# mimbres/neural-audio-fp

Hardware: AMD Instinct MI355X
Metric: fingerprint generation throughput (1-s segments/s) (higher is better)
Workload: dtype f32

## Files before the change

### include/nafp.h

```cpp
#ifndef NAFP_H
#define NAFP_H

#include <stdint.h>

#ifdef __cplusplus
extern "C" {
#endif

#define NAFP_ABI_VERSION 1

enum {
    NAFP_OK = 0,
    NAFP_ERR_INVALID_ARG = 1,
    NAFP_ERR_UNSUPPORTED = 2,
    NAFP_ERR_HIP = 3,
    NAFP_ERR_WORKSPACE = 4,
    NAFP_ERR_NO_WEIGHTS = 5
};

typedef struct nafp_melspec nafp_melspec;
typedef struct nafp_encoder nafp_encoder;

int nafp_abi_version(void);
const char* nafp_status_string(int status);
// ... 165 lines not shown
    int64_t n_indexed;
    int64_t indexed_samples;
    int32_t rate, channels, bps, min_block, max_block, refusal;
    uint8_t md5[16];
} nafp_flac_info;

typedef struct nafp_flac_index_entry {
    int64_t offset;
    int64_t first_sample;
    int64_t n_bytes;
    int32_t block_size;
    int32_t reserved;
} nafp_flac_index_entry;

typedef struct nafp_flac_frame {
    int64_t raw_off;
    int64_t scratch_off;
    int32_t n_bytes;
    int32_t block_size;
    int32_t channels;
    int32_t bps;
    int32_t rate;
    int32_t reserved;
} nafp_flac_frame;

int nafp_flac_streaminfo_host(const void* bytes, int64_t n_bytes, nafp_flac_info* info);
int nafp_flac_index_host(const void* bytes, int64_t n_bytes, nafp_flac_info* info, nafp_flac_index_entry* frames_out, int64_t cap);
int nafp_flac_decode_host(const void* raw, int64_t raw_size, const nafp_flac_frame* frames_host, int64_t n_frames, void* scratch,
                          int64_t scratch_size, int32_t* status_out);
int nafp_flac_check_frames_host(const nafp_flac_frame* frames_host, int64_t n_frames, int64_t raw_size, int64_t scratch_size);
int nafp_flac_decode(const uint8_t* raw, int64_t raw_size, const nafp_flac_frame* frames_dev, int64_t n_frames, uint8_t* scratch,
                     int64_t scratch_size, int32_t* status_dev, void* stream);


int nafp_encoder_create(nafp_encoder** enc, int in_f, int in_t, int emb_sz);
int nafp_encoder_destroy(nafp_encoder* enc);

#define NAFP_NORM_LAYER2D 0
#define NAFP_NORM_LAYER1D 1
#define NAFP_NORM_BATCH 2
int nafp_encoder_create_ex(nafp_encoder** enc, int in_f, int in_t, int emb_sz, int norm);
int nafp_encoder_norm(const nafp_encoder* enc);
int nafp_encoder_n_trainable(const nafp_encoder* enc);

int nafp_encoder_n_tensors(const nafp_encoder* enc);
int64_t nafp_encoder_tensor_numel(const nafp_encoder* enc, int index);
int nafp_encoder_tensor_shape(const nafp_encoder* enc, int index, int64_t dims_out[4]);
int64_t nafp_encoder_flat_dim(const nafp_encoder* enc);

int nafp_encoder_set_weights(nafp_encoder* enc, const float* const* tensors_host_array,
                             void* stream);

int64_t nafp_encoder_workspace_bytes(const nafp_encoder* enc, int64_t n_seg);

int nafp_encoder_forward(nafp_encoder* enc, const float* feat, int64_t n_seg,
                         void* workspace, int64_t workspace_bytes,
                         float* out_flat, float* out_emb, int l2norm, void* stream);

int nafp_encoder_forward_raw(nafp_encoder* enc, const float* raw_feat, const float* group_stat, int group_size,
                             int segment_norm, int64_t n_seg, void* workspace, int64_t workspace_bytes,
                             float* out_flat, float* out_emb, int l2norm, void* stream);

int64_t nafp_encoder_conv0_numel(const nafp_encoder* enc);
int nafp_encoder_conv0(nafp_encoder* enc, const float* feat, const float* group_stat, int group_size, int segment_norm,
                       int64_t n_seg, float* z0_out, long long* stats_out, void* stream);

#define NAFP_ENCODER_PROFILE_KERNELS 17
int nafp_encoder_profile_enable(nafp_encoder* enc, int max_forwards);
int nafp_encoder_profile_count(const nafp_encoder* enc);
int nafp_encoder_profile_coarse(nafp_encoder* enc, int coarse);
int nafp_encoder_profile_read(nafp_encoder* enc, int slot, float* ms_out_host);
int nafp_conv_timeline(void* dev_buf, int64_t capacity_u64, int cin, int cout, int positions);
int nafp_conv_timeline_grid(int* out5_host);
#define NAFP_CONV_PLAN_FIELDS 30
#define NAFP_PLAN_PLAIN 1
#define NAFP_PLAN_DGRAD 2
#define NAFP_PLAN_V_OUT 4
#define NAFP_PLAN_TICKETS 8
#define NAFP_PLAN_SPLIT_WEIGHTS 16
#define NAFP_PLAN_FUSE0 32
#define NAFP_PLAN_SIZE_DGRAD 64
int nafp_conv_plan(int in_f, int in_t, int layer, int64_t n_seg, int64_t plan_b, int flags, int64_t slab_floats,
                   int64_t* record_host, char* kernel_name_host, int name_capacity);

int64_t nafp_encoder_train_workspace_bytes(const nafp_encoder* enc, int64_t n_seg);
int nafp_encoder_forward_train(nafp_encoder* enc, const float* feat, int64_t n_seg, void* workspace,
                               int64_t workspace_bytes, float* out_emb, int l2norm, void* stream);
int nafp_encoder_backward(nafp_encoder* enc, const float* feat, const float* d_emb, int64_t n_seg,
                          void* workspace, int64_t workspace_bytes, float* const* grads_host_array,
                          int l2norm, void* stream);

#define NAFP_GRAD_GROUPS 4
int nafp_encoder_grad_group_range(const nafp_encoder* enc, int group, int* first_tensor, int* last_tensor);
int nafp_encoder_grad_group_wait(nafp_encoder* enc, int group, void* stream);

#define NAFP_OPT_FUSE_CONV0 1
#define NAFP_OPT_FUSED_LN_BWD 2
#define NAFP_OPT_BWD_OVERLAP 4
#define NAFP_OPT_SMALLNET 5
#define NAFP_OPT_BF16X3 3
#define NAFP_OPT_NONMATRIX 8
#define NAFP_NONMATRIX_CONV0 1
#define NAFP_NONMATRIX_KEEP_OWN 2
#define NAFP_NONMATRIX_ALL 3
#define NAFP_NONMATRIX_DEFAULT NAFP_NONMATRIX_ALL
int nafp_encoder_set_option(nafp_encoder* enc, int option, int value);

int nafp_encoder_div_enc(nafp_encoder* enc, const float* flat, int64_t n_seg,
                         float* out_emb, int l2norm, void* stream);

int nafp_l2_normalize_rows(const float* x, int64_t n_rows, int dim, float* out, void* stream);

int nafp_pack_embedding_grads(const float* d_a_all, const float* d_b_all, const float* loss_sum, float loss_scale,
                              int64_t world, int64_t n_anchors, int dim, float* send, void* stream);


int64_t nafp_ntxent_workspace_bytes(int64_t n_local, int64_t n_global);

int nafp_ntxent_forward(const float* emb_org_local, const float* emb_rep_local,
                        const float* emb_org_all, const float* emb_rep_all,
                        int64_t n_local, int64_t n_global, int64_t rank_offset, int d,
                        float tau, float* loss_sum, float* sim_mtx,
                        float* d_org_all, float* d_rep_all,
                        void* workspace, int64_t workspace_bytes, void* stream);


typedef struct { int f0, f1, t0, t1; } nafp_rect;

int nafp_specaug_apply(float* feat, int64_t n_seg, int F, int T, const nafp_rect* rects_host,
                       int n_rects, const unsigned char* active, float fill_value, void* stream);

int nafp_specaug_apply_fill_dev(float* feat, int64_t n_seg, int F, int T, const nafp_rect* rects_host,
                                int n_rects, const unsigned char* active, const float* fill_value_dev,
                                void* stream);
int64_t nafp_specaug_mean_workspace_bytes(void);
int nafp_specaug_mean(const float* feat, int64_t n, float* mean_out, void* workspace, int64_t workspace_bytes,
                      void* stream);

int nafp_specaug_apply_ex(float* feat, int64_t n_seg, int F, int T, const int32_t* rects_dev, int n_rects, int64_t n_sets,
                          const unsigned char* active_dev, const float* filler, int64_t n_fill_seg,
                          const float* scale_offset_dev, void* stream);
int nafp_specaug_range(const float* feat, int64_t n, float* scale_offset_out, void* workspace, int64_t workspace_bytes,
                       void* stream);


typedef struct {
    float* param; const float* grad; float* m; float* v;
    int64_t numel; int64_t var_len;
} nafp_opt_tensor;

float nafp_cosine_decay_lr_host(float lr0, int64_t step, int64_t decay_steps, float alpha);
float nafp_cosine_decay_restarts_lr_host(float lr0, int64_t step, int64_t first_decay_steps, float t_mul,
                                         float m_mul, float alpha);

int nafp_adam_step(const nafp_opt_tensor* tensors_host, int n, float lr, float beta1, float beta2,
                   float eps, int64_t step, void* stream);

int64_t nafp_lamb_workspace_bytes(const nafp_opt_tensor* tensors_host, int n);
int nafp_lamb_step(const nafp_opt_tensor* tensors_host, int n, float lr, float beta1, float beta2,
                   float eps, float weight_decay, int64_t step, void* workspace,
                   int64_t workspace_bytes, void* stream);

int64_t nafp_triplet_workspace_bytes(int64_t n_anchor, int64_t n_pos);
int nafp_triplet_forward(const float* emb_anchor, const float* emb_pos, int64_t n_anchor, int64_t n_pos, int dim,
                         int mode, float margin, float* loss_out, float* pairwise_dist, float* d_anchor,
                         float* d_pos, void* workspace, int64_t workspace_bytes, void* stream);
// ... 156 lines not shown
```

### neural-audio-fp_amd/_lib.py

```python
import ctypes
import os

import torch

_HERE = os.path.dirname(os.path.abspath(__file__))
LIB_PATH = os.environ.get('NAFP_LIB') or os.path.join(_HERE, 'libnafp.so')

c_i64 = ctypes.c_int64
c_int = ctypes.c_int
c_float = ctypes.c_float
c_void_p = ctypes.c_void_p

PROTOTYPES = {
    'nafp_abi_version': (c_int, []),
    'nafp_status_string': (ctypes.c_char_p, [c_int]),
    'nafp_last_hip_error': (c_int, []),
    'nafp_crc32c_host': (ctypes.c_uint32, [c_void_p, c_i64, ctypes.c_uint32]),
    'nafp_mel_filterbank_host': (c_int, [c_int, c_int, c_int, c_float, c_float, c_void_p]),
    'nafp_melspec_create': (c_int, [ctypes.POINTER(c_void_p), c_int, c_int, c_int, c_int, c_int, c_float, c_float]),
    'nafp_melspec_create_ex': (c_int, [ctypes.POINTER(c_void_p), c_int, c_int, c_int, c_int, c_int, c_float, c_float, c_int]),
    'nafp_melspec_plan_host': (c_int, [c_int, c_int, c_int, c_int, c_int, c_float, c_float, c_int, c_void_p]),
    'nafp_melspec_kernel': (c_int, [c_void_p]),
    'nafp_melspec_destroy': (c_int, [c_void_p]),
    'nafp_melspec_n_frames': (c_int, [c_void_p]),
    'nafp_melspec_n_mels': (c_int, [c_void_p]),
    'nafp_melspec_forward_f32': (c_int, [c_void_p, c_void_p, c_i64, c_int, c_int, c_void_p, c_void_p, c_void_p]),
    'nafp_melspec_forward_i16': (c_int, [c_void_p, c_void_p, c_i64, c_int, c_int, c_void_p, c_void_p, c_void_p]),
    'nafp_melspec_finish': (c_int, [c_void_p, c_void_p, c_void_p, c_i64, c_int, c_int, c_void_p]),
    'nafp_melspec_forward_windows_i16': (c_int, [c_void_p, c_void_p, c_void_p, c_void_p, c_i64, c_int, c_int, c_void_p,
                                                 c_void_p, c_void_p]),
    'nafp_resample_geometry': (c_int, [c_int, c_int, ctypes.POINTER(c_int), ctypes.POINTER(c_int), ctypes.POINTER(c_int),
                                       ctypes.POINTER(c_int)]),
    'nafp_resample_table_host': (c_int, [c_int, c_int, c_void_p]),
    'nafp_resample_n_out': (c_i64, [c_i64, c_int, c_int]),
    'nafp_resample_input_range': (c_int, [c_i64, c_i64, c_i64, c_int, c_int, ctypes.POINTER(c_i64), ctypes.POINTER(c_i64)]),
    'nafp_resample_check_pieces_host': (c_int, [c_int, c_int, c_void_p, c_i64, c_i64, c_i64]),
    'nafp_resample_create': (c_int, [ctypes.POINTER(c_void_p), c_int, c_int]),
    'nafp_resample_destroy': (c_int, [c_void_p]),
    'nafp_resample_i16': (c_int, [c_void_p, c_void_p, c_i64, c_void_p, c_i64, c_void_p, c_i64, c_void_p]),
    'nafp_ingest_geometry': (c_int, [c_int, c_int, ctypes.POINTER(c_int), ctypes.POINTER(c_int), ctypes.POINTER(c_int),
                                     ctypes.POINTER(c_int)]),
    'nafp_ingest_table_host': (c_int, [c_int, c_int, c_void_p]),
    'nafp_ingest_n_out': (c_i64, [c_i64, c_int, c_int]),
    'nafp_ingest_input_range': (c_int, [c_i64, c_i64, c_i64, c_int, c_int, ctypes.POINTER(c_i64), ctypes.POINTER(c_i64)]),
    'nafp_ingest_decode_host': (c_int, [c_int, c_void_p, c_i64, c_void_p]),
    'nafp_ingest_check_pieces_host': (c_int, [c_int, c_int, c_void_p, c_i64, c_i64, c_i64]),
    'nafp_ingest_create': (c_int, [ctypes.POINTER(c_void_p), c_int, c_int]),
    'nafp_ingest_destroy': (c_int, [c_void_p]),
    'nafp_ingest_i16': (c_int, [c_void_p, c_void_p, c_i64, c_void_p, c_i64, c_void_p, c_i64, c_void_p]),
    'nafp_varispeed_geometry': (c_int, [ctypes.c_uint32, ctypes.POINTER(c_int), ctypes.POINTER(c_int)]),
    'nafp_varispeed_table_host': (c_int, [ctypes.c_uint32, c_void_p]),
    'nafp_varispeed_n_out': (c_i64, [c_i64, ctypes.c_uint32]),
    'nafp_varispeed_input_range': (c_int, [c_i64, c_i64, c_i64, ctypes.c_uint32, ctypes.POINTER(c_i64), ctypes.POINTER(c_i64)]),
    'nafp_varispeed_check_pieces_host': (c_int, [ctypes.c_uint32, c_void_p, c_i64, c_i64, c_i64]),
    'nafp_varispeed_create': (c_int, [ctypes.POINTER(c_void_p), ctypes.c_uint32]),
    'nafp_varispeed_destroy': (c_int, [c_void_p]),
    'nafp_varispeed_i16': (c_int, [c_void_p, c_void_p, c_i64, c_void_p, c_i64, c_void_p, c_i64, c_void_p]),
    'nafp_codec_samples_per_block': (c_int, [c_int, c_int, c_int]),
    'nafp_codec_blocks_per_group': (c_int, [c_int, c_int, c_int]),
    'nafp_codec_decode_host': (c_int, [c_int, c_int, c_int, c_void_p, c_i64, c_void_p]),
    'nafp_codec_check_pieces_host': (c_int, [c_void_p, c_i64, c_i64, c_i64]),
    'nafp_codec_decode_i16': (c_int, [c_void_p, c_i64, c_void_p, c_i64, c_void_p, c_i64, c_void_p]),
    'nafp_flac_streaminfo_host': (c_int, [c_void_p, c_i64, c_void_p]),
    'nafp_flac_index_host': (c_int, [c_void_p, c_i64, c_void_p, c_void_p, c_i64]),
    'nafp_flac_decode_host': (c_int, [c_void_p, c_i64, c_void_p, c_i64, c_void_p, c_i64, c_void_p]),
    'nafp_flac_check_frames_host': (c_int, [c_void_p, c_i64, c_i64, c_i64]),
    'nafp_flac_decode': (c_int, [c_void_p, c_i64, c_void_p, c_i64, c_void_p, c_i64, c_void_p, c_void_p]),
    'nafp_encoder_create': (c_int, [ctypes.POINTER(c_void_p), c_int, c_int, c_int]),
    'nafp_encoder_create_ex': (c_int, [ctypes.POINTER(c_void_p), c_int, c_int, c_int, c_int]),
    'nafp_encoder_norm': (c_int, [c_void_p]),
    'nafp_encoder_n_trainable': (c_int, [c_void_p]),
    'nafp_encoder_destroy': (c_int, [c_void_p]),
    'nafp_encoder_n_tensors': (c_int, [c_void_p]),
    'nafp_encoder_tensor_numel': (c_i64, [c_void_p, c_int]),
    'nafp_encoder_tensor_shape': (c_int, [c_void_p, c_int, ctypes.POINTER(c_i64)]),
    'nafp_encoder_flat_dim': (c_i64, [c_void_p]),
    'nafp_encoder_set_weights': (c_int, [c_void_p, ctypes.POINTER(c_void_p), c_void_p]),
    'nafp_encoder_workspace_bytes': (c_i64, [c_void_p, c_i64]),
    'nafp_encoder_forward': (c_int, [c_void_p, c_void_p, c_i64, c_void_p, c_i64, c_void_p, c_void_p, c_int, c_void_p]),
    'nafp_encoder_forward_raw': (c_int, [c_void_p, c_void_p, c_void_p, c_int, c_int, c_i64, c_void_p, c_i64, c_void_p, c_void_p,
                                         c_int, c_void_p]),
    'nafp_encoder_conv0_numel': (c_i64, [c_void_p]),
    'nafp_encoder_conv0': (c_int, [c_void_p, c_void_p, c_void_p, c_int, c_int, c_i64, c_void_p, c_void_p, c_void_p]),
    'nafp_encoder_profile_enable': (c_int, [c_void_p, c_int]),
    'nafp_encoder_profile_count': (c_int, [c_void_p]),
    'nafp_encoder_profile_coarse': (c_int, [c_void_p, c_int]),
    'nafp_encoder_profile_read': (c_int, [c_void_p, c_int, c_void_p]),
    'nafp_conv_timeline': (c_int, [c_void_p, c_i64, c_int, c_int, c_int]),
    'nafp_conv_timeline_grid': (c_int, [c_void_p]),
    'nafp_conv_plan': (c_int, [c_int, c_int, c_int, c_i64, c_i64, c_int, c_i64, c_void_p, c_void_p, c_int]),
    'nafp_encoder_set_option': (c_int, [c_void_p, c_int, c_int]),
    'nafp_encoder_train_workspace_bytes': (c_i64, [c_void_p, c_i64]),
    'nafp_encoder_forward_train': (c_int, [c_void_p, c_void_p, c_i64, c_void_p, c_i64, c_void_p, c_int, c_void_p]),
    'nafp_encoder_backward': (c_int, [c_void_p, c_void_p, c_void_p, c_i64, c_void_p, c_i64,
                                      ctypes.POINTER(c_void_p), c_int, c_void_p]),
    'nafp_encoder_grad_group_range': (c_int, [c_void_p, c_int, ctypes.POINTER(c_int), ctypes.POINTER(c_int)]),
    'nafp_encoder_grad_group_wait': (c_int, [c_void_p, c_int, c_void_p]),
    'nafp_encoder_div_enc': (c_int, [c_void_p, c_void_p, c_i64, c_void_p, c_int, c_void_p]),
    'nafp_ntxent_workspace_bytes': (c_i64, [c_i64, c_i64]),
    'nafp_ntxent_forward': (c_int, [c_void_p, c_void_p, c_void_p, c_void_p, c_i64, c_i64, c_i64, c_int,
                                    c_float, c_void_p, c_void_p, c_void_p, c_void_p, c_void_p, c_i64, c_void_p]),
    'nafp_specaug_apply': (c_int, [c_void_p, c_i64, c_int, c_int, c_void_p, c_int, c_void_p, c_float, c_void_p]),
    'nafp_specaug_apply_fill_dev': (c_int, [c_void_p, c_i64, c_int, c_int, c_void_p, c_int, c_void_p, c_void_p, c_void_p]),
    'nafp_specaug_mean_workspace_bytes': (c_i64, []),
    'nafp_specaug_mean': (c_int, [c_void_p, c_i64, c_void_p, c_void_p, c_i64, c_void_p]),
    'nafp_specaug_apply_ex': (c_int, [c_void_p, c_i64, c_int, c_int, c_void_p, c_int, c_i64, c_void_p, c_void_p, c_i64, c_void_p, c_void_p]),
    'nafp_specaug_range': (c_int, [c_void_p, c_i64, c_void_p, c_void_p, c_i64, c_void_p]),
    'nafp_l2_normalize_rows': (c_int, [c_void_p, c_i64, c_int, c_void_p, c_void_p]),
    'nafp_pack_embedding_grads': (c_int, [c_void_p, c_void_p, c_void_p, c_float, c_i64, c_i64, c_int, c_void_p, c_void_p]),
    'nafp_cosine_decay_lr_host': (c_float, [c_float, c_i64, c_i64, c_float]),
    'nafp_cosine_decay_restarts_lr_host': (c_float, [c_float, c_i64, c_i64, c_float, c_float, c_float]),
    'nafp_adam_step': (c_int, [c_void_p, c_int, c_float, c_float, c_float, c_float, c_i64, c_void_p]),
    'nafp_lamb_workspace_bytes': (c_i64, [c_void_p, c_int]),
    'nafp_triplet_workspace_bytes': (c_i64, [c_i64, c_i64]),
    'nafp_triplet_forward': (c_int, [c_void_p, c_void_p, c_i64, c_i64, c_int, c_int, c_float, c_void_p, c_void_p, c_void_p,
                                     c_void_p, c_void_p, c_i64, c_void_p]),
    'nafp_augment_rows': (c_int, [c_void_p, c_void_p, c_i64, c_int, c_void_p, c_void_p]),
    'nafp_search_index_aux_floats': (c_i64, [c_i64]),
    'nafp_search_index_prepare': (c_int, [c_void_p, c_i64, c_int, c_void_p, c_void_p]),
    'nafp_search_workspace_bytes': (c_i64, [c_i64, c_i64, c_int]),
    'nafp_search_topk_l2': (c_int, [c_void_p, c_i64, c_void_p, c_void_p, c_i64, c_int, c_int, c_void_p, c_void_p,
                                    c_void_p, c_i64, c_void_p]),
    'nafp_search_topk_l2_excl': (c_int, [c_void_p, c_i64, c_void_p, c_void_p, c_i64, c_int, c_int, c_void_p, c_void_p, c_void_p,
                                         c_void_p, c_i64, c_void_p]),
    'nafp_search_seq_scores': (c_int, [c_void_p, c_void_p, c_i64, c_int, c_void_p, c_void_p, c_i64, c_void_p, c_int,
                                       c_void_p, c_void_p]),
    'nafp_search_seq_match': (c_int, [c_void_p, c_i64, c_void_p, c_i64, c_int, c_void_p, c_int, c_void_p, c_void_p, c_i64, c_int,
                                      c_int, c_void_p, c_void_p, c_void_p, c_void_p]),
    'nafp_search_identify': (c_int, [c_void_p, c_i64, c_void_p, c_i64, c_int, c_void_p, c_int, c_void_p, c_void_p, c_i64, c_int,
                                     c_void_p, c_int, c_int, c_int, c_int, c_int, c_void_p, c_void_p, c_void_p, c_void_p, c_void_p,
                                     c_void_p, c_void_p]),
    'nafp_search_identify_check_tracks_host': (c_int, [c_void_p, c_int, c_i64]),
    'nafp_search_identify_tempo': (c_int, [c_void_p, c_i64, c_void_p, c_i64, c_int, c_void_p, c_int, c_void_p, c_void_p, c_i64, c_int,
                                           c_void_p, c_int, c_void_p, c_int, c_int, c_int, c_int, c_int, c_void_p, c_void_p, c_void_p,
                                           c_void_p, c_void_p, c_void_p, c_void_p, c_void_p]),
    'nafp_ivf_bucket_workspace_bytes': (c_i64, [c_i64, c_int, c_int]),
    'nafp_ivf_bucket': (c_int, [c_void_p, c_int, c_i64, c_int, c_int, c_void_p, c_void_p, c_void_p, c_i64, c_void_p]),
    'nafp_ivf_kmeans_update': (c_int, [c_void_p, c_i64, c_int, c_int, c_void_p, c_void_p, c_int, c_void_p, c_void_p, c_void_p]),
    'nafp_ivf_residuals': (c_int, [c_void_p, c_i64, c_int, c_void_p, c_void_p, c_void_p, c_void_p]),
    'nafp_ivf_pq_encode': (c_int, [c_void_p, c_i64, c_int, c_void_p, c_void_p, c_void_p, c_int, c_void_p, c_void_p]),
    'nafp_ivf_probe': (c_int, [c_void_p, c_i64, c_void_p, c_int, c_int, c_int, c_void_p, c_void_p]),
    'nafp_ivf_flat_rows_bound': (c_i64, [c_i64, c_int]),
    'nafp_ivf_flat_lists': (c_int, [c_void_p, c_i64, c_int, c_void_p, c_void_p, c_int, c_void_p, c_void_p, c_void_p, c_void_p,
                                    c_void_p]),
    'nafp_ivf_pq_lists': (c_int, [c_void_p, c_i64, c_int, c_void_p, c_void_p, c_void_p]),
    'nafp_ivf_search_workspace_bytes': (c_i64, [c_i64, c_int, c_int, c_int, c_int]),
    'nafp_ivf_flat_search': (c_int, [c_void_p, c_i64, c_void_p, c_int, c_int, c_int, c_void_p, c_void_p, c_void_p, c_void_p, c_int,
                                     c_void_p, c_void_p, c_void_p, c_i64, c_void_p]),
    'nafp_ivf_pq_search': (c_int, [c_void_p, c_i64, c_void_p, c_int, c_int, c_int, c_void_p, c_int, c_void_p, c_void_p, c_void_p,
                                   c_int, c_void_p, c_void_p, c_void_p, c_i64, c_void_p]),
    'nafp_ivf_pq_search_ex': (c_int, [c_void_p, c_i64, c_void_p, c_int, c_int, c_int, c_void_p, c_int, c_void_p, c_void_p, c_void_p,
                                      c_int, c_void_p, c_void_p, c_int, c_void_p, c_i64, c_void_p]),
    'nafp_ivf_pq_adc_tables': (c_int, [c_void_p, c_i64, c_void_p, c_void_p, c_i64, c_void_p, c_int, c_int, c_void_p, c_int, c_int,
                                       c_void_p, c_void_p]),
    'nafp_ivf_pq_residuals': (c_int, [c_void_p, c_i64, c_int, c_void_p, c_int, c_void_p, c_void_p, c_void_p]),
    'nafp_ivf_refine_encode': (c_int, [c_void_p, c_i64, c_int, c_void_p, c_int, c_int, c_int, c_void_p, c_void_p]),
    'nafp_ivf_pq_wide_workspace_bytes': (c_i64, [c_i64, c_int, c_int, c_int]),
    'nafp_ivf_pq_search_wide': (c_int, [c_void_p, c_i64, c_void_p, c_int, c_int, c_int, c_void_p, c_int, c_void_p, c_void_p, c_void_p,
                                        c_int, c_void_p, c_void_p, c_int, c_void_p, c_i64, c_void_p]),
    'nafp_ivf_pqr_rerank': (c_int, [c_void_p, c_i64, c_int, c_void_p, c_int, c_void_p, c_void_p, c_void_p, c_int, c_void_p, c_void_p,
                                    c_int, c_int, c_void_p, c_i64, c_int, c_void_p, c_void_p, c_void_p]),
    'nafp_ivf_pqr_search': (c_int, [c_void_p, c_i64, c_void_p, c_int, c_int, c_int, c_void_p, c_int, c_void_p, c_void_p, c_void_p,
                                    c_void_p, c_void_p, c_void_p, c_int, c_int, c_void_p, c_i64, c_int, c_int, c_void_p, c_void_p,
                                    c_void_p, c_void_p, c_int, c_void_p, c_i64, c_void_p]),
    'nafp_hnsw_default_max_expansions': (c_int, [c_int]),
    'nafp_hnsw_reverse_workspace_bytes': (c_i64, [c_i64, c_i64, c_int, c_int]),
    'nafp_hnsw_search_workspace_bytes': (c_i64, [c_i64, c_int, c_int]),
    'nafp_hnsw_search_layer': (c_int, [c_void_p, c_i64, c_int, c_void_p, c_void_p, c_i64, c_i64, c_int, c_int, c_void_p, c_i64, c_void_p,
                                       c_void_p, c_int, c_int, c_int, c_void_p, c_void_p, c_void_p]),
    'nafp_hnsw_select_forward': (c_int, [c_void_p, c_i64, c_int, c_i64, c_i64, c_void_p, c_int, c_int, c_void_p, c_void_p, c_int, c_void_p,
                                         c_void_p, c_i64, c_i64, c_void_p]),
    'nafp_hnsw_reverse_links': (c_int, [c_void_p, c_i64, c_int, c_i64, c_i64, c_void_p, c_int, c_int, c_void_p, c_void_p, c_i64, c_i64,
                                        c_void_p, c_i64, c_void_p]),
# ... 97 lines not shown
```

### neural-audio-fp_amd/build.py

```python
import hashlib
import os
import subprocess
import sys
from concurrent.futures import ThreadPoolExecutor

HERE = os.path.dirname(os.path.abspath(__file__))
CSRC = os.path.join(HERE, 'csrc')
OBJ = os.path.join(HERE, 'build')
LIB = os.path.join(HERE, 'libnafp.so')
STAMP = os.path.join(HERE, '.libnafp.stamp')
SOURCES = ['api.hip', 'melspec.hip', 'melspec_any.hip', 'conv.hip', 'conv_plan.hip', 'tail.hip', 'ntxent.hip', 'optim.hip', 'specaug.hip', 'backward.hip',
           'search.hip', 'augment.hip', 'triplet.hip', 'norm.hip', 'ivf.hip', 'hnsw.hip', 'resample.hip', 'ingest.hip', 'codec.hip', 'flac.hip', 'varispeed.hip']
HEADERS = ['nafp_common.h', 'melspec_plan.h', 'codec_decode.h', 'flac_decode.h', os.path.join('..', '..', 'include', 'nafp.h')]
NO_PACKED_F32 = ['-Xclang', '-target-feature', '-Xclang', '-packed-fp32-ops']
FLAGS = ['--offload-arch=gfx950', '-O3', '-std=c++17', '-fPIC', '-Wall', '-Wno-unused-result', '-fno-gpu-rdc'] + NO_PACKED_F32
RESOURCE_FLAG = '-Rpass-analysis=kernel-resource-usage'


def _sha(paths, extra=''):
    h = hashlib.sha256()
    for f in paths:
        with open(os.path.join(CSRC, f), 'rb') as fh:
            h.update(fh.read())
    h.update(extra.encode())
    return h.hexdigest()


def _digest():
    return _sha(SOURCES + HEADERS, ' '.join(FLAGS))


def build(force=False, verbose=True):
    want = _digest()
    if not force and os.path.exists(LIB) and os.path.exists(STAMP):
        with open(STAMP) as fh:
            if fh.read().strip() == want:
                return LIB
    hipcc = os.environ.get('HIPCC', '/opt/rocm/bin/hipcc')
    os.makedirs(OBJ, exist_ok=True)

    def compile_one(src):
        obj = os.path.join(OBJ, src[:-4] + '.o')
        tag = _sha([src] + HEADERS, ' '.join(FLAGS))
        tag_path = obj + '.sha'
        if not force and os.path.exists(obj) and os.path.exists(tag_path) and open(tag_path).read().strip() == tag:
            return obj
        cmd = [hipcc] + FLAGS + [RESOURCE_FLAG, '-c', os.path.join(CSRC, src), '-o', obj]
        if verbose:
            print('[nafp build]', ' '.join(cmd), flush=True)
        res = subprocess.run(cmd, check=False, stderr=subprocess.PIPE, text=True)
        remarks = [ln for ln in res.stderr.splitlines() if 'kernel-resource-usage' in ln]
        rest = [ln for ln in res.stderr.splitlines() if 'kernel-resource-usage' not in ln and "'-packed-fp32-ops' is not a recognized feature" not in ln]
        if rest:
            print('\n'.join(rest), file=sys.stderr, flush=True)
        if res.returncode != 0:
            raise subprocess.CalledProcessError(res.returncode, cmd)
        with open(obj[:-2] + '.resources.txt', 'w') as fh:
            fh.write('\n'.join(ln.split('remark: ', 1)[-1].replace(' [-Rpass-analysis=kernel-resource-usage]', '') for ln in remarks) + '\n')
        with open(tag_path, 'w') as fh:
            fh.write(tag)
        return obj

    with ThreadPoolExecutor(max_workers=min(len(SOURCES), os.cpu_count() or 1, 8)) as pool:
        objs = list(pool.map(compile_one, SOURCES))
    cmd = [hipcc, '--offload-arch=gfx950', '-shared', '-fPIC', '-fno-gpu-rdc'] + objs + ['-o', LIB]
    if verbose:
        print('[nafp build]', ' '.join(cmd), flush=True)
    subprocess.run(cmd, check=True)
    with open(STAMP, 'w') as fh:
        fh.write(want)
    return LIB


def device_disassembly(lib=None):
    import struct
    import tempfile
    lib = lib or LIB
    llvm = os.environ.get('LLVM_BIN', '/opt/rocm/lib/llvm/bin')
    out = []
    with tempfile.TemporaryDirectory() as tmp:
        fat = os.path.join(tmp, 'fat.bin')
        subprocess.run([os.path.join(llvm, 'llvm-objcopy'), '--dump-section', '.hip_fatbin=' + fat, lib, os.path.join(tmp, 'unused.so')], check=True)
        blob = open(fat, 'rb').read()
        magic = b'__CLANG_OFFLOAD_BUNDLE__'
        at, n_obj = blob.find(magic), 0
        while at >= 0:
            n_entries, = struct.unpack_from('<Q', blob, at + len(magic))
            pos = at + len(magic) + 8
            for _ in range(n_entries):
                off, size, tlen = struct.unpack_from('<QQQ', blob, pos)
                triple = blob[pos + 24: pos + 24 + tlen].decode()
                pos += 24 + tlen
                if 'gfx950' in triple and size:
                    co = os.path.join(tmp, f'co{n_obj}.o')
                    with open(co, 'wb') as fh:
                        fh.write(blob[at + off: at + off + size])
# ... 31 lines not shown
```

### neural-audio-fp_amd/csrc/api.hip

```cpp
#include "nafp_common.h"

#include <algorithm>
#include <cstdio>
#include <cstdlib>
#include <cstring>
#include <vector>

namespace nafp {

thread_local int g_last_hip_error = 0;

static const int kHiddenCh[8] = {128, 128, 256, 256, 512, 512, 1024, 1024};
static const int kStrideT[8] = {2, 2, 2, 2, 1, 2, 1, 2};

std::vector<ConvGeom> encoder_geometry(int in_f, int in_t) {
    std::vector<ConvGeom> g;
    int F = in_f, T = in_t, C = 1;
    for (int i = 0; i < 8; ++i) {
        SamePad pt = same_pad(T, 3, kStrideT[i]);
        g.push_back(ConvGeom{0, F, T, C, F, pt.n_out, kHiddenCh[i], kStrideT[i], pt.before});
        T = pt.n_out; C = kHiddenCh[i];
        SamePad pf = same_pad(F, 3, 2);
        g.push_back(ConvGeom{1, F, T, C, pf.n_out, T, kHiddenCh[i], 2, pf.before});
        F = pf.n_out;
    }
    return g;
}

struct CopyTable { const float* src[96]; float* dst[96]; int64_t n[96]; int nz[96]; int count; int* nonfinite; };
__device__ __forceinline__ float nz_scale(float g) { return fabsf(g) < 1e-30f ? copysignf(1e-30f, g) : g; }
__device__ __forceinline__ bool nonfinite4(float4 v) {
    return !(fabsf(v.x) <= 3.4028234664e38f) || !(fabsf(v.y) <= 3.4028234664e38f) || !(fabsf(v.z) <= 3.4028234664e38f) || !(fabsf(v.w) <= 3.4028234664e38f);
}
__global__ __launch_bounds__(256) void multi_copy_kernel(const CopyTable t) {
    const int e = blockIdx.y;
    const float* __restrict__ s = t.src[e]; float* __restrict__ d = t.dst[e];
    const int64_t n = t.n[e];
    const bool nz = t.nz[e] != 0;
    bool bad = false;
    if ((((uintptr_t)s | (uintptr_t)d) & 15) == 0) {
        for (int64_t i = blockIdx.x * 256ll + threadIdx.x; i < n / 4; i += (int64_t)gridDim.x * 256) {
            float4 v = ((const float4*)s)[i];
            bad = bad || nonfinite4(v);
            if (nz) { v.x = nz_scale(v.x); v.y = nz_scale(v.y); v.z = nz_scale(v.z); v.w = nz_scale(v.w); }
            ((float4*)d)[i] = v;
        }
        for (int64_t i = n / 4 * 4 + blockIdx.x * 256ll + threadIdx.x; i < n; i += (int64_t)gridDim.x * 256) {
            bad = bad || !(fabsf(s[i]) <= 3.4028234664e38f);
            d[i] = nz ? nz_scale(s[i]) : s[i];
        }
    } else {
        for (int64_t i = blockIdx.x * 256ll + threadIdx.x; i < n; i += (int64_t)gridDim.x * 256) {
            bad = bad || !(fabsf(s[i]) <= 3.4028234664e38f);
            d[i] = nz ? nz_scale(s[i]) : s[i];
        }
    }
    if (bad && t.nonfinite) atomicOr(t.nonfinite, 1);
}
#define NAFP_OPT_DEBUG_SIDE_DELAY 6
#define NAFP_OPT_DEBUG_SW_DELAY 7
__global__ void debug_delay_kernel(long long us) {
    const unsigned long long t0 = __builtin_amdgcn_s_memrealtime();
    while ((long long)(__builtin_amdgcn_s_memrealtime() - t0) < us * 100) __builtin_amdgcn_s_sleep(32);
}
struct BiasTable { float* hb[16]; const float* bias[16]; int64_t n[16]; int cout[16]; int count; };
__global__ __launch_bounds__(256) void add_bias_kernel(const BiasTable t) {
    const int e = blockIdx.y;
    float* __restrict__ h = t.hb[e]; const float* __restrict__ b = t.bias[e];
    const int64_t n = t.n[e]; const int C = t.cout[e];
    for (int64_t i = blockIdx.x * 256ll + threadIdx.x; i < n; i += (int64_t)gridDim.x * 256) h[i] += b[i % C];
}

}

using namespace nafp;

constexpr int NAFP_PROF_EV = 34;
struct nafp_encoder {
    int in_f, in_t, emb_sz;
    int norm = NAFP_NORM_LAYER2D;
    int n_trainable = 68;
    std::vector<float*> d_gc, d_bc, d_mm, d_mv;
    bool ln1d_images_set = false;
// ... 580 lines not shown
    t.w1p = e->d_w1p; t.b1p = e->d_b1p; t.w2p = e->d_w2p; t.b2 = e->d_b2;
    t.out_flat = out_flat; t.out_emb = out_emb;
    t.D = (int)e->flat_dim; t.Q = e->emb_sz; t.S = e->S; t.l2norm = l2norm; t.nonfinite_weights = e->d_wflag; t.launch_error = nullptr;
    if (ev && e->prof_coarse < 2) NAFP_HIP_CHECK(hipEventRecord(ev[32], st));
    rc = launch_tail(t, n_seg, st);
    if (rc != NAFP_OK) return rc;
    if (ev && e->prof_coarse < 2) NAFP_HIP_CHECK(hipEventRecord(ev[33], st));
    return NAFP_OK;
}

extern "C" int nafp_encoder_profile_enable(nafp_encoder* e, int max_forwards) {
    if (!e || max_forwards < 0 || max_forwards > 4096) return NAFP_ERR_INVALID_ARG;
    profile_free(e);
    for (int i = 0; i < max_forwards * NAFP_PROF_EV; ++i) {
        hipEvent_t ev;
        static const int ev_mode = []() { const char* v = getenv("NAFP_PROF_EVENT_FENCE"); return v ? atoi(v) : 0; }();
        hipError_t err = ev_mode == 1 ? hipEventCreate(&ev)
                         : hipEventCreateWithFlags(&ev, ev_mode == 2 ? hipEventReleaseToDevice : hipEventDisableSystemFence);
        if (err != hipSuccess) { g_last_hip_error = (int)err; profile_free(e); return NAFP_ERR_HIP; }
        e->prof_events.push_back(ev);
    }
    e->prof_max = max_forwards;
    return NAFP_OK;
}

extern "C" int nafp_encoder_profile_coarse(nafp_encoder* e, int coarse) {
    if (!e) return NAFP_ERR_INVALID_ARG;
    e->prof_coarse = coarse < 0 ? 0 : (coarse > 2 ? 2 : coarse);
    return NAFP_OK;
}

extern "C" int nafp_encoder_profile_count(const nafp_encoder* e) { return e ? e->prof_count : -1; }

extern "C" int nafp_encoder_profile_read(nafp_encoder* e, int slot, float* ms_out_host) {
    if (!e || !ms_out_host || slot < 0 || slot >= e->prof_count) return NAFP_ERR_INVALID_ARG;
    hipEvent_t* ev = e->prof_events.data() + (size_t)NAFP_PROF_EV * slot;
    NAFP_HIP_CHECK(hipEventSynchronize(e->prof_coarse == 2 ? ev[31] : ev[33]));
    for (int k = 0; k < 17; ++k) ms_out_host[k] = 0.f;
    if (e->prof_coarse == 2) {
        NAFP_HIP_CHECK(hipEventElapsedTime(ms_out_host + 1, ev[2], ev[31]));
        return NAFP_OK;
    }
    NAFP_HIP_CHECK(hipEventElapsedTime(ms_out_host + 0, ev[0], ev[1]));
    NAFP_HIP_CHECK(hipEventElapsedTime(ms_out_host + 16, ev[32], ev[33]));
    if (e->prof_coarse) {
        NAFP_HIP_CHECK(hipEventElapsedTime(ms_out_host + 1, ev[1], ev[32]));
        return NAFP_OK;
    }
    for (int j = 1; j < 16; ++j) NAFP_HIP_CHECK(hipEventElapsedTime(ms_out_host + j, ev[2 * j], ev[2 * j + 1]));
    return NAFP_OK;
}

extern "C" int nafp_conv_timeline(void* dev_buf, int64_t capacity_u64, int cin, int cout, int positions) {
    if (dev_buf && capacity_u64 <= 0) return NAFP_ERR_INVALID_ARG;
    return conv_timeline_set((unsigned long long*)dev_buf, capacity_u64, cin, cout, positions);
}
extern "C" int nafp_conv_timeline_grid(int* out5_host) {
    if (!out5_host) return NAFP_ERR_INVALID_ARG;
    return conv_timeline_grid(out5_host);
}

extern "C" int nafp_conv_plan(int in_f, int in_t, int layer, int64_t n_seg, int64_t plan_b, int flags, int64_t slab_floats,
                              int64_t* record_host, char* kernel_name_host, int name_capacity) {
    if (in_f <= 0 || in_t <= 0 || layer < 1 || layer > 15 || n_seg <= 0 || plan_b < 0 || slab_floats < 0 || !record_host) return NAFP_ERR_INVALID_ARG;
    const std::vector<ConvGeom> geom = encoder_geometry(in_f, in_t);
    ConvPlanIn in{};
    in.B = n_seg; in.plan_b = plan_b; in.slab_floats = slab_floats;
    in.plain = flags & NAFP_PLAN_PLAIN; in.dgrad = flags & NAFP_PLAN_DGRAD; in.v_out = flags & NAFP_PLAN_V_OUT; in.tickets = flags & NAFP_PLAN_TICKETS;
    in.split_weights = flags & NAFP_PLAN_SPLIT_WEIGHTS; in.bf16x3 = (flags >> 8) & 3;
    in.fuse0 = flags & NAFP_PLAN_FUSE0; in.f0_geom = in.fuse0 ? &geom[0] : nullptr;
    const ConvPlan pl = plan_conv_gemm(in, geom[layer], conv_knobs());
    for (int i = 0; i < NAFP_CONV_PLAN_FIELDS; ++i) record_host[i] = 0;
    record_host[29] = conv_gemm_slab_floats(n_seg, geom[layer], (flags & NAFP_PLAN_SIZE_DGRAD) != 0, plan_b);
    if (pl.rc != NAFP_OK) return pl.rc;
    const ConvKernelRow& row = conv_kernel_rows[pl.kernel];
    const int64_t rec[29] = {pl.kernel, pl.BM, pl.bn, row.ring, pl.lds_bytes, pl.grid.x, pl.grid.y, pl.grid.z, pl.PT, pl.ST, pl.n_sg, pl.n_pb, pl.k_steps,
                             pl.S, pl.finish, pl.finish_f4, pl.finish_grid, pl.mode, row.epi, row.arith, pl.perm_on, pl.perm_n0, pl.perm_c0,
                             pl.opt, pl.xcd_group, pl.xcd_full, pl.log2_ncol, pl.range_step, pl.abl};
    for (int i = 0; i < 29; ++i) record_host[i] = rec[i];
    if (kernel_name_host && name_capacity > 0) snprintf(kernel_name_host, (size_t)name_capacity, "%s", row.name);
    return NAFP_OK;
}

extern "C" int nafp_encoder_div_enc(nafp_encoder* e, const float* flat, int64_t n_seg,
                                    float* out_emb, int l2norm, void* stream) {
    if (!e || !flat || !out_emb || n_seg < 0) return NAFP_ERR_INVALID_ARG;
    if (!e->has_weights) return NAFP_ERR_NO_WEIGHTS;
    TailArgs t;
    t.x = flat; t.stats = nullptr; t.ident_stats = false; t.gamma = nullptr; t.beta = nullptr;
    t.w1p = e->d_w1p; t.b1p = e->d_b1p; t.w2p = e->d_w2p; t.b2 = e->d_b2;
    t.out_flat = nullptr; t.out_emb = out_emb;
    t.D = (int)e->flat_dim; t.Q = e->emb_sz; t.S = e->S; t.l2norm = l2norm; t.nonfinite_weights = e->d_wflag; t.launch_error = nullptr;
    { int wrc = wait_weights(e, (hipStream_t)stream); if (wrc != NAFP_OK) return wrc; }
    return launch_tail(t, n_seg, (hipStream_t)stream);
}


namespace {
struct TrainLayout {
    int64_t B;
    stat_t* stats; unsigned* tickets; float* mr; float* sc;
    char* zero_begin; int64_t zero_bytes;
    double* lnsum[16]; float* S1[16]; float* S2[16];
    float* z[16]; float* v[16];
    float* slab; int64_t slab_floats;
    float* slab2; int64_t slab2_floats; unsigned* tickets2;
    float* dA; float* dB; float* dy;
    float* dts[16];
    float* dgp; float* dbp;
    int64_t bytes;
};

TrainLayout train_layout(const nafp_encoder* e, int64_t B, void* ws) {
    TrainLayout L; L.B = B;
    char* p = (char*)(((uintptr_t)ws + 255) & ~(uintptr_t)255);
    char* p0 = p;
    auto take = [&](int64_t bytes) { char* r = p; p += (bytes + 255) / 256 * 256; return r; };
    L.stats = (stat_t*)take((int64_t)sizeof(stat_t) * 2 * 16 * B);
    L.tickets = (unsigned*)take(2 * NAFP_TICKET_SLOTS * (int64_t)sizeof(unsigned));
    L.tickets2 = L.tickets + NAFP_TICKET_SLOTS;
    L.mr = (float*)take((int64_t)sizeof(float) * 2 * 16 * B);
    L.sc = (float*)take((int64_t)sizeof(float) * 8 * B);
    L.zero_begin = p;
    for (int j = 0; j < 16; ++j) L.lnsum[j] = (double*)take((int64_t)sizeof(double) * 2 * B);
    for (int j = 0; j < 16; ++j) {
        const int64_t n = (int64_t)e->geom[j].Fout * e->geom[j].Tout * e->geom[j].Cout;
        L.S1[j] = (float*)take((int64_t)sizeof(float) * n);
        L.S2[j] = (float*)take((int64_t)sizeof(float) * n);
    }
    L.zero_bytes = p - L.zero_begin;
    int64_t max_n = 0;
    for (int j = 0; j < 16; ++j) {
        const int64_t n = (int64_t)e->geom[j].Fout * e->geom[j].Tout * e->geom[j].Cout;
        max_n = std::max(max_n, n);
        L.z[j] = (float*)take((int64_t)sizeof(float) * n * B);
        L.v[j] = ((j == 0 && e->norm != NAFP_NORM_LAYER1D) || !e->keep_t()) ? nullptr : (float*)take((int64_t)sizeof(float) * n * B);
    }
    L.slab_floats = 0;
    for (int j = 1; j < 16; ++j)
        L.slab_floats = std::max(L.slab_floats, std::max(conv_gemm_slab_floats(B, e->geom[j], true), wgrad_slab_floats(B, e->geom[j])));
    L.slab = (float*)take((int64_t)sizeof(float) * L.slab_floats);
    L.slab2_floats = 0;
    for (int j = 1; j < 16; ++j)
        if (e->geom[j].Fout * e->geom[j].Tout < 16) L.slab2_floats = std::max(L.slab2_floats, wgrad_slab_floats(B, e->geom[j]));
    L.slab2 = (float*)take((int64_t)sizeof(float) * L.slab2_floats);
    L.dA = (float*)take((int64_t)sizeof(float) * max_n * B);
    L.dB = (float*)take((int64_t)sizeof(float) * max_n * B);
    L.dy = (float*)take((int64_t)sizeof(float) * e->emb_sz * B);
    for (int j = 0; j < 16; ++j) {
        const int64_t n = (int64_t)e->geom[j].Fout * e->geom[j].Tout * e->geom[j].Cout;
        L.dts[j] = (j >= 1 && e->geom[j].Fout * e->geom[j].Tout < 16) ? (float*)take((int64_t)sizeof(float) * n * B) : nullptr;
    }
    L.dgp = nullptr; L.dbp = nullptr;
    if (e->norm != NAFP_NORM_LAYER2D) {
        L.dgp = (float*)take((int64_t)sizeof(float) * 2 * max_n);
        L.dbp = L.dgp + max_n;
    }
    L.bytes = (p - p0) + 256;
    return L;
}
}

extern "C" int64_t nafp_encoder_train_workspace_bytes(const nafp_encoder* e, int64_t n_seg) {
    if (!e || n_seg < 0) return -1;
    return train_layout(e, n_seg, nullptr).bytes;
}
// ... 252 lines not shown
```

### neural-audio-fp_amd/csrc/conv.hip

```cpp
#include "nafp_common.h"
#include <hip/hip_ext.h>

#include <cstdlib>

namespace nafp {

using f32x16 = __attribute__((ext_vector_type(16))) float;
using f32x2 = __attribute__((ext_vector_type(2))) float;
#ifndef NAFP_Z_AUX
#define NAFP_Z_AUX 0
#endif
#ifndef NAFP_T_AUX
#define NAFP_T_AUX 2
#endif
__device__ __forceinline__ int f2i(float x) { return __builtin_bit_cast(int, x); }

__device__ __forceinline__ f32x2 elu2(f32x2 t) {
    const f32x2 m = t * 1.44269504088896341f;
    f32x2 e;
    e.x = fminf(fmaxf(__builtin_amdgcn_exp2f(m.x), 0.f), 1.f);
    e.y = fminf(fmaxf(__builtin_amdgcn_exp2f(m.y), 0.f), 1.f);
    e = e - 1.0f;
    f32x2 r;
    r.x = fmaxf(t.x, e.x); r.y = fmaxf(t.y, e.y);
    return r;
}



template <bool STORE, int ROWS0>
__global__ __launch_bounds__(256) void conv0_kernel(
        const float* __restrict__ feat, const float* __restrict__ w3, const float* __restrict__ bias,
        const float* __restrict__ gamma, float* __restrict__ y, float* __restrict__ v_out,
        stat_t* __restrict__ stats, int F, int Tin, int Tout, int Cout, int stride, int pad,
        const float* __restrict__ gstat, int group_size, int segment_norm, int ident_stats) {
    constexpr int NP = 4;
    __shared__ float s_x[ROWS0 * 64 + 8];
    __shared__ double red[8];
    const int tid = threadIdx.x, lane = tid & 63, wave = tid >> 6;
    const int blocks_per_sample = (F + ROWS0 - 1) / ROWS0;
    const int64_t b = blockIdx.x / blocks_per_sample;
    const int f0 = (blockIdx.x % blocks_per_sample) * ROWS0;
    const int cgroups = Cout / 4;
    const int pos_per_iter = 256 / cgroups;
    const int cg = tid % cgroups, pslot = tid / cgroups;
    const int rows = min(ROWS0, F - f0);
    const int npos = rows * Tout;
    {
        float gmax = 0.f, nh = 0.f, nd = 1.f;
        if (gstat) {
            const int64_t g = group_size > 0 ? b / group_size : 0;
            gmax = gstat[2 * g];
            if (segment_norm) {
                const float mn = fmaxf(gstat[2 * g + 1] - gmax, -80.f);
                nh = mn / 2.f; nd = fabsf(nh + 1e-10f);
            }
        }
        const float* xin = feat + (b * F + f0) * (int64_t)Tin;
        for (int i = tid; i < rows * Tin; i += 256) {
            float v = xin[i];
            if (gstat) {
                v = max_keep_nan(v - gmax, -80.f);
                if (segment_norm) v = (v - nh) / nd;
            }
            s_x[(i / Tin) * 64 + (i % Tin)] = v;
        }
    }
    const float4 w0 = *(const float4*)(w3 + 0 * Cout + 4 * cg);
    const float4 w1 = *(const float4*)(w3 + 1 * Cout + 4 * cg);
    const float4 w2 = *(const float4*)(w3 + 2 * Cout + 4 * cg);
    const float4 bb = *(const float4*)(bias + 4 * cg);
    float* yout = STORE ? y + ((b * F + f0) * (int64_t)Tout) * Cout : nullptr;
    const float* gin = STORE ? gamma + ((int64_t)f0 * Tout) * Cout : nullptr;
    __syncthreads();
    float s = 0.f, q = 0.f;
    float4 g[NP], gn[NP];
#pragma unroll
    for (int i = 0; i < NP; ++i) {
        const int p = pslot + i * pos_per_iter;
        g[i] = make_float4(0.f, 0.f, 0.f, 0.f);
        if (STORE && p < npos) g[i] = *(const float4*)(gin + (int64_t)p * Cout + 4 * cg);
    }
    for (int p0 = pslot; p0 < npos; p0 += NP * pos_per_iter) {
// ... 223 lines not shown
        s += v; q = fmaf(v, v, q);
    }
    if (!live) { s = 0.f; q = 0.f; }
    const double ds = wave_sum((double)s), dq = wave_sum((double)q);
    if (lane == 0) { red[wave] = ds; red[4 + wave] = dq; }
    __syncthreads();
    if (tid == 0) {
        stat_add(stats + 2 * b, red[0] + red[1] + red[2] + red[3]);
        stat_add(stats + 2 * b + 1, red[4] + red[5] + red[6] + red[7]);
    }
}

int launch_conv0_stats(const float* feat, const float* w3, const float* bias, stat_t* stats, int64_t B,
                       const ConvGeom& g, hipStream_t st, const float* gstat, int group_size, int segment_norm) {
    if (g.Cin != 1 || g.axis != 0 || (g.Cout % 4) != 0 || 256 % (g.Cout / 4) != 0 || g.Tin > 64) return NAFP_ERR_UNSUPPORTED;
    static const bool old_form = []() { const char* e = getenv("NAFP_CONV0_STATS_OLD"); return e && e[0] == '1'; }();
    if (!old_form) {
        const int64_t bps = ((int64_t)g.Fin * g.Tout + 255) / 256;
        conv0_stats_kernel<<<dim3((unsigned)(B * bps)), 256, 0, st>>>(feat, w3, bias, stats, g.Fin, g.Tin, g.Tout, g.Cout, g.stride, g.pad,
                                                                      gstat, group_size, segment_norm);
        NAFP_LAUNCH_CHECK();
        return NAFP_OK;
    }
    constexpr int R = 32;
    const int64_t blocks = B * ((g.Fin + R - 1) / R);
    conv0_kernel<false, R><<<dim3((unsigned)blocks), 256, 0, st>>>(feat, w3, bias, nullptr, nullptr, nullptr, stats,
                                                                   g.Fin, g.Tin, g.Tout, g.Cout, g.stride, g.pad, gstat, group_size, segment_norm, 0);
    NAFP_LAUNCH_CHECK();
    return NAFP_OK;
}

constexpr int BN = 128;

#ifdef NAFP_ABLATION
#define NAFP_ABL(p_, bits_) ((p_).abl & (bits_))
#elif defined(NAFP_ABL_CONST)
#define NAFP_ABL(p_, bits_) ((NAFP_ABL_CONST) & (bits_))
#else
#define NAFP_ABL(p_, bits_) (0)
#endif

struct ConvKernelParams {
    const float* x;
    const float* wp;
    const float* wp_hm;
    const unsigned short* wp_l;
    const float* G;
    const float* Hb;
    const float* gamma_out;
    const float* bias;
    const stat_t* stats_in;
    stat_t* stats_out;
    float* y;
    float* v_out;
    int Fin, Tin, Cin, Tout, Cout;
    int axis, stride, pad;
    int B, P;
    int PT, ST, log2ST;
    int n_sg;
    int n_pb, log2_ncol;
    int xcd_group, xcd_full;
    int64_t sample_in;
    int tap_stride;
    double inv_n_in;
    int mode;
    int dgrad;
    int perm_on, perm_n0, perm_c0;
    unsigned wp_bytes;
    int n_split;
    int abl;
    unsigned* tickets;
    float* y_final;
    unsigned long long* tl;
    int opt;
    int keep_own;
    const float* f0_feat;
    const float* f0_w;
    const float* f0_bias;
    const float* f0_gamma;
    int f0_T, f0_stride, f0_pad;
    const float* f0_gstat;
    int f0_group, f0_segnorm;
    ScalarsJob sj;
};

typedef __attribute__((address_space(3))) void* lds_ptr_t;
typedef unsigned u32x4 __attribute__((ext_vector_type(4)));

__device__ __forceinline__ u32x4 make_rsrc(const void* base, unsigned bytes) {
    const unsigned long long a = (unsigned long long)base;
    u32x4 r;
    r.x = __builtin_amdgcn_readfirstlane((unsigned)a);
    r.y = __builtin_amdgcn_readfirstlane((unsigned)(a >> 32) & 0xffffu);
    r.z = __builtin_amdgcn_readfirstlane(bytes);
    r.w = 0x00020000u;
    return r;
}

__device__ __forceinline__ void lds_dma16(unsigned lds_addr, unsigned voff, u32x4 rsrc, unsigned soff) {
    unsigned keep;
    lds_addr = __builtin_amdgcn_readfirstlane(lds_addr);
    soff = __builtin_amdgcn_readfirstlane(soff);
    asm volatile("s_mov_b32 %0, m0\n\ts_mov_b32 m0, %1\n\ts_nop 4\n\t"
                 "buffer_load_dwordx4 %2, %3, %4 offen lds\n\ts_mov_b32 m0, %0"
                 : "=&s"(keep) : "s"(lds_addr), "v"(voff), "s"(rsrc), "s"(soff) : "memory");
}

struct RowGeom { int inner; unsigned mask; };
__device__ __forceinline__ RowGeom row_geom(const ConvKernelParams& p, int pos) {
    const int fo = pos / p.Tout, to = pos - fo * p.Tout;
    RowGeom g; g.mask = 0;
    if (!p.dgrad) {
        int pos0, lim;
        if (p.axis == 0) { pos0 = to * p.stride - p.pad; lim = p.Tin; g.inner = (fo * p.Tin + pos0) * p.Cin; }
        else             { pos0 = fo * p.stride - p.pad; lim = p.Fin; g.inner = (pos0 * p.Tin + to) * p.Cin; }
#pragma unroll
        for (int t = 0; t < 3; ++t)
            if (pos0 + t >= 0 && pos0 + t < lim) g.mask |= 1u << t;
    } else {
        const int u = (p.axis == 0 ? to : fo) + p.pad;
        const int n_out = p.axis == 0 ? p.Tin : p.Fin;
        const int S = p.axis == 0 ? p.Cin : p.Tin * p.Cin;
        const int A0 = p.axis == 0 ? (fo * p.Tin) * p.Cin : to * p.Cin;
        const int sh = p.stride == 2 ? 1 : 0;
        g.inner = A0 + ((u * S) >> sh);
#pragma unroll
        for (int k = 0; k < 3; ++k) {
            const int d = u - k;
            if (d >= 0 && (d & sh) == 0 && (d >> sh) < n_out) g.mask |= 1u << k;
        }
    }
    return g;
}

__device__ __forceinline__ int tile_pos(const ConvKernelParams& p, int idx) {
    if (!p.perm_on || idx >= p.P) return idx;
    if (p.perm_on == 2) {
        const int L = p.Tout, lines = p.P / L, n0 = L - 1;
        if (idx < lines * n0) { const int line = idx / n0; return line * L + (idx - line * n0); }
        return (idx - lines * n0) * L + n0;
    }
    const int n0 = p.perm_n0;
    if (p.axis == 0) {
        const int L = p.Tout, lines = p.P / L, n1 = L - n0;
        if (idx < lines * n0) { const int line = idx / n0; return line * L + 2 * (idx - line * n0) + p.perm_c0; }
        const int j = idx - lines * n0, line = j / n1;
        return line * L + 2 * (j - line * n1) + 1 - p.perm_c0;
    }
    if (idx < n0 * p.Tout) { const int e = idx / p.Tout; return (2 * e + p.perm_c0) * p.Tout + (idx - e * p.Tout); }
    const int j = idx - n0 * p.Tout, e = j / p.Tout;
    return (2 * e + 1 - p.perm_c0) * p.Tout + (j - e * p.Tout);
}

__device__ __forceinline__ float half_wave_sum_dpp(float x) {
    int v = __builtin_bit_cast(int, x);
#define NAFP_DPP_ADD(ctrl_, rmask_)                                                                       \
    v = __builtin_bit_cast(int, __builtin_bit_cast(float, v) +                                            \
                                    __builtin_bit_cast(float, __builtin_amdgcn_update_dpp(0, v, ctrl_, rmask_, 0xf, true)));
    NAFP_DPP_ADD(0x111, 0xf)
    NAFP_DPP_ADD(0x112, 0xf)
    NAFP_DPP_ADD(0x114, 0xf)
    NAFP_DPP_ADD(0x118, 0xf)
    NAFP_DPP_ADD(0x142, 0xa)
#undef NAFP_DPP_ADD
    return __builtin_bit_cast(float, v);
}

#ifndef NAFP_EXP_X6_NOSPLIT
#define NAFP_EXP_X6_NOSPLIT 0
#endif
#ifndef NAFP_EXP_SKIP_TAP2
#define NAFP_EXP_SKIP_TAP2 0
#endif
template <int BM, int BNT, int BK, int NSTAGE, bool FUSE0, int EPI, int PREC = 0>
__device__ __forceinline__ bool conv_gemm_body(const ConvKernelParams& p) {
    static_assert(!FUSE0 || (BK == 16 && BM == 128), "the in-kernel conv0 generator is written for BK = 16, BM = 128");
    static_assert(BM == 128 || BM == 256, "tile rows");
    static_assert(BNT == 128 || (BNT == 64 && BM == 128 && !FUSE0), "tile columns");
    constexpr int NIW = BNT / 64;
    constexpr int NT = 2 * BM;
    constexpr int NW = BM / 32;
    constexpr int CH = BK / 4;
    constexpr int RPI = 64 / CH;
    constexpr int NI = 32 / RPI;
    constexpr int BROWS = BNT / NW;
    constexpr int NIB = BROWS / RPI;
    static_assert(NIB >= 1, "B rows per wave");
    constexpr int TILE = (FUSE0 && PREC == 2) ? BM * 24 : BM * BK;
    constexpr int TILEB = BNT * BK;
    constexpr int LROWS = BNT / NW;
    constexpr int TILEL = PREC == 2 ? BNT * 8 : 0;
    constexpr int STAGE = TILE + TILEB + TILEL;
    constexpr int NDMA = NI + NIB + (PREC == 2 ? 1 : 0);
    extern __shared__ __attribute__((aligned(16))) float smem[];
    float* sRB = smem + NSTAGE * STAGE;
    float* sCB = sRB + BM;
    int* sPos = (int*)(sCB + BM);
    int* sInner = sPos + 32;
    unsigned* sMask = (unsigned*)(sPos + 64);
    float* sW0 = sCB + BM + 96;
    const int tid = threadIdx.x, lane = tid & 63;
    const int wave = __builtin_amdgcn_readfirstlane(tid >> 6);
    const int wm = wave >> 1, wn = wave & 1;
    int sg = blockIdx.x, pb = blockIdx.y, colz = blockIdx.z, zsp = 0;
    if (p.opt & 8) {
        const unsigned lin = blockIdx.x, G = (unsigned)p.xcd_group;
        unsigned v = lin;
        if (lin < (unsigned)p.xcd_full) {
            const unsigned xcd = lin & 7u, j = lin >> 3;
            const unsigned blk = j / G, i = j - blk * G;
            v = (blk * 8u + xcd) * G + i;
        }
        unsigned rt;
        if (p.opt & 16) {
            const unsigned n_rt = (unsigned)(p.n_sg * p.n_pb);
            unsigned t = v / n_rt; rt = v - t * n_rt;
            if (p.n_split > 1) { const unsigned c = t / (unsigned)p.n_split; zsp = (int)(t - c * (unsigned)p.n_split); t = c; }
            colz = (int)t;
        } else {
            colz = (int)(v & ((1u << p.log2_ncol) - 1u)); v >>= p.log2_ncol;
            if (p.n_split > 1) { const unsigned r = v / (unsigned)p.n_split; zsp = (int)(v - r * (unsigned)p.n_split); v = r; }
            rt = v;
        }
        pb = (int)(rt / (unsigned)p.n_sg); sg = (int)(rt - (unsigned)pb * (unsigned)p.n_sg);
    } else
    if (!(p.opt & 4)) { pb = blockIdx.x / p.n_sg; sg = blockIdx.x - pb * p.n_sg; colz = blockIdx.y; zsp = blockIdx.z; }
    if ((EPI == 3 || EPI == 5) && p.sj.sc) {
        const long long wg = blockIdx.x + (long long)gridDim.x * (blockIdx.y + (long long)gridDim.y * blockIdx.z);
        const long long n_wg = (long long)gridDim.x * gridDim.y * gridDim.z;
        for (long long b = wg * NT + tid; b < p.sj.B; b += n_wg * NT) {
            const float mean = p.sj.mr[2 * b], rstd = p.sj.mr[2 * b + 1];
            float* o = p.sj.sc + 8 * b;
            o[0] = mean; o[1] = rstd;
            o[2] = (float)(p.sj.lnsum[2 * b] * p.sj.inv_n); o[3] = (float)(p.sj.lnsum[2 * b + 1] * p.sj.inv_n);
            o[4] = 1.f / rstd;
            o[5] = p.sj.mr_prev ? p.sj.mr_prev[2 * b + 1] : 1.f;
            o[6] = p.sj.mr_prev ? -p.sj.mr_prev[2 * b] : 0.f;
            o[7] = 0.f;
        }
    }
    const int tile_n0 = colz * BNT;
    const int K = 3 * p.Cin;
#define NAFP_TL(k_)                                                                            \
    if (p.tl && lane == 0)                                                                                 \
        p.tl[(((size_t)blockIdx.x + (size_t)gridDim.x * (blockIdx.y + (size_t)gridDim.y * blockIdx.z)) * 8 + wave) * 8 + (k_)] = \
            __builtin_readcyclecounter();
    if (p.tl && lane == 0)
        p.tl[(((size_t)blockIdx.x + (size_t)gridDim.x * (blockIdx.y + (size_t)gridDim.y * blockIdx.z)) * 8 + wave) * 8] =
            (unsigned long long)__builtin_amdgcn_s_getreg(0xF804) |
            ((unsigned long long)__builtin_amdgcn_s_getreg(0xF814) << 32);
    NAFP_TL(1)
    if (p.opt & 1) __builtin_amdgcn_s_setprio(3);
    const int ST1 = p.ST - 1;
    const int b0 = sg * p.ST;
    const int nb = min(p.ST, p.B - b0);

    const bool stat_thread = tid >= 64 && tid < 64 + p.ST;
    double st_sum = 0.0, st_sq = 0.0;
    if (stat_thread && p.mode != 1 && b0 + tid - 64 < p.B) {
        st_sum = stat_get(p.stats_in + 2 * (int64_t)(b0 + tid - 64));
        st_sq = stat_get(p.stats_in + 2 * (int64_t)(b0 + tid - 64) + 1);
        if (st_sq != st_sq && p.stats_out) stat_poison(p.stats_out + 2 * (int64_t)(b0 + tid - 64));
    }
    if (tid < 32) {
        int pos = p.P, inner = 0; unsigned mask = 0;
        if (tid < p.PT) {
            pos = tile_pos(p, pb * p.PT + tid);
            if (pos < p.P) { const RowGeom rg = row_geom(p, pos); inner = rg.inner; mask = rg.mask; }
        }
        sPos[tid] = pos; sInner[tid] = inner; sMask[tid] = mask;
    }
    __syncthreads();

    constexpr unsigned OOB = 0x80000000u;
    unsigned voffA[NI];
    unsigned vmaskA[NI];
    unsigned voffB[NIB];
#pragma unroll
    for (int q = 0; q < NIB; ++q) {
        const int lr = wave * BROWS + q * RPI + lane / CH;
        const int pc = lane % CH;
        const int swz = BK == 32 ? ((lr >> 1) & 7) : ((lr >> 2) & 3);
        voffB[q] = (unsigned)((tile_n0 + lr) * K + (pc ^ swz) * 4) * 4u;
    }
#pragma unroll
    for (int q = 0; q < NI; ++q) {
        const int lr = wave * 32 + q * RPI + lane / CH;
        const int pc = lane % CH;
        const int swz = BK == 32 ? ((lr >> 1) & 7) : ((lr >> 2) & 3);
        const int lc = pc ^ swz;
        const int slot_q = lr >> p.log2ST;
        const int sl = lr & ST1;
        voffA[q] = 0; vmaskA[q] = 0;
        if (sPos[slot_q] < p.P && sl < nb) {
            voffA[q] = (unsigned)(sl * (int)p.sample_in + sInner[slot_q] + lc * 4) * 4u;
            vmaskA[q] = sMask[slot_q];
        }
    }
    float x0[3][3];
    unsigned g_valid = 0;
    int g_off = 0;
    const int g_row = tid >> 1, g_ch = (tid & 1) * 8;
    const int g_swz = (g_row >> 2) & 3;
    if (FUSE0) {
        for (int i = tid; i < 4 * p.Cin; i += NT) sW0[i] = i < 3 * p.Cin ? p.f0_w[i] : p.f0_bias[i - 3 * p.Cin];
#pragma unroll
        for (int t = 0; t < 3; ++t) { x0[t][0] = 0.f; x0[t][1] = 0.f; x0[t][2] = 0.f; }
        const int pos = pb * p.PT + (g_row >> p.log2ST);
        const int sl = g_row & ST1;
        if (pos < p.P && sl < nb) {
            float f0_gmax = 0.f, f0_nh = 0.f, f0_nd = 1.f;
            if (p.f0_gstat) {
                const int64_t gi = p.f0_group > 0 ? (int64_t)(b0 + sl) / p.f0_group : 0;
                f0_gmax = p.f0_gstat[2 * gi];
                if (p.f0_segnorm) { const float mn = fmaxf(p.f0_gstat[2 * gi + 1] - f0_gmax, -80.f); f0_nh = mn / 2.f; f0_nd = fabsf(f0_nh + 1e-10f); }
            }
            const int fo = pos / p.Tout, to = pos - fo * p.Tout;
            const int f00 = fo * p.stride - p.pad;
            g_off = (f00 * p.Tin + to) * p.Cin;
            const int t00 = to * p.f0_stride - p.f0_pad;
            const float* fb = p.f0_feat + ((int64_t)(b0 + sl) * p.Fin) * p.f0_T;
#pragma unroll
            for (int t = 0; t < 3; ++t) {
                const int f = f00 + t;
                if (f >= 0 && f < p.Fin) {
                    g_valid |= 1u << t;
#pragma unroll
                    for (int k = 0; k < 3; ++k) {
                        const int tt = t00 + k;
                        float xv = 0.f;
                        if (tt >= 0 && tt < p.f0_T) {
                            xv = fb[(int64_t)f * p.f0_T + tt];
                            if (p.f0_gstat) {
                                xv = max_keep_nan(xv - f0_gmax, -80.f);
                                if (p.f0_segnorm) xv = (xv - f0_nh) / f0_nd;
                            }
                        }
                        x0[t][k] = xv;
                    }
                }
            }
        }
        __syncthreads();
    }
    unsigned live = 0;
    {
        const unsigned m = sMask[lane & 31];
#pragma unroll
        for (int t = 0; t < 3; ++t)
            if (__ballot((m >> t) & 1u) != 0ull) live |= 1u << t;
    }
    unsigned tap_pack = 0; int n_live = 0;
#pragma unroll
    for (int t = 0; t < 3; ++t)
        if (live & (1u << t)) { tap_pack |= (unsigned)t << (2 * n_live); ++n_live; }
    const int cpt = p.Cin / BK;
    const int n_steps_all = n_live * cpt;
    int s_begin = 0, n_steps = n_steps_all;
    if (p.n_split > 1) {
        s_begin = (int)((unsigned)(n_steps_all * zsp) / (unsigned)p.n_split);
        n_steps = (int)((unsigned)(n_steps_all * (zsp + 1)) / (unsigned)p.n_split);
    }
#define NAFP_STEP_AT(step_, tsel_, c0_)                                                        \
    const int tsel_ = s_begin == 0 ? ((step_) >= cpt ? 1 : 0) : (step_) / cpt;                 \
    const int c0_ = ((step_) - tsel_ * cpt) * BK;

    const u32x4 rsA = make_rsrc(p.x + (int64_t)b0 * p.sample_in,
                                NAFP_ABL(p, 512) ? 0u : (unsigned)nb * (unsigned)p.sample_in * 4u);
    const u32x4 rsB = make_rsrc(PREC == 2 ? p.wp_hm : p.wp, NAFP_ABL(p, 4096) ? 0u : p.wp_bytes);
    const unsigned lds0 = (unsigned)(unsigned long long)(lds_ptr_t)smem + (unsigned)(wave * 32 * BK * 4);
    const unsigned ldsB0 = (unsigned)(unsigned long long)(lds_ptr_t)smem + (unsigned)((TILE + wave * BROWS * BK) * 4);
    const u32x4 rsL = make_rsrc((const float*)p.wp_l, NAFP_ABL(p, 4096) ? 0u : p.wp_bytes / 2);
    const unsigned ldsL0 = (unsigned)(unsigned long long)(lds_ptr_t)smem + (unsigned)((TILE + TILEB) * 4 + wave * LROWS * 32);
    const unsigned voffL = (unsigned)((tile_n0 + wave * LROWS + (lane >> 1)) * K) * 2u + (unsigned)(lane & 1) * 16u;
#define NAFP_DMA_L(slot_, k0_)                                                                 \
    if (PREC == 2 && lane < 2 * LROWS) lds_dma16(ldsL0 + (unsigned)((slot_) * STAGE * 4), voffL, rsL, (unsigned)((k0_) * 2));

#define NAFP_DMA_STEP(s_, slot_)                                                              \
    {                                                                                          \
        NAFP_STEP_AT(s_, tsel_l, c0_l)                                                         \
        const int tap_l = (int)((tap_pack >> (2 * tsel_l)) & 3u);                              \
        const unsigned la_l = lds0 + (unsigned)((slot_) * STAGE * 4);                          \
        const unsigned lb_l = ldsB0 + (unsigned)((slot_) * STAGE * 4);                         \
        const unsigned tapb_l = (unsigned)(tap_l * p.tap_stride) * 4u;                         \
        _Pragma("unroll") for (int q = 0; q < NI; ++q) {                                       \
            const unsigned va = ((vmaskA[q] >> tap_l) & 1u) ? voffA[q] + tapb_l : OOB;         \
            if (!FUSE0) lds_dma16(la_l + q * RPI * BK * 4, va, rsA, (unsigned)(c0_l * 4));     \
            if (q < NIB) lds_dma16(lb_l + q * RPI * BK * 4, voffB[q], rsB,                      \
                                   (unsigned)((tap_l * p.Cin + c0_l) * 4));                    \
        }                                                                                      \
        NAFP_DMA_L(slot_, tap_l * p.Cin + c0_l)                                                \
    }
    float4 gg0 = make_float4(0.f, 0.f, 0.f, 0.f), gg1 = gg0;
#define NAFP_GEN_LOAD(s_)                                                                     \
    {                                                                                          \
        const int tsel_l = (s_) / cpt;                                                         \
        const int tap_l = (int)((tap_pack >> (2 * tsel_l)) & 3u);                              \
        const int c0_l = ((s_) - tsel_l * cpt) * BK;                                           \
        const int go_l = ((g_valid >> tap_l) & 1u) ? g_off + tap_l * p.tap_stride + c0_l + g_ch : 0; \
        gg0 = *(const float4*)(p.f0_gamma + go_l);                                             \
        gg1 = *(const float4*)(p.f0_gamma + go_l + 4);                                         \
    }
#define NAFP_GEN_ONE(j_, G_) \
    __fmul_rn((ok_l ? elu1(fmaf(xc_l, wt_l[2 * p.Cin + (j_)], fmaf(xb_l, wt_l[p.Cin + (j_)], fmaf(xa_l, wt_l[(j_)], wt_l[3 * p.Cin + (j_)])))) : 0.f), (G_))
#define NAFP_GEN_STORE(s_, slot_)                                                             \
    {                                                                                          \
        const int tsel_l = (s_) / cpt;                                                         \
        const int tap_l = (int)((tap_pack >> (2 * tsel_l)) & 3u);                              \
        const int c0_l = ((s_) - tsel_l * cpt) * BK;                                           \
        const bool ok_l = (g_valid >> tap_l) & 1u;                                             \
        const float xa_l = tap_l == 0 ? x0[0][0] : (tap_l == 1 ? x0[1][0] : x0[2][0]);         \
        const float xb_l = tap_l == 0 ? x0[0][1] : (tap_l == 1 ? x0[1][1] : x0[2][1]);         \
        const float xc_l = tap_l == 0 ? x0[0][2] : (tap_l == 1 ? x0[1][2] : x0[2][2]);         \
        const float* wt_l = sW0 + c0_l + g_ch;                                                 \
        float* dst_l = smem + (slot_) * STAGE + g_row * BK;                                    \
        *(float4*)(dst_l + (((2 * (tid & 1)) ^ g_swz) * 4)) = make_float4(                      \
            NAFP_GEN_ONE(0, gg0.x), NAFP_GEN_ONE(1, gg0.y), NAFP_GEN_ONE(2, gg0.z), NAFP_GEN_ONE(3, gg0.w)); \
        *(float4*)(dst_l + (((2 * (tid & 1) + 1) ^ g_swz) * 4)) = make_float4(                  \
            NAFP_GEN_ONE(4, gg1.x), NAFP_GEN_ONE(5, gg1.y), NAFP_GEN_ONE(6, gg1.z), NAFP_GEN_ONE(7, gg1.w)); \
    }

    f32x16 acc[2][NIW];
#pragma unroll
    for (int mi = 0; mi < 2; ++mi)
#pragma unroll
        for (int ni = 0; ni < NIW; ++ni)
#pragma unroll
            for (int r = 0; r < 16; ++r) acc[mi][ni][r] = 0.f;

    NAFP_TL(2)
    if (p.opt & 1) __builtin_amdgcn_s_setprio(0);
#pragma unroll
    for (int s = 0; s < NSTAGE - 1; ++s)
        if (s_begin + s < n_steps) {
            NAFP_DMA_STEP(s_begin + s, s)
            if (FUSE0 && PREC != 2) {
                NAFP_GEN_LOAD(s_begin + s)
                NAFP_GEN_STORE(s_begin + s, s)
            }
        }

    if (stat_thread) {
        float r = 0.f, c = 0.f;
        if (p.mode != 1 && b0 + tid - 64 < p.B) {
            if (p.inv_n_in < 0.0) {
                const double z = st_sq * 0.0;
                r = (float)(1.0 + z); c = (float)z;
            } else {
                const double mean = st_sum * p.inv_n_in;
                double var = st_sq * p.inv_n_in - mean * mean;
                var = var < 0.0 ? 0.0 : var;
                const double rstd = 1.0 / sqrt(var + (double)LN_EPS);
                r = (float)rstd; c = (float)(-mean * rstd);
            }
        }
        sRB[tid - 64] = r; sCB[tid - 64] = c;
    }

    const int rl = lane & 31, hh = lane >> 5;
    const int rswz = BK == 32 ? ((rl >> 1) & 7) : ((rl >> 2) & 3);
    const int aoff = (wm * 64 + rl) * BK, boff = TILE + (wn * (BNT / 2) + rl) * BK;
    const int ncol = lane & 31;
    const int n_base = tile_n0 + wn * (BNT / 2) + ncol;
    const int g4 = p.ST >> 2;
    constexpr int MIL = 1;
    float Gv[MIL][4][NIW], Hv[MIL][4][NIW], gv[MIL][4][NIW];
    const int pc_bytes = p.P * p.Cout * 4;
    const __amdgpu_buffer_rsrc_t rsG = __builtin_amdgcn_make_buffer_rsrc(const_cast<float*>(p.G), 0, pc_bytes, 0x00020000);
    const __amdgpu_buffer_rsrc_t rsH = __builtin_amdgcn_make_buffer_rsrc(const_cast<float*>(p.Hb), 0, pc_bytes, 0x00020000);
    const __amdgpu_buffer_rsrc_t rsg = __builtin_amdgcn_make_buffer_rsrc(const_cast<float*>(p.gamma_out), 0, pc_bytes, 0x00020000);
#define NAFP_EPI_LOAD(mi_, slot_)                                                              \
    _Pragma("unroll") for (int rg = 0; rg < 4; ++rg) {                                         \
        const int grp_l = wm * 16 + (mi_) * 8 + 2 * rg + (lane >> 5);                          \
        const int pos_l = sPos[grp_l >> (p.log2ST - 2)];                \
        const int pofs_l = pos_l < p.P ? (pos_l * p.Cout + n_base) * 4 : (int)0x80000000;      \
        _Pragma("unroll") for (int ni = 0; ni < NIW; ++ni) {                                   \
            if NAFP_ABL(p, 32) { Gv[slot_][rg][ni] = 0.5f; Hv[slot_][rg][ni] = 0.25f; gv[slot_][rg][ni] = 1.5f; continue; } \
            Gv[slot_][rg][ni] = __builtin_bit_cast(float, __builtin_amdgcn_raw_buffer_load_b32(rsG, pofs_l, ni * 128, 0)); \
            Hv[slot_][rg][ni] = __builtin_bit_cast(float, __builtin_amdgcn_raw_buffer_load_b32(rsH, pofs_l, ni * 128, 0)); \
            gv[slot_][rg][ni] = __builtin_bit_cast(float, __builtin_amdgcn_raw_buffer_load_b32(rsg, pofs_l, ni * 128, 0)); \
        }                                                                                      \
    }
    int slot = 0;
    if NAFP_ABL(p, 8) {
        asm volatile("s_waitcnt vmcnt(0)" ::: "memory");
        if (acc[0][0][0] == 12345.678f) p.y[tid] = smem[tid];
        return false;
    }
#define NAFP_LD_FRAG(St_, kk_, a_, b_)                                                         \
    {                                                                                          \
        const int pc4_l = ((2 * (kk_) + hh) ^ rswz) * 4;                                       \
        _Pragma("unroll") for (int mi = 0; mi < 2; ++mi) a_[mi] = *(const float4*)((St_) + aoff + mi * 32 * BK + pc4_l);   \
        _Pragma("unroll") for (int ni = 0; ni < NIW; ++ni) b_[ni] = *(const float4*)((St_) + boff + ni * 32 * BK + pc4_l); \
    }
#define NAFP_MM_FRAG(a_, b_)                                                                   \
    _Pragma("unroll") for (int mi = 0; mi < 2; ++mi)                                           \
        _Pragma("unroll") for (int ni = 0; ni < NIW; ++ni) {                                   \
            acc[mi][ni] = __builtin_amdgcn_mfma_f32_32x32x2f32(a_[mi].x, b_[ni].x, acc[mi][ni], 0, 0, 0); \
            acc[mi][ni] = __builtin_amdgcn_mfma_f32_32x32x2f32(a_[mi].y, b_[ni].y, acc[mi][ni], 0, 0, 0); \
            acc[mi][ni] = __builtin_amdgcn_mfma_f32_32x32x2f32(a_[mi].z, b_[ni].z, acc[mi][ni], 0, 0, 0); \
            acc[mi][ni] = __builtin_amdgcn_mfma_f32_32x32x2f32(a_[mi].w, b_[ni].w, acc[mi][ni], 0, 0, 0); \
        }
#define NAFP_WAIT_STEP(s_)                                                                     \
    if (NSTAGE == 2 || (s_) + NSTAGE - 2 >= n_steps) asm volatile("s_waitcnt vmcnt(0)" ::: "memory"); \
    else asm volatile("s_waitcnt vmcnt(%0)" :: "i"((NSTAGE - 2) * NDMA) : "memory");
    if (!FUSE0 && BK == 16 && !NAFP_ABL(p, 4 | 2048) && s_begin < n_steps) {
        float4 a0[2], b0[NIW], a1[2], b1[NIW];
        NAFP_STEP_AT(s_begin + NSTAGE - 1, d_tsel0, d_c00)
        int d_tsel = d_tsel0, d_c0 = d_c00;
        int d_tap = 0; unsigned d_tapb = 0;
        unsigned cur_va[NI];
#define NAFP_DMA_TAP()                                                                         \
        {                                                                                      \
            d_tap = (int)((tap_pack >> (2 * d_tsel)) & 3u); d_tapb = (unsigned)(d_tap * p.tap_stride) * 4u; \
            _Pragma("unroll") for (int q = 0; q < NI; ++q) cur_va[q] = (((vmaskA[q] >> d_tap) & 1u) && !(NAFP_EXP_SKIP_TAP2 && d_tap == 2)) ? voffA[q] + d_tapb : OOB; \
        }
        NAFP_DMA_TAP()
#define NAFP_DMA_PIECE(q_, slot_)                                                              \
        {                                                                                      \
            lds_dma16(lds0 + (unsigned)((slot_) * STAGE * 4) + (q_) * RPI * BK * 4, cur_va[q_], rsA, (unsigned)(d_c0 * 4)); \
            if ((q_) < NIB) lds_dma16(ldsB0 + (unsigned)((slot_) * STAGE * 4) + (q_) * RPI * BK * 4, voffB[(q_) < NIB ? (q_) : 0], rsB, \
                                      (unsigned)((d_tap * p.Cin + d_c0) * 4));                 \
            if ((q_) == NI - 1) { d_c0 += BK; if (d_c0 == p.Cin) { d_c0 = 0; ++d_tsel; NAFP_DMA_TAP() } } \
        }
#define NAFP_MM_HALF(a_, b_, mi_)                                                              \
        _Pragma("unroll") for (int ni = 0; ni < NIW; ++ni) {                                   \
            acc[mi_][ni] = __builtin_amdgcn_mfma_f32_32x32x2f32(a_[mi_].x, b_[ni].x, acc[mi_][ni], 0, 0, 0); \
            acc[mi_][ni] = __builtin_amdgcn_mfma_f32_32x32x2f32(a_[mi_].y, b_[ni].y, acc[mi_][ni], 0, 0, 0); \
            acc[mi_][ni] = __builtin_amdgcn_mfma_f32_32x32x2f32(a_[mi_].z, b_[ni].z, acc[mi_][ni], 0, 0, 0); \
            acc[mi_][ni] = __builtin_amdgcn_mfma_f32_32x32x2f32(a_[mi_].w, b_[ni].w, acc[mi_][ni], 0, 0, 0); \
        }
        static_assert(NI == 2, "the DMA of a step is issued as two pieces");
        if (PREC >= 1) {
            typedef __bf16 bf16x8 __attribute__((ext_vector_type(8)));
            for (int s = s_begin; s < n_steps; ++s) {
                NAFP_WAIT_STEP(s)
                __builtin_amdgcn_s_barrier();
                if (s == s_begin) { NAFP_TL(3) }
                const bool has_next = s + NSTAGE - 1 < n_steps && !NAFP_ABL(p, 1);
                int nslot = slot + NSTAGE - 1; if (nslot >= NSTAGE) nslot -= NSTAGE;
                const float* St = smem + slot * STAGE;
                float4 af[2][2], bf[PREC == 2 ? 1 : NIW][2];
                bf16x8 ah[2], al[2], bh[NIW], bl[NIW];
                bf16x8 am[PREC == 2 ? 2 : 1], bm[PREC == 2 ? NIW : 1];
#pragma unroll
                for (int c = 0; c < 2; ++c) {
                    const int pc4 = ((2 * hh + c) ^ rswz) * 4;
#pragma unroll
                    for (int mi = 0; mi < 2; ++mi) af[mi][c] = *(const float4*)(St + aoff + mi * 32 * BK + pc4);
                    if (PREC != 2) {
#pragma unroll
                        for (int ni = 0; ni < NIW; ++ni) bf[ni][c] = *(const float4*)(St + boff + ni * 32 * BK + pc4);
                    }
                }
                if (PREC == 2) {
#pragma unroll
                    for (int ni = 0; ni < NIW; ++ni) {
                        bh[ni] = *(const bf16x8*)(St + boff + ni * 32 * BK + ((hh ^ rswz) * 4));
                        bm[ni] = *(const bf16x8*)(St + boff + ni * 32 * BK + (((2 + hh) ^ rswz) * 4));
                        bl[ni] = *(const bf16x8*)(St + TILE + TILEB + (wn * (BNT / 2) + ni * 32 + rl) * 8 + hh * 4);
                    }
                }
                if (has_next) { NAFP_DMA_PIECE(0, nslot) NAFP_DMA_L(nslot, d_tap * p.Cin + d_c0) NAFP_DMA_PIECE(1, nslot) }
#define NAFP_SPLIT8(f_, hi_, mid_, lo_)                                                        \
                {                                                                                  \
                    const float x_l[8] = {f_[0].x, f_[0].y, f_[0].z, f_[0].w, f_[1].x, f_[1].y, f_[1].z, f_[1].w}; \
                    _Pragma("unroll") for (int e = 0; e < 8; ++e) {                                \
                        const __bf16 h_l = (__bf16)x_l[e];                                         \
                        const float r1_l = x_l[e] - (float)h_l;                                    \
                        hi_[e] = h_l;                                                              \
                        if (PREC == 2 && NAFP_EXP_X6_NOSPLIT) {                                    \
                            mid_[e] = h_l; lo_[e] = h_l;       \
                        } else if (PREC == 2) {                                                    \
                            const __bf16 m_l = (__bf16)r1_l;                                       \
                            mid_[e] = m_l; lo_[e] = (__bf16)(r1_l - (float)m_l);                   \
                        } else {                                                                   \
                            lo_[e] = (__bf16)r1_l;                                                 \
                        }                                                                          \
                    }                                                                              \
                }
#define NAFP_SPLIT8_PAIRS(f_, hi_, mid_, lo_)                                                  \
                {                                                                                  \
                    typedef __bf16 bf16x2_l __attribute__((ext_vector_type(2)));                   \
                    typedef float f32x2_l __attribute__((ext_vector_type(2)));                     \
                    typedef unsigned u32x4_l __attribute__((ext_vector_type(4)));                  \
                    const float x_l[8] = {f_[0].x, f_[0].y, f_[0].z, f_[0].w, f_[1].x, f_[1].y, f_[1].z, f_[1].w}; \
                    u32x4_l uh_l, um_l, ul_l;                                                      \
                    _Pragma("unroll") for (int e = 0; e < 4; ++e) {                                \
                        f32x2_l x2; x2.x = x_l[2 * e]; x2.y = x_l[2 * e + 1];                      \
                        const unsigned h2 = __builtin_bit_cast(unsigned, __builtin_convertvector(x2, bf16x2_l)); \
                        f32x2_l r2; r2.x = x2.x - __uint_as_float(h2 << 16); r2.y = x2.y - __uint_as_float(h2 & 0xffff0000u); \
                        const unsigned m2 = __builtin_bit_cast(unsigned, __builtin_convertvector(r2, bf16x2_l)); \
                        f32x2_l t2; t2.x = r2.x - __uint_as_float(m2 << 16); t2.y = r2.y - __uint_as_float(m2 & 0xffff0000u); \
                        uh_l[e] = h2; um_l[e] = m2; ul_l[e] = __builtin_bit_cast(unsigned, __builtin_convertvector(t2, bf16x2_l)); \
                    }                                                                              \
                    hi_ = __builtin_bit_cast(bf16x8, uh_l); mid_ = __builtin_bit_cast(bf16x8, um_l); lo_ = __builtin_bit_cast(bf16x8, ul_l); \
                }
                if (PREC == 2 && !NAFP_EXP_X6_NOSPLIT) {
#pragma unroll
                    for (int mi = 0; mi < 2; ++mi) NAFP_SPLIT8_PAIRS(af[mi], ah[mi], am[PREC == 2 ? mi : 0], al[mi])
                } else {
#pragma unroll
                for (int mi = 0; mi < 2; ++mi) NAFP_SPLIT8(af[mi], ah[mi], am[PREC == 2 ? mi : 0], al[mi])
                }
#undef NAFP_SPLIT8_PAIRS
                if (PREC != 2) {
#pragma unroll
                    for (int ni = 0; ni < NIW; ++ni) NAFP_SPLIT8(bf[PREC == 2 ? 0 : ni], bh[ni], bm[0], bl[ni])
                }
#undef NAFP_SPLIT8
#pragma unroll
                for (int mi = 0; mi < 2; ++mi)
#pragma unroll
                    for (int ni = 0; ni < NIW; ++ni) {
                        if (PREC == 2) {
                            acc[mi][ni] = __builtin_amdgcn_mfma_f32_32x32x16_bf16(al[mi], bh[ni], acc[mi][ni], 0, 0, 0);
                            acc[mi][ni] = __builtin_amdgcn_mfma_f32_32x32x16_bf16(am[PREC == 2 ? mi : 0], bm[PREC == 2 ? ni : 0], acc[mi][ni], 0, 0, 0);
                            acc[mi][ni] = __builtin_amdgcn_mfma_f32_32x32x16_bf16(ah[mi], bl[ni], acc[mi][ni], 0, 0, 0);
                            acc[mi][ni] = __builtin_amdgcn_mfma_f32_32x32x16_bf16(am[PREC == 2 ? mi : 0], bh[ni], acc[mi][ni], 0, 0, 0);
                            acc[mi][ni] = __builtin_amdgcn_mfma_f32_32x32x16_bf16(ah[mi], bm[PREC == 2 ? ni : 0], acc[mi][ni], 0, 0, 0);
                            acc[mi][ni] = __builtin_amdgcn_mfma_f32_32x32x16_bf16(ah[mi], bh[ni], acc[mi][ni], 0, 0, 0);
                        } else {
                            acc[mi][ni] = __builtin_amdgcn_mfma_f32_32x32x16_bf16(al[mi], bh[ni], acc[mi][ni], 0, 0, 0);
                            acc[mi][ni] = __builtin_amdgcn_mfma_f32_32x32x16_bf16(ah[mi], bl[ni], acc[mi][ni], 0, 0, 0);
                            acc[mi][ni] = __builtin_amdgcn_mfma_f32_32x32x16_bf16(ah[mi], bh[ni], acc[mi][ni], 0, 0, 0);
                        }
                    }
                if (++slot == NSTAGE) slot = 0;
            }
        } else {
        {
            NAFP_WAIT_STEP(s_begin)
            __builtin_amdgcn_s_barrier();
            NAFP_TL(3)
            const float* St = smem + slot * STAGE;
            NAFP_LD_FRAG(St, 0, a0, b0)
            NAFP_LD_FRAG(St, 1, a1, b1)
            __builtin_amdgcn_sched_barrier(0);
            if (s_begin + NSTAGE - 1 < n_steps && !NAFP_ABL(p, 1)) { NAFP_DMA_PIECE(0, NSTAGE - 1) NAFP_DMA_PIECE(1, NSTAGE - 1) }
            __builtin_amdgcn_sched_barrier(0);
            NAFP_MM_FRAG(a0, b0)
            __builtin_amdgcn_sched_barrier(0);
            slot = 1;
        }
#define NAFP_K_STEP(SLOT_, NSLOT_)                                                             \
        {                                                                                      \
             \
            asm volatile("s_waitcnt lgkmcnt(0)" ::: "memory");                                 \
            NAFP_WAIT_STEP(s)                                                                  \
            __builtin_amdgcn_s_barrier();                                                      \
            const bool has_next = s + NSTAGE - 1 < n_steps && !NAFP_ABL(p, 1);                 \
            const int nslot = (NSLOT_);                                                        \
            const float* St = smem + (SLOT_) * STAGE;                                          \
            NAFP_LD_FRAG(St, 0, a0, b0)                                                        \
            __builtin_amdgcn_sched_barrier(0);                                                 \
            NAFP_MM_HALF(a1, b1, 0)                                                            \
            __builtin_amdgcn_sched_barrier(0);                                                 \
            if (has_next) { NAFP_DMA_PIECE(0, nslot) }                                         \
            __builtin_amdgcn_sched_barrier(0);                                                 \
            NAFP_MM_HALF(a1, b1, 1)                                                            \
            __builtin_amdgcn_sched_barrier(0);                                                 \
            if (has_next) { NAFP_DMA_PIECE(1, nslot) }                                         \
            NAFP_LD_FRAG(St, 1, a1, b1)                                                        \
            __builtin_amdgcn_sched_barrier(0);                                                 \
            if (s == n_steps - 1) break;           \
            NAFP_MM_FRAG(a0, b0)                                                               \
            __builtin_amdgcn_sched_barrier(0);                                                 \
            ++s;                                                                               \
        }
        static_assert(PREC != 0 || NSTAGE == 3 || BNT == 64, "the K-loop body is written out once per ring slot (128-column tiles)");
        if (s_begin + 1 < n_steps) {
            if (BNT == 128) {
                for (int s = s_begin + 1;;) {
                    NAFP_K_STEP(1, 0)
                    NAFP_K_STEP(2, 1)
                    NAFP_K_STEP(0, 2)
                }
            } else {
                int rs = 1;
                int s = s_begin + 1;
                for (; s < n_steps - 1;) {
                    NAFP_K_STEP(rs, (rs == 0 ? NSTAGE - 1 : rs - 1))
                    if (++rs == NSTAGE) rs = 0;
                }
                do { NAFP_K_STEP(rs, (rs == 0 ? NSTAGE - 1 : rs - 1)) } while (false);
            }
        }
#undef NAFP_K_STEP
        if ((EPI == 0 || EPI == 1) && BM == 128) { NAFP_EPI_LOAD(0, 0) }
        __builtin_amdgcn_sched_barrier(0);
        if (s_begin + 1 < n_steps) { NAFP_MM_FRAG(a0, b0) }
        NAFP_MM_FRAG(a1, b1)
        }
#undef NAFP_DMA_PIECE
#undef NAFP_DMA_TAP
#undef NAFP_MM_HALF
    } else if (FUSE0 && PREC == 2) {
        typedef __bf16 bf16x8 __attribute__((ext_vector_type(8)));
        static_assert(!(FUSE0 && PREC == 2) || NSTAGE == 2, "two ring slots");
        constexpr int C0 = 128;
        const int a_rd = (wm * 64 + rl) * 8 + ((hh ^ ((rl >> 3) & 1)) * 4);
        const int a_wr = g_row * 8 + (((tid & 1) ^ ((g_row >> 3) & 1)) * 4);
        const __amdgpu_buffer_rsrc_t rsG0 = __builtin_amdgcn_make_buffer_rsrc(const_cast<float*>(p.f0_gamma), 0, (int)((unsigned)p.sample_in * 4u), 0x00020000);
        int gvoff0, gvoff1, gvoff2;
        gvoff0 = (g_valid & 1u) ? (g_off + g_ch) * 4 : (int)0x80000000;
        gvoff1 = (g_valid & 2u) ? (g_off + p.tap_stride + g_ch) * 4 : (int)0x80000000;
        gvoff2 = (g_valid & 4u) ? (g_off + 2 * p.tap_stride + g_ch) * 4 : (int)0x80000000;
        const float* wrow = sW0 + g_ch;
        int g_tsel = 0, g_c0 = 0;
        float4 wq[8], gq[2];
        float gxa = 0.f, gxb = 0.f, gxc = 0.f;
#define NAFP_X6_GEN_REQ()                                                                      \
        {                                                                                      \
            const int tap_l = (int)((tap_pack >> (2 * g_tsel)) & 3u);                          \
            gxa = tap_l == 0 ? x0[0][0] : (tap_l == 1 ? x0[1][0] : x0[2][0]);                  \
            gxb = tap_l == 0 ? x0[0][1] : (tap_l == 1 ? x0[1][1] : x0[2][1]);                  \
            gxc = tap_l == 0 ? x0[0][2] : (tap_l == 1 ? x0[1][2] : x0[2][2]);                  \
            const int gv_l = tap_l == 0 ? gvoff0 : (tap_l == 1 ? gvoff1 : gvoff2);             \
            gq[0] = __builtin_bit_cast(float4, __builtin_amdgcn_raw_buffer_load_b128(rsG0, gv_l, g_c0 * 4, 0));      \
            gq[1] = __builtin_bit_cast(float4, __builtin_amdgcn_raw_buffer_load_b128(rsG0, gv_l + 16, g_c0 * 4, 0)); \
            const float* w_l = wrow + g_c0;                                                    \
            _Pragma("unroll") for (int r_ = 0; r_ < 4; ++r_) {                                 \
                wq[2 * r_] = *(const float4*)(w_l + r_ * C0); wq[2 * r_ + 1] = *(const float4*)(w_l + r_ * C0 + 4); \
            }                                                                                  \
            g_c0 += BK; if (g_c0 == C0) { g_c0 = 0; ++g_tsel; }                                \
        }
#define NAFP_X6_GEN_ONE(e_) \
        __fmul_rn(elu1(fmaf(gxc, ((const float*)&wq[4])[e_], fmaf(gxb, ((const float*)&wq[2])[e_], fmaf(gxa, ((const float*)&wq[0])[e_], ((const float*)&wq[6])[e_])))), ((const float*)&gq[0])[e_])
#define NAFP_X6_GEN(slot_)                                                                     \
        {                                                                                      \
            bf16x8 h_l, m_l, l_l;                                                              \
            _Pragma("unroll") for (int e = 0; e < 8; ++e) {                                    \
                const float v_l = NAFP_X6_GEN_ONE(e);                                          \
                const __bf16 hh_l = (__bf16)v_l;                                               \
                const float r1_l = v_l - (float)hh_l;                                          \
                const __bf16 mm_l = (__bf16)r1_l;                                              \
                h_l[e] = hh_l; m_l[e] = mm_l; l_l[e] = (__bf16)(r1_l - (float)mm_l);           \
            }                                                                                  \
            float* dst_l = smem + (slot_) * STAGE + a_wr;                                      \
            *(bf16x8*)dst_l = h_l; *(bf16x8*)(dst_l + BM * 8) = m_l; *(bf16x8*)(dst_l + 2 * BM * 8) = l_l; \
        }
        NAFP_X6_GEN_REQ()
        NAFP_X6_GEN(0)
#define NAFP_X6_MFMAS()                                                                        \
        _Pragma("unroll") for (int mi = 0; mi < 2; ++mi)                                       \
            _Pragma("unroll") for (int ni = 0; ni < NIW; ++ni) {                               \
                acc[mi][ni] = __builtin_amdgcn_mfma_f32_32x32x16_bf16(al[mi], bh[ni], acc[mi][ni], 0, 0, 0); \
                acc[mi][ni] = __builtin_amdgcn_mfma_f32_32x32x16_bf16(am[mi], bm[ni], acc[mi][ni], 0, 0, 0); \
                acc[mi][ni] = __builtin_amdgcn_mfma_f32_32x32x16_bf16(ah[mi], bl[ni], acc[mi][ni], 0, 0, 0); \
                acc[mi][ni] = __builtin_amdgcn_mfma_f32_32x32x16_bf16(am[mi], bh[ni], acc[mi][ni], 0, 0, 0); \
                acc[mi][ni] = __builtin_amdgcn_mfma_f32_32x32x16_bf16(ah[mi], bm[ni], acc[mi][ni], 0, 0, 0); \
                acc[mi][ni] = __builtin_amdgcn_mfma_f32_32x32x16_bf16(ah[mi], bh[ni], acc[mi][ni], 0, 0, 0); \
            }
#define NAFP_X6_READ_FRAGS(St_)                                                                \
        _Pragma("unroll") for (int mi = 0; mi < 2; ++mi) {                                     \
            ah[mi] = *(const bf16x8*)((St_) + a_rd + mi * 32 * 8);                             \
            am[mi] = *(const bf16x8*)((St_) + BM * 8 + a_rd + mi * 32 * 8);                    \
            al[mi] = *(const bf16x8*)((St_) + 2 * BM * 8 + a_rd + mi * 32 * 8);                \
        }                                                                                      \
        _Pragma("unroll") for (int ni = 0; ni < NIW; ++ni) {                                   \
            bh[ni] = *(const bf16x8*)((St_) + boff + ni * 32 * BK + ((hh ^ rswz) * 4));        \
            bm[ni] = *(const bf16x8*)((St_) + boff + ni * 32 * BK + (((2 + hh) ^ rswz) * 4));  \
            bl[ni] = *(const bf16x8*)((St_) + TILE + TILEB + (wn * (BNT / 2) + ni * 32 + rl) * 8 + hh * 4); \
        }
        int s = 0;
        for (; s + 1 < n_steps; ++s) {
            asm volatile("s_waitcnt vmcnt(0) lgkmcnt(0)" ::: "memory");
            __builtin_amdgcn_s_barrier();
            if (s == 0) { NAFP_TL(3) }
            const int nslot = slot ^ 1;
            const float* St = smem + slot * STAGE;
            bf16x8 ah[2], am[2], al[2], bh[NIW], bm[NIW], bl[NIW];
            NAFP_X6_READ_FRAGS(St)
            NAFP_DMA_STEP(s + 1, nslot)
            NAFP_X6_GEN_REQ()
            NAFP_X6_MFMAS()
            NAFP_X6_GEN(nslot)
            slot = nslot;
        }
        {
            asm volatile("s_waitcnt vmcnt(0) lgkmcnt(0)" ::: "memory");
            __builtin_amdgcn_s_barrier();
            const float* St = smem + slot * STAGE;
            bf16x8 ah[2], am[2], al[2], bh[NIW], bm[NIW], bl[NIW];
            NAFP_X6_READ_FRAGS(St)
            NAFP_X6_MFMAS()
        }
#undef NAFP_X6_GEN_REQ
#undef NAFP_X6_GEN_ONE
#undef NAFP_X6_GEN
#undef NAFP_X6_MFMAS
#undef NAFP_X6_READ_FRAGS
    } else
    for (int s = s_begin; s < n_steps; ++s) {
        if (FUSE0) asm volatile("s_waitcnt vmcnt(0) lgkmcnt(0)" ::: "memory");
        else if (NSTAGE == 2 || s + NSTAGE - 2 >= n_steps) asm volatile("s_waitcnt vmcnt(0)" ::: "memory");
        else asm volatile("s_waitcnt vmcnt(%0)" :: "i"((NSTAGE - 2) * (NI + NIB)) : "memory");
        __builtin_amdgcn_s_barrier();
        const bool has_next = s + NSTAGE - 1 < n_steps && !NAFP_ABL(p, 1);
        int nslot = slot + NSTAGE - 1; if (nslot >= NSTAGE) nslot -= NSTAGE;
        const float* St = smem + slot * STAGE;
        if NAFP_ABL(p, 4) {
            if (has_next) { NAFP_DMA_STEP(s + NSTAGE - 1, nslot) }
            if (++slot == NSTAGE) slot = 0;
            continue;
        }
        float4 a0[2], b0[NIW];
        {
            const int pc4 = ((0 + hh) ^ rswz) * 4;
#pragma unroll
            for (int mi = 0; mi < 2; ++mi) a0[mi] = *(const float4*)(St + aoff + mi * 32 * BK + pc4);
#pragma unroll
            for (int ni = 0; ni < NIW; ++ni) b0[ni] = *(const float4*)(St + boff + ni * 32 * BK + pc4);
        }
        if (has_next) {
            NAFP_DMA_STEP(s + NSTAGE - 1, nslot)
            if (FUSE0) NAFP_GEN_LOAD(s + NSTAGE - 1)
        }
#pragma unroll
        for (int kk = 0; kk < BK / 8; ++kk) {
            const int pc4 = ((2 * kk + hh) ^ rswz) * 4;
            float4 a[2], b[NIW];
#pragma unroll
            for (int mi = 0; mi < 2; ++mi) a[mi] = kk == 0 ? a0[mi] : *(const float4*)(St + aoff + mi * 32 * BK + pc4);
#pragma unroll
            for (int ni = 0; ni < NIW; ++ni) b[ni] = kk == 0 ? b0[ni] : *(const float4*)(St + boff + ni * 32 * BK + pc4);
#pragma unroll
            for (int mi = 0; mi < 2; ++mi)
#pragma unroll
                for (int ni = 0; ni < NIW; ++ni) {
                    acc[mi][ni] = __builtin_amdgcn_mfma_f32_32x32x2f32(a[mi].x, b[ni].x, acc[mi][ni], 0, 0, 0);
                    acc[mi][ni] = __builtin_amdgcn_mfma_f32_32x32x2f32(a[mi].y, b[ni].y, acc[mi][ni], 0, 0, 0);
                    acc[mi][ni] = __builtin_amdgcn_mfma_f32_32x32x2f32(a[mi].z, b[ni].z, acc[mi][ni], 0, 0, 0);
                    acc[mi][ni] = __builtin_amdgcn_mfma_f32_32x32x2f32(a[mi].w, b[ni].w, acc[mi][ni], 0, 0, 0);
                }
        }
        if (FUSE0 && has_next) NAFP_GEN_STORE(s + NSTAGE - 1, nslot)
        if (++slot == NSTAGE) slot = 0;
    }
    NAFP_TL(4)
    if (p.opt & 2) __builtin_amdgcn_s_setprio(3);
    asm volatile("s_waitcnt lgkmcnt(0)" ::: "memory");
    __builtin_amdgcn_s_barrier();
    NAFP_TL(5)

    if NAFP_ABL(p, 2) {
        float t = 0.f;
#pragma unroll
        for (int mi = 0; mi < 2; ++mi)
#pragma unroll
            for (int ni = 0; ni < NIW; ++ni)
#pragma unroll
                for (int r = 0; r < 16; ++r) t += acc[mi][ni][r];
        if (t == 12345.678f) p.y[tid] = t;
        return false;
    }
    const int ystep_b = p.P * p.Cout * 4;
    if (EPI == 3) {
        float bv[NIW];
#pragma unroll
        for (int ni = 0; ni < NIW; ++ni) bv[ni] = p.bias ? p.bias[n_base + ni * 32] : 0.f;
#pragma unroll
        for (int ni = 0; ni < NIW; ++ni) asm volatile("" : "+v"(bv[ni]));
        const __amdgpu_buffer_rsrc_t rsP = __builtin_amdgcn_make_buffer_rsrc(
            p.y + ((int64_t)zsp * p.B + b0) * p.P * p.Cout, 0, (int)((unsigned)nb * (unsigned)ystep_b), 0x00020000);
#pragma unroll
        for (int mi = 0; mi < 2; ++mi)
#pragma unroll
            for (int rg = 0; rg < 4; ++rg) {
                const int grp = wm * 16 + mi * 8 + 2 * rg + (lane >> 5);
                const int pos = sPos[grp >> (p.log2ST - 2)];
                const int sl0 = (grp & (g4 - 1)) << 2;
                const int voff = pos < p.P ? ((sl0 * p.P + pos) * p.Cout + n_base) * 4 : (int)0x80000000;
#pragma unroll
                for (int q = 0; q < 4; ++q)
#pragma unroll
                    for (int ni = 0; ni < NIW; ++ni)
                        __builtin_amdgcn_raw_buffer_store_b32(f2i(acc[mi][ni][rg * 4 + q] + bv[ni]), rsP, voff, q * ystep_b + ni * 128, 0);
            }
        NAFP_TL(6)
        NAFP_TL(7)
        return false;
    }

    if (EPI == 4 || EPI == 5) {
        const __amdgpu_buffer_rsrc_t rsP = __builtin_amdgcn_make_buffer_rsrc(
            p.y + ((int64_t)zsp * p.B + b0) * p.P * p.Cout, 0, (int)((unsigned)nb * (unsigned)ystep_b), 0x00020000);
        auto form_voff = [&](int mi, int rg) {
            const int grp = wm * 16 + mi * 8 + 2 * rg + (lane >> 5);
            const int pos = sPos[grp >> (p.log2ST - 2)];
            const int sl0 = (grp & (g4 - 1)) << 2;
            return pos < p.P ? ((sl0 * p.P + pos) * p.Cout + n_base) * 4 : (int)0x80000000;
        };
        int voffs[2][4];
        if (EPI == 5) {
#pragma unroll
            for (int mi = 0; mi < 2; ++mi)
#pragma unroll
                for (int rg = 0; rg < 4; ++rg) voffs[mi][rg] = form_voff(mi, rg);
        }
        auto voff_of = [&](int mi, int rg) { return EPI == 5 ? voffs[mi][rg] : form_voff(mi, rg); };
        auto store_part = [&]() {
#pragma unroll
            for (int mi = 0; mi < 2; ++mi)
#pragma unroll
                for (int rg = 0; rg < 4; ++rg) {
                    const int voff = voff_of(mi, rg);
#pragma unroll
                    for (int q = 0; q < 4; ++q)
#pragma unroll
                        for (int ni = 0; ni < NIW; ++ni)
                            __builtin_amdgcn_raw_buffer_store_b32(f2i(acc[mi][ni][rg * 4 + q]), rsP, voff, q * ystep_b + ni * 128, 17);
                }
            asm volatile("s_waitcnt vmcnt(0)" ::: "memory");
            __builtin_amdgcn_s_barrier();
        };
        unsigned* sTicket = (unsigned*)smem;
        const unsigned tile_id = (unsigned)((pb * p.n_sg + sg) * (p.Cout / BNT) + colz);
        const bool keep_own = EPI == 4 && p.keep_own;
        if (keep_own) {
            __syncthreads();
            if (tid == 0) sTicket[0] = __hip_atomic_fetch_add(p.tickets + tile_id, 1u, __ATOMIC_RELAXED, __HIP_MEMORY_SCOPE_AGENT);
// ... 59 lines not shown
        }
    }

    f32x2 s2[2] = {{0.f, 0.f}, {0.f, 0.f}}, q2[2] = {{0.f, 0.f}, {0.f, 0.f}};
    float* rowS = smem;
    float* rowQ = smem + BM;
    const bool fast_stats = (EPI != 2 && EPI != 4) || p.ST == 4 || p.ST == 8;
    if (!fast_stats) {
        if (tid < BM) { rowS[tid] = 0.f; rowQ[tid] = 0.f; }
        __syncthreads();
    }
    constexpr bool PREF = (EPI == 0 || EPI == 1) && !FUSE0 && BK == 16 && BM == 128 && PREC == 0;
    if (MIL == 2) { if (!PREF) { NAFP_EPI_LOAD(0, 0) } NAFP_EPI_LOAD(1, MIL - 1) }
    const __amdgpu_buffer_rsrc_t rsY = __builtin_amdgcn_make_buffer_rsrc(
        (EPI == 4 ? p.y_final : p.y) + (int64_t)b0 * p.P * p.Cout, 0, (int)((unsigned)nb * (unsigned)ystep_b), 0x00020000);
    const __amdgpu_buffer_rsrc_t rsV = __builtin_amdgcn_make_buffer_rsrc(
        (p.v_out ? p.v_out : (EPI == 4 ? p.y_final : p.y)) + (int64_t)b0 * p.P * p.Cout, 0, (int)((unsigned)nb * (unsigned)ystep_b), 0x00020000);
#define NAFP_EPI_MAIN(KEEP_, FAST_)                                                            \
    _Pragma("unroll") for (int mi = 0; mi < 2; ++mi) {                                         \
        const int ms = MIL == 2 ? mi : 0;                                                      \
        if (MIL == 1 && !(PREF && mi == 0)) { NAFP_EPI_LOAD(mi, 0) }                           \
        _Pragma("unroll") for (int rg = 0; rg < 4; ++rg) {                                     \
            const int grp = wm * 16 + mi * 8 + 2 * rg + (lane >> 5);       \
            const int pos = sPos[grp >> (p.log2ST - 2)];                                       \
            const int sl0 = (grp & (g4 - 1)) << 2;                          \
            const int voff = pos < p.P ? ((sl0 * p.P + pos) * p.Cout + n_base) * 4 : (int)0x80000000; \
            _Pragma("unroll") for (int qp = 0; qp < 2; ++qp) {              \
                const int r0 = rg * 4 + 2 * qp;                                                \
                const f32x2 rb2 = *(const f32x2*)(sRB + sl0 + 2 * qp), cb2 = *(const f32x2*)(sCB + sl0 + 2 * qp); \
                f32x2 rs2 = {0.f, 0.f}, rq2 = {0.f, 0.f};                                      \
                _Pragma("unroll") for (int ni = 0; ni < NIW; ++ni) {                           \
                    const f32x2 a2 = {acc[mi][ni][r0], acc[mi][ni][r0 + 1]};                   \
                    const f32x2 t2 = __builtin_elementwise_fma(rb2, a2, __builtin_elementwise_fma(cb2, (f32x2)(Gv[ms][rg][ni]), (f32x2)(Hv[ms][rg][ni]))); \
                    const f32x2 v2 = NAFP_ABL(p, 128) ? t2 : elu2(t2);     \
                    const f32x2 z2 = v2 * gv[ms][rg][ni];                                      \
                    if (!NAFP_ABL(p, 64)) {                                 \
                        __builtin_amdgcn_raw_buffer_store_b32(f2i(z2.x), rsY, voff, (2 * qp) * ystep_b + ni * 128, NAFP_Z_AUX); \
                        __builtin_amdgcn_raw_buffer_store_b32(f2i(z2.y), rsY, voff, (2 * qp + 1) * ystep_b + ni * 128, NAFP_Z_AUX); \
                    }                                                                          \
                    if (KEEP_) {                                            \
                        __builtin_amdgcn_raw_buffer_store_b32(f2i(t2.x), rsV, voff, (2 * qp) * ystep_b + ni * 128, NAFP_T_AUX); \
                        __builtin_amdgcn_raw_buffer_store_b32(f2i(t2.y), rsV, voff, (2 * qp + 1) * ystep_b + ni * 128, NAFP_T_AUX); \
                    }                                                                          \
                    rs2 += v2; rq2 = __builtin_elementwise_fma(v2, v2, rq2);                   \
                }                                                                              \
                if (FAST_) { s2[qp] += rs2; q2[qp] += rq2; }                                   \
                else {                                                                         \
                    _Pragma("unroll") for (int h2 = 0; h2 < 2; ++h2) {                         \
                        float rs = rs2[h2], rq = rq2[h2];                                      \
                        _Pragma("unroll") for (int o = 16; o > 0; o >>= 1) { rs += __shfl_xor(rs, o, 64); rq += __shfl_xor(rq, o, 64); } \
                        if (ncol == 0) { atomicAdd(rowS + (grp << 2) + 2 * qp + h2, rs); atomicAdd(rowQ + (grp << 2) + 2 * qp + h2, rq); } \
                    }                                                                          \
                }                                                                              \
            }                                                                                  \
        }                                                                                      \
    }
    if (EPI == 0) { NAFP_EPI_MAIN(false, true) }
    else if (EPI == 1) { NAFP_EPI_MAIN(true, true) }
    else if (fast_stats) {
        if (p.v_out) { NAFP_EPI_MAIN(true, true) } else { NAFP_EPI_MAIN(false, true) }
    } else {
        if (p.v_out) { NAFP_EPI_MAIN(true, false) } else { NAFP_EPI_MAIN(false, false) }
    }
#undef NAFP_EPI_MAIN
    NAFP_TL(6)
    if NAFP_ABL(p, 16) {
        if (s2[0].x + s2[0].y + s2[1].x + s2[1].y + q2[0].x + q2[0].y + q2[1].x + q2[1].y == 12345.678f) p.y[tid] = 1.f;
        return false;
    }
    if (fast_stats) {
        double* red = (double*)smem;
        float hs[4], hq[4];
#pragma unroll
        for (int q = 0; q < 4; ++q) { hs[q] = half_wave_sum_dpp(s2[q >> 1][q & 1]); hq[q] = half_wave_sum_dpp(q2[q >> 1][q & 1]); }
        if ((lane & 31) == 31) {
#pragma unroll
            for (int q = 0; q < 4; ++q) {
                red[wave * 16 + (lane >> 5) * 8 + q] = (double)hs[q];
                red[wave * 16 + (lane >> 5) * 8 + 4 + q] = (double)hq[q];
            }
        }
        __syncthreads();
        if (tid < 2 * p.ST) {
            const int which = tid / p.ST, sl = tid - which * p.ST;
            const int b = sg * p.ST + sl;
            if (b < p.B) {
                double t = 0.0;
                if (p.ST == 8) {
#pragma unroll
                    for (int w = 0; w < NW; ++w) t += red[w * 16 + (sl >> 2) * 8 + which * 4 + (sl & 3)];
                } else {
#pragma unroll
                    for (int w = 0; w < NW; ++w) t += red[w * 16 + which * 4 + sl] + red[w * 16 + 8 + which * 4 + sl];
                }
                stat_add(p.stats_out + 2 * (int64_t)b + which, t, p.inv_n_in < 0.0);
            }
        }
    } else {
        __syncthreads();
        if (tid < p.ST) {
            const int b = sg * p.ST + tid;
            if (b < p.B) {
                double ds = 0.0, dq = 0.0;
                for (int pl = 0; pl < p.PT; ++pl) { ds += (double)rowS[pl * p.ST + tid]; dq += (double)rowQ[pl * p.ST + tid]; }
                stat_add(p.stats_out + 2 * (int64_t)b, ds, p.inv_n_in < 0.0);
                stat_add(p.stats_out + 2 * (int64_t)b + 1, dq, p.inv_n_in < 0.0);
            }
        }
    }
    NAFP_TL(7)
#undef NAFP_TL
    return true;
}

#define NAFP_GEMM_KERNEL(name_, BM_, BN_, BK_, NSTAGE_, MINW_, FUSE0_, EPI_)                 \
    __global__ __launch_bounds__(2 * BM_, MINW_) void name_(const ConvKernelParams p) {       \
        conv_gemm_body<BM_, BN_, BK_, NSTAGE_, FUSE0_, EPI_>(p);                              \
    }
#define NAFP_GEMM_KERNEL_BF16X3(name_, BM_, BN_, NSTAGE_, MINW_)                                \
    __global__ __launch_bounds__(2 * BM_, MINW_) void name_(const ConvKernelParams p) {       \
        conv_gemm_body<BM_, BN_, 16, NSTAGE_, false, 0, 1>(p);                                \
    }
#define NAFP_GEMM_KERNEL_BF16X6(name_, BM_, BN_, NSTAGE_, MINW_, EPI_)                          \
    __global__ __launch_bounds__(2 * BM_, MINW_) void name_(const ConvKernelParams p) {       \
        conv_gemm_body<BM_, BN_, 16, NSTAGE_, false, EPI_, 2>(p);                             \
    }
#define NAFP_GEMM_KERNELS(name_, BM_, BN_, MINW_)                                             \
    NAFP_GEMM_KERNEL(name_##_infer, BM_, BN_, 16, 3, MINW_, false, 0)                         \
    NAFP_GEMM_KERNEL(name_##_train, BM_, BN_, 16, 3, MINW_, false, 1)                         \
    NAFP_GEMM_KERNEL(name_##_any, BM_, BN_, 16, 3, MINW_, false, 2)                           \
    NAFP_GEMM_KERNEL(name_##_plain, BM_, BN_, 16, 3, MINW_, false, 3)
NAFP_GEMM_KERNELS(conv_gemm_k16s3, 128, 128, 3)
NAFP_GEMM_KERNEL(conv_gemm_k16s3_fuse0, 128, 128, 16, 3, 3, true, 0)
NAFP_GEMM_KERNEL(conv_gemm_n64k16s3_infer, 128, 64, 16, 3, 4, false, 0)
NAFP_GEMM_KERNEL(conv_gemm_n64k16s3_train, 128, 64, 16, 3, 4, false, 1)
NAFP_GEMM_KERNEL(conv_gemm_n64k16s3_any, 128, 64, 16, 3, 4, false, 2)
NAFP_GEMM_KERNEL(conv_gemm_n64k16s3_plain, 128, 64, 16, 3, 4, false, 3)
NAFP_GEMM_KERNEL(conv_gemm_n64k16s3_splitfin, 128, 64, 16, 3, 4, false, 4)
NAFP_GEMM_KERNEL(conv_gemm_n64k16s3_plainfin, 128, 64, 16, 3, 4, false, 5)
NAFP_GEMM_KERNEL(conv_gemm_k16s3_plainfin, 128, 128, 16, 3, 3, false, 5)
NAFP_GEMM_KERNEL(conv_gemm_n64k16s2_infer, 128, 64, 16, 2, 5, false, 0)
NAFP_GEMM_KERNEL(conv_gemm_n64k16s2_train, 128, 64, 16, 2, 5, false, 1)
NAFP_GEMM_KERNEL(conv_gemm_n64k16s2_splitfin, 128, 64, 16, 2, 5, false, 4)
NAFP_GEMM_KERNEL(conv_gemm_m256k16s3_infer, 256, 128, 16, 3, 4, false, 0)
NAFP_GEMM_KERNEL(conv_gemm_m256k16s3_train, 256, 128, 16, 3, 4, false, 1)
NAFP_GEMM_KERNEL(conv_gemm_m256k16s3_plain, 256, 128, 16, 3, 4, false, 3)

NAFP_GEMM_KERNEL_BF16X3(conv_gemm_k16s3_infer_bf16x3, 128, 128, 3, 3)
NAFP_GEMM_KERNEL_BF16X3(conv_gemm_m256k16s3_infer_bf16x3, 256, 128, 3, 4)
NAFP_GEMM_KERNEL_BF16X3(conv_gemm_n64k16s2_infer_bf16x3, 128, 64, 2, 5)
#ifndef NAFP_X6_K16_NSTAGE
#define NAFP_X6_K16_NSTAGE 2
#endif
#ifndef NAFP_X6_K16_MINW
#define NAFP_X6_K16_MINW 3
#endif
NAFP_GEMM_KERNEL_BF16X6(conv_gemm_k16s3_infer_bf16x6, 128, 128, NAFP_X6_K16_NSTAGE, NAFP_X6_K16_MINW, 0)
NAFP_GEMM_KERNEL_BF16X6(conv_gemm_n64k16s2_infer_bf16x6, 128, 64, 2, 4, 0)
NAFP_GEMM_KERNEL_BF16X6(conv_gemm_k16s3_plain_bf16x6, 128, 128, NAFP_X6_K16_NSTAGE, NAFP_X6_K16_MINW, 3)
NAFP_GEMM_KERNEL_BF16X6(conv_gemm_k16s3_train_bf16x6, 128, 128, NAFP_X6_K16_NSTAGE, NAFP_X6_K16_MINW, 1)
NAFP_GEMM_KERNEL_BF16X6(conv_gemm_n64k16s2_train_bf16x6, 128, 64, 2, 4, 1)
NAFP_GEMM_KERNEL_BF16X6(conv_gemm_k16s3_any_bf16x6, 128, 128, NAFP_X6_K16_NSTAGE, NAFP_X6_K16_MINW, 2)
NAFP_GEMM_KERNEL_BF16X6(conv_gemm_n64k16s2_any_bf16x6, 128, 64, 2, 4, 2)
NAFP_GEMM_KERNEL_BF16X6(conv_gemm_n64k16s2_plain_bf16x6, 128, 64, 2, 4, 3)
__global__ __launch_bounds__(256, 3) void conv_gemm_k16s2_fuse0_bf16x6(const ConvKernelParams p) {
    conv_gemm_body<128, 128, 16, 2, true, 0, 2>(p);
}

#define NAFP_ROW(k_, BM_, bn_, ring_, extra_, epi_, arith_, fuse0_) {k_, #k_, BM_, bn_, ring_, extra_, epi_, arith_, fuse0_},
const ConvKernelRow conv_kernel_rows[] = {
    NAFP_ROW(conv_gemm_k16s3_infer, 128, 128, 3, 0, 0, 0, false)
    NAFP_ROW(conv_gemm_k16s3_train, 128, 128, 3, 0, 1, 0, false)
    NAFP_ROW(conv_gemm_k16s3_any, 128, 128, 3, 0, 2, 0, false)
    NAFP_ROW(conv_gemm_k16s3_plain, 128, 128, 3, 0, 3, 0, false)
    NAFP_ROW(conv_gemm_k16s3_plainfin, 128, 128, 3, 0, 5, 0, false)
    NAFP_ROW(conv_gemm_k16s3_fuse0, 128, 128, 3, 0, 0, 0, true)
    NAFP_ROW(conv_gemm_n64k16s3_infer, 128, 64, 3, 0, 0, 0, false)
    NAFP_ROW(conv_gemm_n64k16s3_train, 128, 64, 3, 0, 1, 0, false)
    NAFP_ROW(conv_gemm_n64k16s3_any, 128, 64, 3, 0, 2, 0, false)
    NAFP_ROW(conv_gemm_n64k16s3_plain, 128, 64, 3, 0, 3, 0, false)
    NAFP_ROW(conv_gemm_n64k16s3_splitfin, 128, 64, 3, 0, 4, 0, false)
    NAFP_ROW(conv_gemm_n64k16s3_plainfin, 128, 64, 3, 0, 5, 0, false)
    NAFP_ROW(conv_gemm_n64k16s2_infer, 128, 64, 2, 0, 0, 0, false)
    NAFP_ROW(conv_gemm_n64k16s2_train, 128, 64, 2, 0, 1, 0, false)
    NAFP_ROW(conv_gemm_n64k16s2_splitfin, 128, 64, 2, 0, 4, 0, false)
    NAFP_ROW(conv_gemm_m256k16s3_infer, 256, 128, 3, 0, 0, 0, false)
    NAFP_ROW(conv_gemm_m256k16s3_train, 256, 128, 3, 0, 1, 0, false)
    NAFP_ROW(conv_gemm_m256k16s3_plain, 256, 128, 3, 0, 3, 0, false)
    NAFP_ROW(conv_gemm_k16s3_infer_bf16x3, 128, 128, 3, 0, 0, 1, false)
    NAFP_ROW(conv_gemm_m256k16s3_infer_bf16x3, 256, 128, 3, 0, 0, 1, false)
    NAFP_ROW(conv_gemm_n64k16s2_infer_bf16x3, 128, 64, 2, 0, 0, 1, false)
    NAFP_ROW(conv_gemm_k16s3_infer_bf16x6, 128, 128, NAFP_X6_K16_NSTAGE, 128 * 8, 0, 2, false)
    NAFP_ROW(conv_gemm_k16s3_train_bf16x6, 128, 128, NAFP_X6_K16_NSTAGE, 128 * 8, 1, 2, false)
    NAFP_ROW(conv_gemm_k16s3_any_bf16x6, 128, 128, NAFP_X6_K16_NSTAGE, 128 * 8, 2, 2, false)
    NAFP_ROW(conv_gemm_k16s3_plain_bf16x6, 128, 128, NAFP_X6_K16_NSTAGE, 128 * 8, 3, 2, false)
    NAFP_ROW(conv_gemm_n64k16s2_infer_bf16x6, 128, 64, 2, 64 * 8, 0, 2, false)
    NAFP_ROW(conv_gemm_n64k16s2_train_bf16x6, 128, 64, 2, 64 * 8, 1, 2, false)
    NAFP_ROW(conv_gemm_n64k16s2_any_bf16x6, 128, 64, 2, 64 * 8, 2, 2, false)
    NAFP_ROW(conv_gemm_n64k16s2_plain_bf16x6, 128, 64, 2, 64 * 8, 3, 2, false)
    NAFP_ROW(conv_gemm_k16s2_fuse0_bf16x6, 128, 128, 2, 128 * 8 + 128 * 8, 0, 2, true)
};
#undef NAFP_ROW
const int conv_kernel_row_count = (int)(sizeof(conv_kernel_rows) / sizeof(conv_kernel_rows[0]));

__global__ __launch_bounds__(256) void split_weights_multi_kernel(const SplitTable t) {
    const float* __restrict__ wp = t.wp[blockIdx.y];
    unsigned short* __restrict__ hm = (unsigned short*)t.hm[blockIdx.y];
    unsigned short* __restrict__ wl = (unsigned short*)t.wl[blockIdx.y];
    const int64_t n8 = t.n8[blockIdx.y];
    const int K = t.K[blockIdx.y];
    typedef unsigned short u16x8 __attribute__((ext_vector_type(8)));
    for (int64_t i8 = blockIdx.x * 256ll + threadIdx.x; i8 < n8; i8 += (int64_t)gridDim.x * 256) {
        const int64_t i = i8 * 8;
        const float4 a = *(const float4*)(wp + i), b = *(const float4*)(wp + i + 4);
        const float x[8] = {a.x, a.y, a.z, a.w, b.x, b.y, b.z, b.w};
        u16x8 vh, vm, vl;
#pragma unroll
        for (int e = 0; e < 8; ++e) {
            const __bf16 h = (__bf16)x[e];
            const float r1 = x[e] - (float)h;
            const __bf16 m = (__bf16)r1;
            vh[e] = __builtin_bit_cast(unsigned short, h);
            vm[e] = __builtin_bit_cast(unsigned short, m);
            vl[e] = __builtin_bit_cast(unsigned short, (__bf16)(r1 - (float)m));
        }
        const int64_t row = i / K;
        const int k = (int)(i - row * K);
        const int64_t base = row * 2 * K + (int64_t)(k >> 4) * 32 + (k & 8);
        *(u16x8*)(hm + base) = vh;
        *(u16x8*)(hm + base + 16) = vm;
        *(u16x8*)(wl + i) = vl;
    }
}

int launch_split_weights_multi(const SplitTable& t, hipStream_t st) {
    if (t.count <= 0) return NAFP_OK;
    int64_t n8_max = 0;
    for (int j = 0; j < t.count; ++j) {
        if (t.K[j] % 16 != 0) return NAFP_ERR_UNSUPPORTED;
        n8_max = std::max(n8_max, t.n8[j]);
    }
    split_weights_multi_kernel<<<dim3((unsigned)std::min<int64_t>((n8_max + 255) / 256, 1024), (unsigned)t.count), 256, 0, st>>>(t);
    NAFP_LAUNCH_CHECK();
    return NAFP_OK;
}

static int launch_variant(const ConvKernelRow& row, int lds, ConvKernelParams p, dim3 grid, hipStream_t st, hipEvent_t ev_start, hipEvent_t ev_stop) {
    NAFP_HIP_CHECK(hipFuncSetAttribute((const void*)row.fn, hipFuncAttributeMaxDynamicSharedMemorySize, lds));
    if (ev_start || ev_stop) {
        void* args[] = {(void*)&p};
        NAFP_HIP_CHECK(hipExtLaunchKernel((const void*)row.fn, grid, dim3(2 * row.BM), args, (size_t)lds, st, ev_start, ev_stop, 0));
    } else {
        row.fn<<<grid, 2 * row.BM, lds, st>>>(p);
    }
    NAFP_LAUNCH_CHECK();
    return NAFP_OK;
}

constexpr int FIN_MAXS = 64;
template <int FIN_F4>
__global__ __launch_bounds__(256) void splitk_finish_kernel(
        const float* __restrict__ slab, int S, const float* __restrict__ G, const float* __restrict__ Hb,
        const float* __restrict__ gamma_out, const stat_t* __restrict__ stats_in,
        stat_t* __restrict__ stats_out, float* __restrict__ y, float* __restrict__ v_out, int B, int P, int Cout,
        double inv_n_in) {
    __shared__ float sR[FIN_MAXS], sC[FIN_MAXS];
    __shared__ float sPart[4][FIN_F4 / 256][2][2];
    __shared__ int sPartB[4][FIN_F4 / 256][2];
    const int tid = threadIdx.x, lane = tid & 63;
    const int c4 = Cout / 4;
    const int64_t total = (int64_t)B * P * c4;
    const int64_t i0 = (int64_t)blockIdx.x * FIN_F4;
    const int64_t i_last = std::min<int64_t>(total, i0 + FIN_F4) - 1;
    const int b_first = (int)((i0 / c4) / P), b_last = (int)((i_last / c4) / P);
    if (tid <= b_last - b_first) {
        const int b = b_first + tid;
        stat_ln_scalars(stats_in + 2 * (int64_t)b, inv_n_in, &sR[tid], &sC[tid]);
        stat_forward_poison(stats_in + 2 * (int64_t)b, stats_out + 2 * (int64_t)b);
    }
    __syncthreads();
    const int64_t slab_stride4 = total;
#pragma unroll 1
    for (int e = 0; e < FIN_F4 / 256; ++e) {
        const int64_t idx = i0 + e * 256 + tid;
        const bool live = idx < total;
        const int64_t ii = live ? idx : i0;
        const int64_t row = ii / c4;
        const int n = (int)(ii - row * c4) * 4;
        const int b = (int)(row / P), pos = (int)(row - (int64_t)b * P);
        const float4* src = (const float4*)slab + ii;
        float4 acc = src[0];
        for (int sp = 1; sp < S; ++sp) {
            const float4 t = src[sp * slab_stride4];
            acc.x += t.x; acc.y += t.y; acc.z += t.z; acc.w += t.w;
        }
        const float4 g4 = *(const float4*)(G + (int64_t)pos * Cout + n);
        const float4 h4 = *(const float4*)(Hb + (int64_t)pos * Cout + n);
        const float4 go = *(const float4*)(gamma_out + (int64_t)pos * Cout + n);
        const float rb = sR[b - b_first], cb = sC[b - b_first];
        float4 tq, v;
        tq.x = fmaf(rb, acc.x, fmaf(cb, g4.x, h4.x));
        tq.y = fmaf(rb, acc.y, fmaf(cb, g4.y, h4.y));
        tq.z = fmaf(rb, acc.z, fmaf(cb, g4.z, h4.z));
        tq.w = fmaf(rb, acc.w, fmaf(cb, g4.w, h4.w));
        v.x = elu1(tq.x); v.y = elu1(tq.y); v.z = elu1(tq.z); v.w = elu1(tq.w);
        float s = live ? (v.x + v.y) + (v.z + v.w) : 0.f;
        float q = live ? (v.x * v.x + v.y * v.y) + (v.z * v.z + v.w * v.w) : 0.f;
        if (live) {
            ((float4*)y)[idx] = make_float4(v.x * go.x, v.y * go.y, v.z * go.z, v.w * go.w);
            if (v_out) ((float4*)v_out)[idx] = tq;
        }
        const int b_lo = __shfl(b, 0, 64), b_hi = __shfl(b, 63, 64);
        const float s_lo = wave_sum(b == b_lo ? s : 0.f), q_lo = wave_sum(b == b_lo ? q : 0.f);
        const float s_hi = wave_sum(b != b_lo ? s : 0.f), q_hi = wave_sum(b != b_lo ? q : 0.f);
        if (lane == 0) {
            const int w = tid >> 6;
            sPart[w][e][0][0] = s_lo; sPart[w][e][0][1] = q_lo; sPartB[w][e][0] = b_lo;
            sPart[w][e][1][0] = s_hi; sPart[w][e][1][1] = q_hi; sPartB[w][e][1] = b_hi != b_lo ? b_hi : -1;
        }
    }
    __syncthreads();
    if (tid <= b_last - b_first) {
        const int b = b_first + tid;
        double ds = 0.0, dq = 0.0;
        for (int w = 0; w < 4; ++w)
            for (int e = 0; e < FIN_F4 / 256; ++e)
                for (int h = 0; h < 2; ++h)
                    if (sPartB[w][e][h] == b) { ds += (double)sPart[w][e][h][0]; dq += (double)sPart[w][e][h][1]; }
        stat_add(stats_out + 2 * (int64_t)b, ds, inv_n_in < 0.0);
        stat_add(stats_out + 2 * (int64_t)b + 1, dq, inv_n_in < 0.0);
    }
}

__global__ __launch_bounds__(256) void plain_finish_kernel(const float* __restrict__ slab, int S, const float* __restrict__ bias,
                                                          float* __restrict__ y, int64_t n4, int Cout) {
    for (int64_t i = blockIdx.x * 256ll + threadIdx.x; i < n4; i += (int64_t)gridDim.x * 256) {
        float4 acc = ((const float4*)slab)[i];
        for (int sp = 1; sp < S; ++sp) {
            const float4 t = ((const float4*)slab)[i + sp * n4];
            acc.x += t.x; acc.y += t.y; acc.z += t.z; acc.w += t.w;
        }
        if (bias) {
            const float4 bv = *(const float4*)(bias + (4 * i) % Cout);
            acc.x += bv.x; acc.y += bv.y; acc.z += bv.z; acc.w += bv.w;
        }
        ((float4*)y)[i] = acc;
    }
}

static struct { unsigned long long* buf; int64_t capacity; int cin, cout, positions; int last_grid[5]; } g_timeline = {};
int conv_timeline_set(unsigned long long* buf, int64_t capacity_u64, int cin, int cout, int positions) {
    g_timeline.buf = buf; g_timeline.capacity = capacity_u64; g_timeline.cin = cin; g_timeline.cout = cout; g_timeline.positions = positions;
    return NAFP_OK;
}
int conv_timeline_grid(int* out5) { for (int i = 0; i < 5; ++i) out5[i] = g_timeline.last_grid[i]; return NAFP_OK; }

template <int FIN_F4>
static void launch_splitk_finish(const ConvGemmArgs& a, const ConvPlan& pl, const ConvKernelParams& p, hipStream_t st) {
    if (a.ev_stop) hipExtLaunchKernelGGL(splitk_finish_kernel<FIN_F4>, dim3(pl.finish_grid), dim3(256), 0, st, nullptr, a.ev_stop, 0, (const float*)a.slab,
                                         pl.S, a.G, a.Hb, a.gamma_out, a.stats_in, a.stats_out, a.y, a.v_out, p.B, p.P, p.Cout, p.inv_n_in);
    else splitk_finish_kernel<FIN_F4><<<pl.finish_grid, 256, 0, st>>>(a.slab, pl.S, a.G, a.Hb, a.gamma_out, a.stats_in, a.stats_out, a.y, a.v_out,
                                                                     p.B, p.P, p.Cout, p.inv_n_in);
}

int launch_conv_gemm(const ConvGemmArgs& a, int64_t B, const ConvGeom& g, hipStream_t st) {
    ConvPlanIn in{};
    in.B = B; in.plan_b = a.plan_b; in.plain = a.plain; in.dgrad = a.dgrad; in.v_out = a.v_out != nullptr; in.tickets = a.tickets != nullptr;
    in.split_weights = a.wp_hm && a.wp_l; in.bf16x3 = a.bf16x3; in.slab_floats = a.slab ? a.slab_floats : 0;
    in.fuse0 = a.f0_feat != nullptr; in.f0_geom = a.f0_geom;
    const ConvPlan pl = plan_conv_gemm(in, g, conv_knobs());
    if (pl.rc != NAFP_OK) return pl.rc;
    const ConvKernelRow& row = conv_kernel_rows[pl.kernel];
    const bool d = a.dgrad, in_kernel = pl.finish == CONV_FINISH_IN_KERNEL_FULL || pl.finish == CONV_FINISH_IN_KERNEL_PLAIN;

    ConvKernelParams p;
    p.x = a.x; p.wp = a.wp; p.G = a.G; p.Hb = a.Hb; p.gamma_out = a.gamma_out; p.bias = a.bias;
    p.wp_hm = row.arith == 2 ? a.wp_hm : nullptr; p.wp_l = row.arith == 2 ? (const unsigned short*)a.wp_l : nullptr;
    p.stats_in = a.stats_in; p.stats_out = a.stats_out; p.y = a.y; p.v_out = a.v_out;
    p.Fin = d ? g.Fout : g.Fin; p.Tin = d ? g.Tout : g.Tin; p.Cin = d ? g.Cout : g.Cin; p.Tout = d ? g.Tin : g.Tout; p.Cout = d ? g.Cin : g.Cout;
    p.axis = g.axis; p.stride = g.stride; p.pad = g.pad;
    p.B = (int)B; p.P = pl.P;
    p.PT = pl.PT; p.ST = pl.ST;
    p.log2ST = 0;
    while ((1 << p.log2ST) < p.ST) ++p.log2ST;
    p.n_sg = pl.n_sg; p.n_pb = pl.n_pb; p.log2_ncol = pl.log2_ncol; p.xcd_group = pl.xcd_group; p.xcd_full = pl.xcd_full;
    p.sample_in = (int64_t)p.Fin * p.Tin * p.Cin;
    p.tap_stride = d ? -((g.axis == 0 ? g.Cout : g.Tout * g.Cout) / g.stride) : (g.axis == 0 ? g.Cin : g.Tin * g.Cin);
    p.inv_n_in = d ? 1.0 : a.ident_stats ? -1.0 : 1.0 / (double)p.sample_in;
    p.mode = pl.mode; p.dgrad = d;
    p.perm_on = pl.perm_on; p.perm_n0 = pl.perm_n0; p.perm_c0 = pl.perm_c0;
    p.wp_bytes = pl.wp_bytes; p.n_split = pl.S; p.abl = pl.abl; p.opt = pl.opt;
    if (pl.S > 1) { p.y = a.slab; p.bias = pl.finish == CONV_FINISH_IN_KERNEL_PLAIN ? a.bias : nullptr; }
    p.tickets = in_kernel ? a.tickets : nullptr; p.y_final = a.y;
    p.keep_own = (a.nonmatrix & NAFP_NONMATRIX_KEEP_OWN) && pl.finish == CONV_FINISH_IN_KERNEL_FULL && pl.S == 2;
    p.f0_feat = nullptr; p.f0_w = nullptr; p.f0_bias = nullptr; p.f0_gamma = nullptr;
    p.f0_T = 0; p.f0_stride = 1; p.f0_pad = 0; p.f0_gstat = nullptr; p.f0_group = 0; p.f0_segnorm = 0;
    if (a.f0_feat) {
        p.f0_feat = a.f0_feat; p.f0_w = a.f0_w; p.f0_bias = a.f0_bias; p.f0_gamma = a.f0_gamma;
        p.f0_T = a.f0_geom->Tin; p.f0_stride = a.f0_geom->stride; p.f0_pad = a.f0_geom->pad;
        p.f0_gstat = a.f0_gstat; p.f0_group = a.f0_group; p.f0_segnorm = a.f0_segnorm;
    }
    p.sj = (a.sj && a.plain) ? *a.sj : ScalarsJob{nullptr, nullptr, nullptr, nullptr, 0, 0.0};
    p.tl = nullptr;
    if (g_timeline.buf && ((!a.plain && !a.dgrad && g.Cin == g_timeline.cin) || (a.dgrad && g.Cin == -g_timeline.cin)) &&
        g.Cout == g_timeline.cout && g.Fout * g.Tout == g_timeline.positions &&
        (int64_t)pl.grid.x * pl.grid.y * pl.grid.z * 64 <= g_timeline.capacity) {
        p.tl = g_timeline.buf;
        g_timeline.last_grid[0] = (int)pl.grid.x; g_timeline.last_grid[1] = (int)pl.grid.y; g_timeline.last_grid[2] = (int)pl.grid.z;
        g_timeline.last_grid[3] = pl.BM; g_timeline.last_grid[4] = pl.bn;
    }

    const bool finish_follows = pl.finish == CONV_FINISH_KERNEL;
    hipEvent_t ev_stop = finish_follows ? nullptr : a.ev_stop;
    if (pl.range_step > 0) {
        const int64_t out_per_sample = (int64_t)p.P * p.Cout;
        int rc = NAFP_OK;
        for (int64_t b0 = 0; b0 < B && rc == NAFP_OK; b0 += pl.range_step) {
            ConvKernelParams q = p;
            const int64_t bc = std::min<int64_t>(pl.range_step, B - b0);
            q.B = (int)bc; q.n_sg = (int)((bc + p.ST - 1) / p.ST);
            q.x = p.x + b0 * p.sample_in; q.y_final = p.y_final + b0 * out_per_sample;
            if (p.v_out) q.v_out = p.v_out + b0 * out_per_sample;
            q.stats_in = p.stats_in + 2 * b0; q.stats_out = p.stats_out + 2 * b0;
            rc = launch_variant(row, pl.lds_bytes, q, dim3((unsigned)((int64_t)q.n_sg * pl.n_pb), pl.grid.y, pl.grid.z), st,
                                b0 == 0 ? a.ev_start : nullptr, b0 + pl.range_step >= B ? ev_stop : nullptr);
        }
        return rc;
    }
    const int rc = launch_variant(row, pl.lds_bytes, p, pl.grid, st, a.ev_start, ev_stop);
    if (rc != NAFP_OK || !finish_follows) return rc;
    if (a.plain) {
        const int64_t n4 = B * p.P * p.Cout / 4;
        if (a.ev_stop) hipExtLaunchKernelGGL(plain_finish_kernel, dim3(pl.finish_grid), dim3(256), 0, st, nullptr, a.ev_stop, 0, (const float*)a.slab, pl.S, a.bias, a.y, n4, p.Cout);
        else plain_finish_kernel<<<pl.finish_grid, 256, 0, st>>>(a.slab, pl.S, a.bias, a.y, n4, p.Cout);
    } else if (pl.finish_f4 == 1024) launch_splitk_finish<1024>(a, pl, p, st);
    else if (pl.finish_f4 == 512) launch_splitk_finish<512>(a, pl, p, st);
    else launch_splitk_finish<256>(a, pl, p, st);
    NAFP_LAUNCH_CHECK();
    return NAFP_OK;
}

struct DgradLnParams {
    ConvKernelParams c;
    const float* t;
    const float* gamma;
    const float* G; const float* Hb;
    const float* sc;
    float* dts;
    float* dgamma; float* dbeta; float* dbias;
    float* S1; float* S2;
    double* lnsum_below;
    int n_groups, groups_per_wg, n_chunks;
};

__global__ __launch_bounds__(256, 3) void dgrad_ln_kernel(const DgradLnParams q) {
    constexpr int BM = 128, BK = 16, NSTAGE = 3, CH = 4, RPI = 16, NI = 2;
    constexpr int TILE = BM * BK, STAGE = 2 * TILE;
    constexpr unsigned OOB = 0x80000000u;
    const ConvKernelParams& p = q.c;
    extern __shared__ __attribute__((aligned(16))) float smem[];
    float* sSc = smem + NSTAGE * STAGE;
    float* sRow = sSc + BM * 8;
    float* sCol = sRow + BM * 2;
    float* sDummy = sCol + 5 * BN;
    const int tid = threadIdx.x, lane = tid & 63;
    const int wave = __builtin_amdgcn_readfirstlane(tid >> 6);
    const int wm = wave >> 1, wn = wave & 1;
    const int chunk = blockIdx.x % q.n_chunks;
    const int pos = tile_pos(p, blockIdx.x / q.n_chunks);
    const int tile_n0 = blockIdx.y * BN;
    const int K = 3 * p.Cin;
    const int C = p.Cout;
    const RowGeom rg = row_geom(p, pos);
    unsigned tap_pack = 0; int n_live = 0;
#pragma unroll
    for (int t = 0; t < 3; ++t)
        if (rg.mask & (1u << t)) { tap_pack |= (unsigned)t << (2 * n_live); ++n_live; }
    const int cpt = p.Cin / BK, n_steps = n_live * cpt;

    unsigned voffA[NI], voffB[NI];
#pragma unroll
    for (int i = 0; i < NI; ++i) {
        const int lr = wave * 32 + i * RPI + lane / CH;
        const int lc = (lane % CH) ^ ((lr >> 2) & 3);
        voffA[i] = (unsigned)(lr * (int)p.sample_in + rg.inner + lc * 4) * 4u;
        voffB[i] = (unsigned)((tile_n0 + lr) * K + lc * 4) * 4u;
    }
    const u32x4 rsB = make_rsrc(p.wp, p.wp_bytes);
    const unsigned lds0 = (unsigned)(unsigned long long)(lds_ptr_t)smem + (unsigned)(wave * 32 * BK * 4);
    const int rl = lane & 31, hh = lane >> 5;
    const int rswz = (rl >> 2) & 3;
    const int aoff = (wm * 64 + rl) * BK, boff = TILE + (wn * 64 + rl) * BK;
    const int ncol = lane & 31;
    const int n_base = tile_n0 + wn * 64 + ncol;
    float gam[2], Gq[2], Hq[2];
#pragma unroll
    for (int ni = 0; ni < 2; ++ni) {
        const int o = pos * C + n_base + ni * 32;
        gam[ni] = q.gamma[o];
        Gq[ni] = q.lnsum_below ? q.G[o] : 0.f;
        Hq[ni] = q.lnsum_below ? q.Hb[o] : 0.f;
    }
    float ag[2] = {0.f, 0.f}, ab[2] = {0.f, 0.f}, a1[2] = {0.f, 0.f}, a2[2] = {0.f, 0.f};

    const int g_begin = chunk * q.groups_per_wg, g_end = min(q.n_groups, g_begin + q.groups_per_wg);
    for (int grp = g_begin; grp < g_end; ++grp) {
        const int b0 = grp * BM;
        const int nb = min(BM, p.B - b0);
        {
            const int r = tid >> 1, h = tid & 1;
            float4 v = make_float4(0.f, 0.f, 0.f, 0.f);
            if (r < nb) v = *(const float4*)(q.sc + 8 * (int64_t)(b0 + r) + 4 * h);
            *(float4*)(sSc + 8 * r + 4 * h) = v;
            sRow[tid] = 0.f;
            asm volatile("s_waitcnt lgkmcnt(0)" ::: "memory");
        }
        const u32x4 rsA = make_rsrc(p.x + (int64_t)b0 * p.sample_in, (unsigned)nb * (unsigned)p.sample_in * 4u);
        f32x16 acc[2][2];
#pragma unroll
        for (int mi = 0; mi < 2; ++mi)
#pragma unroll
            for (int ni = 0; ni < 2; ++ni)
#pragma unroll
                for (int r = 0; r < 16; ++r) acc[mi][ni][r] = 0.f;
#define NAFP_DL_DMA(s_, slot_)                                                                 \
        {                                                                                      \
            const int tsel_l = (s_) / cpt;                                                     \
            const int tap_l = (int)((tap_pack >> (2 * tsel_l)) & 3u);                          \
            const int c0_l = ((s_) - tsel_l * cpt) * BK;                                       \
            const unsigned la_l = lds0 + (unsigned)((slot_) * STAGE * 4);                      \
            const unsigned tapb_l = (unsigned)(tap_l * p.tap_stride) * 4u;                     \
            _Pragma("unroll") for (int i = 0; i < NI; ++i) {                                   \
                const int lr_l = wave * 32 + i * RPI + lane / CH;                              \
                lds_dma16(la_l + i * RPI * BK * 4, lr_l < nb ? voffA[i] + tapb_l : OOB, rsA, (unsigned)(c0_l * 4)); \
                lds_dma16(la_l + (TILE + i * RPI * BK) * 4, voffB[i], rsB, (unsigned)((tap_l * p.Cin + c0_l) * 4)); \
            }                                                                                  \
        }
#pragma unroll
        for (int s = 0; s < NSTAGE - 1; ++s)
            if (s < n_steps) NAFP_DL_DMA(s, s)
        int slot = 0;
        for (int s = 0; s < n_steps; ++s) {
            if (s + NSTAGE - 2 >= n_steps) asm volatile("s_waitcnt vmcnt(0)" ::: "memory");
            else asm volatile("s_waitcnt vmcnt(%0)" :: "i"((NSTAGE - 2) * 2 * NI) : "memory");
            __builtin_amdgcn_s_barrier();
            int nslot = slot + NSTAGE - 1; if (nslot >= NSTAGE) nslot -= NSTAGE;
            const float* St = smem + slot * STAGE;
            float4 a0[2], b0v[2];
            {
                const int pc4 = ((0 + hh) ^ rswz) * 4;
#pragma unroll
                for (int mi = 0; mi < 2; ++mi) a0[mi] = *(const float4*)(St + aoff + mi * 32 * BK + pc4);
#pragma unroll
                for (int ni = 0; ni < 2; ++ni) b0v[ni] = *(const float4*)(St + boff + ni * 32 * BK + pc4);
            }
            if (s + NSTAGE - 1 < n_steps) NAFP_DL_DMA(s + NSTAGE - 1, nslot)
#pragma unroll
            for (int kk = 0; kk < BK / 8; ++kk) {
                const int pc4 = ((2 * kk + hh) ^ rswz) * 4;
                float4 a[2], b[2];
#pragma unroll
                for (int mi = 0; mi < 2; ++mi) a[mi] = kk == 0 ? a0[mi] : *(const float4*)(St + aoff + mi * 32 * BK + pc4);
#pragma unroll
                for (int ni = 0; ni < 2; ++ni) b[ni] = kk == 0 ? b0v[ni] : *(const float4*)(St + boff + ni * 32 * BK + pc4);
#pragma unroll
                for (int mi = 0; mi < 2; ++mi)
#pragma unroll
                    for (int ni = 0; ni < 2; ++ni) {
                        acc[mi][ni] = __builtin_amdgcn_mfma_f32_32x32x2f32(a[mi].x, b[ni].x, acc[mi][ni], 0, 0, 0);
                        acc[mi][ni] = __builtin_amdgcn_mfma_f32_32x32x2f32(a[mi].y, b[ni].y, acc[mi][ni], 0, 0, 0);
                        acc[mi][ni] = __builtin_amdgcn_mfma_f32_32x32x2f32(a[mi].z, b[ni].z, acc[mi][ni], 0, 0, 0);
                        acc[mi][ni] = __builtin_amdgcn_mfma_f32_32x32x2f32(a[mi].w, b[ni].w, acc[mi][ni], 0, 0, 0);
                    }
            }
            if (++slot == NSTAGE) slot = 0;
        }
#undef NAFP_DL_DMA
        if (n_steps == 0) __syncthreads();
        {
            int PC = p.P * C;
            asm volatile("" : "+s"(PC));
            const __amdgpu_buffer_rsrc_t rsT = __builtin_amdgcn_make_buffer_rsrc(
                const_cast<float*>(q.t) + (int64_t)b0 * PC, 0, (int)((unsigned)nb * (unsigned)PC * 4u), 0x00020000);
            const __amdgpu_buffer_rsrc_t rsO = __builtin_amdgcn_make_buffer_rsrc(
                q.dts + (int64_t)b0 * PC, 0, (int)((unsigned)nb * (unsigned)PC * 4u), 0x00020000);
            const int voff = ((wm * 64 + 4 * hh) * PC + pos * C + n_base) * 4;
            const int row_bytes = PC * 4;
            const float* sScL = sSc + 8 * (wm * 64 + 4 * hh);
            float* sRowL = sRow + 2 * (wm * 64 + 4 * hh);
            const int nbl = nb - (wm * 64 + 4 * hh);
#pragma unroll
            for (int mi = 0; mi < 2; ++mi) {
#pragma unroll
                for (int rq = 0; rq < 4; ++rq) {
                    const int soff0 = (mi * 32 + 8 * rq) * row_bytes;
                    float tv[4][2];
#pragma unroll
                    for (int k = 0; k < 4; ++k) {
                        tv[k][0] = __builtin_bit_cast(float, __builtin_amdgcn_raw_buffer_load_b32(rsT, voff, soff0 + k * row_bytes, 0));
                        tv[k][1] = __builtin_bit_cast(float, __builtin_amdgcn_raw_buffer_load_b32(rsT, voff + 128, soff0 + k * row_bytes, 0));
                    }
#pragma unroll
                    for (int k = 0; k < 4; ++k) {
                        const int r = 4 * rq + k;
                        const int rl_ = mi * 32 + 8 * rq + k;
                        const bool valid = rl_ < nbl;
                        const float4 s0 = *(const float4*)(sScL + 8 * rl_), s1 = *(const float4*)(sScL + 8 * rl_ + 4);
                        const float mean = s0.x, rstd = s0.y, m1 = s0.z, m2 = s0.w, inv_r = s1.x, rprev = s1.y, cprev = s1.z;
                        float q1 = 0.f, q2 = 0.f;
#pragma unroll
                        for (int ni = 0; ni < 2; ++ni) {
                            const float tt = tv[k][ni], dd = acc[mi][ni][r];
                            const float vv = elu1(tt);
                            const float xt = (vv - mean) * rstd;
                            float dt = (dd * gam[ni] - m1 - xt * m2) * (vv > 0.f ? 1.f : vv + 1.f);
                            float du = dd * inv_r;
                            if (!valid) { dt = 0.f; du = 0.f; }
                            const float o = dt * rprev;
                            ag[ni] = fmaf(du, xt, ag[ni]); ab[ni] += du;
                            a1[ni] = fmaf(cprev, o, a1[ni]); a2[ni] += dt;
                            asm volatile("" : "+v"(ag[ni]), "+v"(ab[ni]), "+v"(a1[ni]), "+v"(a2[ni]));
                            q1 = fmaf(o, Gq[ni], q1); q2 = fmaf(o, tt - Hq[ni], q2);
                            __builtin_amdgcn_raw_buffer_store_b32(__builtin_bit_cast(int, o), rsO, voff + 128 * ni, soff0 + k * row_bytes, 0);
                        }
                        q1 = half_wave_sum_dpp(q1); q2 = half_wave_sum_dpp(q2);
                        float* dstq = ncol == 31 ? sRowL + 2 * rl_ : sDummy + lane;
                        atomicAdd(dstq, q1);
                        atomicAdd(ncol == 31 ? dstq + 1 : dstq, q2);
                    }
                    __builtin_amdgcn_sched_barrier(0);
                }
            }
        }
        __syncthreads();
        if (q.lnsum_below && tid < 2 * nb) atomicAdd(q.lnsum_below + 2 * (int64_t)b0 + tid, (double)sRow[tid]);
        __syncthreads();
    }
    for (int i = tid; i < 5 * BN; i += 256) sCol[i] = 0.f;
    __syncthreads();
#pragma unroll
    for (int ni = 0; ni < 2; ++ni) {
        float v0 = ag[ni] + __shfl_xor(ag[ni], 32, 64), v1 = ab[ni] + __shfl_xor(ab[ni], 32, 64);
        float v2 = a1[ni] + __shfl_xor(a1[ni], 32, 64), v3 = a2[ni] + __shfl_xor(a2[ni], 32, 64);
        if (hh == 0) {
            const int cidx = wn * 64 + ni * 32 + ncol;
            atomicAdd(sCol + 0 * BN + cidx, v0); atomicAdd(sCol + 1 * BN + cidx, v1);
            atomicAdd(sCol + 2 * BN + cidx, v2); atomicAdd(sCol + 3 * BN + cidx, v3);
        }
    }
    __syncthreads();
    if (tid < BN) {
        const int o = pos * C + tile_n0 + tid;
        atomicAdd(q.dgamma + o, sCol[0 * BN + tid]);
        atomicAdd(q.dbeta + o, sCol[1 * BN + tid]);
        if (q.S1) { atomicAdd(q.S1 + o, sCol[2 * BN + tid]); atomicAdd(q.S2 + o, sCol[3 * BN + tid]); }
        atomicAdd(q.dbias + tile_n0 + tid, sCol[3 * BN + tid]);
    }
}

bool dgrad_ln_eligible(int64_t B, const ConvGeom& g, int mode) {
    if (mode == 0 || g.Cin % BN != 0 || g.Cout % 16 != 0) return false;
    if ((int64_t)BN * g.Fout * g.Tout * g.Cout * 4 >= ((int64_t)1 << 31)) return false;
    if (mode == 2) return true;
    return B >= 64 && (int64_t)g.Fin * g.Tin * g.Cin >= 32768;
}

int launch_dgrad_ln(const DgradLnArgs& a, int64_t B, const ConvGeom& g, hipStream_t st) {
    if (!dgrad_ln_eligible(B, g, 2)) return NAFP_ERR_UNSUPPORTED;
    DgradLnParams q;
    ConvKernelParams& p = q.c;
    p.x = a.dts_in; p.wp = a.wd; p.G = nullptr; p.Hb = nullptr; p.gamma_out = nullptr; p.bias = nullptr;
    p.stats_in = nullptr; p.stats_out = nullptr; p.y = nullptr; p.v_out = nullptr;
    p.axis = g.axis; p.stride = g.stride; p.pad = g.pad;
    p.dgrad = 1;
    p.Fin = g.Fout; p.Tin = g.Tout; p.Cin = g.Cout; p.Cout = g.Cin; p.Tout = g.Tin;
    p.B = (int)B; p.P = g.Fin * g.Tin;
    p.PT = 1; p.ST = BN; p.log2ST = 7;
    p.n_sg = (int)((B + 127) / 128);
    p.sample_in = (int64_t)g.Fout * g.Tout * g.Cout;
    const int S = g.axis == 0 ? g.Cout : g.Tout * g.Cout;
    p.tap_stride = -(S / g.stride);
    p.inv_n_in = 1.0; p.mode = 1; p.n_split = 1; p.abl = 0; p.tl = nullptr; p.opt = 0; p.tickets = nullptr; p.y_final = nullptr; p.keep_own = 0;
    p.sj = ScalarsJob{nullptr, nullptr, nullptr, nullptr, 0, 0.0};
    p.perm_on = 0; p.perm_n0 = 0; p.perm_c0 = 0;
    p.wp_bytes = (unsigned)((int64_t)g.Cout * 3 * g.Cin * 4);
    p.f0_feat = nullptr; p.f0_w = nullptr; p.f0_bias = nullptr; p.f0_gamma = nullptr; p.f0_T = 0; p.f0_stride = 1; p.f0_pad = 0;
    q.t = a.t; q.gamma = a.gamma; q.G = a.G; q.Hb = a.Hb; q.sc = a.sc; q.dts = a.dts_out;
    q.dgamma = a.dgamma; q.dbeta = a.dbeta; q.dbias = a.dbias; q.S1 = a.S1; q.S2 = a.S2; q.lnsum_below = a.lnsum_below;
    q.n_groups = p.n_sg;
    const int64_t base = (int64_t)p.P * (g.Cin / BN);
    int chunks = (int)std::min<int64_t>(q.n_groups, std::max<int64_t>(1, (1536 + base - 1) / base));
    q.groups_per_wg = (q.n_groups + chunks - 1) / chunks;
    q.n_chunks = (q.n_groups + q.groups_per_wg - 1) / q.groups_per_wg;
    const int lds = (3 * 2 * 128 * 16 + 128 * 8 + 128 * 2 + 5 * BN + 64) * (int)sizeof(float);
    static bool attr = false;
    if (!attr) {
        NAFP_HIP_CHECK(hipFuncSetAttribute((const void*)dgrad_ln_kernel, hipFuncAttributeMaxDynamicSharedMemorySize, lds));
        attr = true;
    }
    dgrad_ln_kernel<<<dim3((unsigned)((int64_t)p.P * q.n_chunks), (unsigned)(g.Cin / BN)), 256, lds, st>>>(q);
    NAFP_LAUNCH_CHECK();
    return NAFP_OK;
}

__global__ void pack_conv_weight_kernel(const float* __restrict__ k3, float* __restrict__ wp, int K, int Cout) {
    __shared__ float t[32][33];
    const int k0 = blockIdx.x * 32, n0 = blockIdx.y * 32;
    const int tx = threadIdx.x & 31, ty = threadIdx.x >> 5;
    for (int r = ty; r < 32; r += 8)
        if (k0 + r < K && n0 + tx < Cout) t[r][tx] = k3[(int64_t)(k0 + r) * Cout + n0 + tx];
    __syncthreads();
    for (int r = ty; r < 32; r += 8)
        if (n0 + r < Cout && k0 + tx < K) wp[(int64_t)(n0 + r) * K + k0 + tx] = t[tx][r];
}

__global__ __launch_bounds__(256) void multi_pack_kernel(const PackTable t) {
    __shared__ float tile[32][33];
    int e = 0;
    while (e + 1 < t.count && t.unit0[e + 1] <= (int)blockIdx.x) ++e;
    const int u = (int)blockIdx.x - t.unit0[e];
    const float* __restrict__ k3 = t.k3[e];
    float* __restrict__ wp = t.wp[e]; float* __restrict__ wd = t.wd[e];
    const int Cin = t.cin[e], Cout = t.cout[e], K = 3 * Cin;
    const int tx = threadIdx.x & 31, ty = threadIdx.x >> 5;
    const int tiles_k = (K + 31) / 32, tiles_n = (Cout + 31) / 32;
    for (int tl = 8 * u; tl < 8 * u + 8 && tl < tiles_k * tiles_n; ++tl) {
        const int k0 = (tl % tiles_k) * 32, n0 = (tl / tiles_k) * 32;
        __syncthreads();
        for (int r = ty; r < 32; r += 8)
            if (k0 + r < K && n0 + tx < Cout) {
                const float w = k3[(int64_t)(k0 + r) * Cout + n0 + tx];
                tile[r][tx] = w;
                if (!(fabsf(w) <= 3.4028234664e38f) && t.nonfinite) atomicOr(t.nonfinite, 1);
            }
        __syncthreads();
        for (int r = ty; r < 32; r += 8)
            if (n0 + r < Cout && k0 + tx < K) wp[(int64_t)(n0 + r) * K + k0 + tx] = tile[tx][r];
    }
    if (wd) {
        const int64_t total = (int64_t)3 * Cin * Cout;
        for (int64_t i = (int64_t)u * 8192 + threadIdx.x; i < (int64_t)(u + 1) * 8192 && i < total; i += 256) {
            const int n = (int)(i % Cout);
            const int64_t r = i / Cout;
            const int c = (int)(r % Cin), k = (int)(r / Cin);
            wd[((int64_t)c * 3 + k) * Cout + n] = k3[i];
        }
    }
}

int launch_multi_pack(const PackTable& t0, hipStream_t st) {
    if (t0.count <= 0) return NAFP_OK;
    PackTable t = t0;
    t.unit0[0] = 0;
    for (int e = 0; e < t.count; ++e) {
        const int64_t tiles = (int64_t)((3 * t.cin[e] + 31) / 32) * ((t.cout[e] + 31) / 32);
        t.unit0[e + 1] = t.unit0[e] + (int)((std::max<int64_t>(tiles * 1024, (int64_t)3 * t.cin[e] * t.cout[e]) + 8191) / 8192);
    }
    multi_pack_kernel<<<dim3((unsigned)t.unit0[t.count]), 256, 0, st>>>(t);
    NAFP_LAUNCH_CHECK();
    return NAFP_OK;
}

__global__ __launch_bounds__(256) void gh_gemv_kernel(const GhTable t) {
    int e = 0;
    while (e + 1 < t.count && t.wg0[e + 1] <= (int)blockIdx.x) ++e;
    const int lane = threadIdx.x & 63, wave = threadIdx.x >> 6;
    const int Cin = t.cin[e], Cout = t.cout[e], P = t.P[e], K3 = 3 * Cin;
    const int n0 = ((int)blockIdx.x - t.wg0[e]) * 16 + wave * 4;
    const float* __restrict__ wp = t.wp[e];
    const float* __restrict__ x = t.x[e];
    float acc[4][16];
// ... 79 lines not shown
```

Measured before the change: 193,600.

## Replace runtime integer divisions with magic-number multiplies and seed accumulators from first MFMA

Result: no change. 192,000 (median of 2 runs) (-0.8%).

```diff
diff --git a/include/nafp.h b/include/nafp.h
--- a/include/nafp.h
+++ b/include/nafp.h
@@ -271,6 +271,8 @@
 #define NAFP_PLAN_SIZE_DGRAD 64
 int nafp_conv_plan(int in_f, int in_t, int layer, int64_t n_seg, int64_t plan_b, int flags, int64_t slab_floats,
                    int64_t* record_host, char* kernel_name_host, int name_capacity);
+
+int nafp_conv_divmagic(const uint32_t* d_host, const uint32_t* n_host, int64_t count, uint32_t* pair_host, uint32_t* q_host);
 
 int64_t nafp_encoder_train_workspace_bytes(const nafp_encoder* enc, int64_t n_seg);
 int nafp_encoder_forward_train(nafp_encoder* enc, const float* feat, int64_t n_seg, void* workspace,
diff --git a/neural-audio-fp_amd/_lib.py b/neural-audio-fp_amd/_lib.py
--- a/neural-audio-fp_amd/_lib.py
+++ b/neural-audio-fp_amd/_lib.py
@@ -89,6 +89,7 @@
     'nafp_conv_timeline': (c_int, [c_void_p, c_i64, c_int, c_int, c_int]),
     'nafp_conv_timeline_grid': (c_int, [c_void_p]),
     'nafp_conv_plan': (c_int, [c_int, c_int, c_int, c_i64, c_i64, c_int, c_i64, c_void_p, c_void_p, c_int]),
+    'nafp_conv_divmagic': (c_int, [c_void_p, c_void_p, c_i64, c_void_p, c_void_p]),
     'nafp_encoder_set_option': (c_int, [c_void_p, c_int, c_int]),
     'nafp_encoder_train_workspace_bytes': (c_i64, [c_void_p, c_i64]),
     'nafp_encoder_forward_train': (c_int, [c_void_p, c_void_p, c_i64, c_void_p, c_i64, c_void_p, c_int, c_void_p]),
diff --git a/neural-audio-fp_amd/build.py b/neural-audio-fp_amd/build.py
--- a/neural-audio-fp_amd/build.py
+++ b/neural-audio-fp_amd/build.py
@@ -11,7 +11,7 @@
 STAMP = os.path.join(HERE, '.libnafp.stamp')
 SOURCES = ['api.hip', 'melspec.hip', 'melspec_any.hip', 'conv.hip', 'conv_plan.hip', 'tail.hip', 'ntxent.hip', 'optim.hip', 'specaug.hip', 'backward.hip',
            'search.hip', 'augment.hip', 'triplet.hip', 'norm.hip', 'ivf.hip', 'hnsw.hip', 'resample.hip', 'ingest.hip', 'codec.hip', 'flac.hip', 'varispeed.hip']
-HEADERS = ['nafp_common.h', 'melspec_plan.h', 'codec_decode.h', 'flac_decode.h', os.path.join('..', '..', 'include', 'nafp.h')]
+HEADERS = ['nafp_common.h', 'conv_geom.h', 'melspec_plan.h', 'codec_decode.h', 'flac_decode.h', os.path.join('..', '..', 'include', 'nafp.h')]
 NO_PACKED_F32 = ['-Xclang', '-target-feature', '-Xclang', '-packed-fp32-ops']
 FLAGS = ['--offload-arch=gfx950', '-O3', '-std=c++17', '-fPIC', '-Wall', '-Wno-unused-result', '-fno-gpu-rdc'] + NO_PACKED_F32
 RESOURCE_FLAG = '-Rpass-analysis=kernel-resource-usage'
diff --git a/neural-audio-fp_amd/csrc/api.hip b/neural-audio-fp_amd/csrc/api.hip
--- a/neural-audio-fp_amd/csrc/api.hip
+++ b/neural-audio-fp_amd/csrc/api.hip
@@ -1,4 +1,5 @@
 #include "nafp_common.h"
+#include "conv_geom.h"
 
 #include <algorithm>
 #include <cstdio>
@@ -745,6 +746,17 @@
     return NAFP_OK;
 }
 
+extern "C" int nafp_conv_divmagic(const uint32_t* d_host, const uint32_t* n_host, int64_t count, uint32_t* pair_host, uint32_t* q_host) {
+    if (!d_host || !n_host || !pair_host || !q_host || count < 0) return NAFP_ERR_INVALID_ARG;
+    for (int64_t i = 0; i < count; ++i) {
+        if (d_host[i] == 0 || d_host[i] >= 0x80000000u || n_host[i] >= 0x80000000u) return NAFP_ERR_INVALID_ARG;
+        const DivMagic k = div_magic((int64_t)d_host[i]);
+        pair_host[2 * i] = k.m; pair_host[2 * i + 1] = k.sh;
+        q_host[i] = div_by(n_host[i], k);
+    }
+    return NAFP_OK;
+}
+
 extern "C" int nafp_encoder_div_enc(nafp_encoder* e, const float* flat, int64_t n_seg,
                                     float* out_emb, int l2norm, void* stream) {
     if (!e || !flat || !out_emb || n_seg < 0) return NAFP_ERR_INVALID_ARG;
diff --git a/neural-audio-fp_amd/csrc/conv.hip b/neural-audio-fp_amd/csrc/conv.hip
--- a/neural-audio-fp_amd/csrc/conv.hip
+++ b/neural-audio-fp_amd/csrc/conv.hip
@@ -1,4 +1,5 @@
 #include "nafp_common.h"
+#include "conv_geom.h"
 #include <hip/hip_ext.h>
 
 #include <cstdlib>
@@ -388,7 +389,19 @@
     const float* f0_gstat;
     int f0_group, f0_segnorm;
     ScalarsJob sj;
+    DivMagic dv_xcd_group, dv_n_rt, dv_n_sg, dv_n_split, dv_cpt, dv_Tout, dv_pn0, dv_pn1, dv_f0_group;
 };
+
+#ifndef NAFP_GEOM_LEGACY
+#define NAFP_GEOM_LEGACY 0
+#endif
+#if NAFP_GEOM_LEGACY
+#define NAFP_UDIV(n_, d_, k_) ((n_) / (d_))
+#define NAFP_VDIV(n_, d_, k_) ((n_) / (d_))
+#else
+#define NAFP_UDIV(n_, d_, k_) (GEOM_MAGIC ? div_by((unsigned)__builtin_amdgcn_readfirstlane((int)(n_)), (k_)) : (unsigned)((n_) / (d_)))
+#define NAFP_VDIV(n_, d_, k_) (GEOM_MAGIC ? (int)div_by((unsigned)(n_), (k_)) : (int)((n_) / (d_)))
+#endif
 
 typedef __attribute__((address_space(3))) void* lds_ptr_t;
 typedef unsigned u32x4 __attribute__((ext_vector_type(4)));
@@ -413,8 +426,9 @@
 }
 
 struct RowGeom { int inner; unsigned mask; };
+template <bool GEOM_MAGIC = true>
 __device__ __forceinline__ RowGeom row_geom(const ConvKernelParams& p, int pos) {
-    const int fo = pos / p.Tout, to = pos - fo * p.Tout;
+    const int fo = NAFP_VDIV(pos, p.Tout, p.dv_Tout), to = pos - fo * p.Tout;
     RowGeom g; g.mask = 0;
     if (!p.dgrad) {
         int pos0, lim;
@@ -439,22 +453,23 @@
     return g;
 }
 
+template <bool GEOM_MAGIC = true>
 __device__ __forceinline__ int tile_pos(const ConvKernelParams& p, int idx) {
     if (!p.perm_on || idx >= p.P) return idx;
     if (p.perm_on == 2) {
-        const int L = p.Tout, lines = p.P / L, n0 = L - 1;
-        if (idx < lines * n0) { const int line = idx / n0; return line * L + (idx - line * n0); }
+        const int L = p.Tout, lines = (int)NAFP_UDIV(p.P, L, p.dv_Tout), n0 = L - 1;
+        if (idx < lines * n0) { const int line = NAFP_VDIV(idx, n0, p.dv_pn0); return line * L + (idx - line * n0); }
         return (idx - lines * n0) * L + n0;
     }
     const int n0 = p.perm_n0;
     if (p.axis == 0) {
-        const int L = p.Tout, lines = p.P / L, n1 = L - n0;
-        if (idx < lines * n0) { const int line = idx / n0; return line * L + 2 * (idx - line * n0) + p.perm_c0; }
-        const int j = idx - lines * n0, line = j / n1;
+        const int L = p.Tout, lines = (int)NAFP_UDIV(p.P, L, p.dv_Tout), n1 = L - n0;
+        if (idx < lines * n0) { const int line = NAFP_VDIV(idx, n0, p.dv_pn0); return line * L + 2 * (idx - line * n0) + p.perm_c0; }
+        const int j = idx - lines * n0, line = NAFP_VDIV(j, n1, p.dv_pn1);
         return line * L + 2 * (j - line * n1) + 1 - p.perm_c0;
     }
-    if (idx < n0 * p.Tout) { const int e = idx / p.Tout; return (2 * e + p.perm_c0) * p.Tout + (idx - e * p.Tout); }
-    const int j = idx - n0 * p.Tout, e = j / p.Tout;
+    if (idx < n0 * p.Tout) { const int e = NAFP_VDIV(idx, p.Tout, p.dv_Tout); return (2 * e + p.perm_c0) * p.Tout + (idx - e * p.Tout); }
+    const int j = idx - n0 * p.Tout, e = NAFP_VDIV(j, p.Tout, p.dv_Tout);
     return (2 * e + 1 - p.perm_c0) * p.Tout + (j - e * p.Tout);
 }
 
@@ -483,6 +498,7 @@
     static_assert(!FUSE0 || (BK == 16 && BM == 128), "the in-kernel conv0 generator is written for BK = 16, BM = 128");
     static_assert(BM == 128 || BM == 256, "tile rows");
     static_assert(BNT == 128 || (BNT == 64 && BM == 128 && !FUSE0), "tile columns");
+    constexpr bool GEOM_MAGIC = !(PREC == 2 && EPI == 2 && BNT == 128);
     constexpr int NIW = BNT / 64;
     constexpr int NT = 2 * BM;
     constexpr int NW = BM / 32;
@@ -514,23 +530,23 @@
         unsigned v = lin;
         if (lin < (unsigned)p.xcd_full) {
             const unsigned xcd = lin & 7u, j = lin >> 3;
-            const unsigned blk = j / G, i = j - blk * G;
+            const unsigned blk = NAFP_UDIV(j, G, p.dv_xcd_group), i = j - blk * G;
             v = (blk * 8u + xcd) * G + i;
         }
         unsigned rt;
         if (p.opt & 16) {
             const unsigned n_rt = (unsigned)(p.n_sg * p.n_pb);
-            unsigned t = v / n_rt; rt = v - t * n_rt;
-            if (p.n_split > 1) { const unsigned c = t / (unsigned)p.n_split; zsp = (int)(t - c * (unsigned)p.n_split); t = c; }
+            unsigned t = NAFP_UDIV(v, n_rt, p.dv_n_rt); rt = v - t * n_rt;
+            if (p.n_split > 1) { const unsigned c = NAFP_UDIV(t, p.n_split, p.dv_n_split); zsp = (int)(t - c * (unsigned)p.n_split); t = c; }
             colz = (int)t;
         } else {
             colz = (int)(v & ((1u << p.log2_ncol) - 1u)); v >>= p.log2_ncol;
-            if (p.n_split > 1) { const unsigned r = v / (unsigned)p.n_split; zsp = (int)(v - r * (unsigned)p.n_split); v = r; }
+            if (p.n_split > 1) { const unsigned r = NAFP_UDIV(v, p.n_split, p.dv_n_split); zsp = (int)(v - r * (unsigned)p.n_split); v = r; }
             rt = v;
         }
-        pb = (int)(rt / (unsigned)p.n_sg); sg = (int)(rt - (unsigned)pb * (unsigned)p.n_sg);
+        pb = (int)NAFP_UDIV(rt, p.n_sg, p.dv_n_sg); sg = (int)(rt - (unsigned)pb * (unsigned)p.n_sg);
     } else
-    if (!(p.opt & 4)) { pb = blockIdx.x / p.n_sg; sg = blockIdx.x - pb * p.n_sg; colz = blockIdx.y; zsp = blockIdx.z; }
+    if (!(p.opt & 4)) { pb = (int)NAFP_UDIV(blockIdx.x, p.n_sg, p.dv_n_sg); sg = blockIdx.x - pb * p.n_sg; colz = blockIdx.y; zsp = blockIdx.z; }
     if ((EPI == 3 || EPI == 5) && p.sj.sc) {
         const long long wg = blockIdx.x + (long long)gridDim.x * (blockIdx.y + (long long)gridDim.y * blockIdx.z);
         const long long n_wg = (long long)gridDim.x * gridDim.y * gridDim.z;
@@ -571,8 +587,8 @@
     if (tid < 32) {
         int pos = p.P, inner = 0; unsigned mask = 0;
         if (tid < p.PT) {
-            pos = tile_pos(p, pb * p.PT + tid);
-            if (pos < p.P) { const RowGeom rg = row_geom(p, pos); inner = rg.inner; mask = rg.mask; }
+            pos = tile_pos<GEOM_MAGIC>(p, pb * p.PT + tid);
+            if (pos < p.P) { const RowGeom rg = row_geom<GEOM_MAGIC>(p, pos); inner = rg.inner; mask = rg.mask; }
         }
         sPos[tid] = pos; sInner[tid] = inner; sMask[tid] = mask;
     }
@@ -617,11 +633,11 @@
         if (pos < p.P && sl < nb) {
             float f0_gmax = 0.f, f0_nh = 0.f, f0_nd = 1.f;
             if (p.f0_gstat) {
-                const int64_t gi = p.f0_group > 0 ? (int64_t)(b0 + sl) / p.f0_group : 0;
+                const int64_t gi = p.f0_group > 0 ? (int64_t)NAFP_VDIV((int64_t)(b0 + sl), p.f0_group, p.dv_f0_group) : 0;
                 f0_gmax = p.f0_gstat[2 * gi];
                 if (p.f0_segnorm) { const float mn = fmaxf(p.f0_gstat[2 * gi + 1] - f0_gmax, -80.f); f0_nh = mn / 2.f; f0_nd = fabsf(f0_nh + 1e-10f); }
             }
-            const int fo = pos / p.Tout, to = pos - fo * p.Tout;
+            const int fo = NAFP_VDIV(pos, p.Tout, p.dv_Tout), to = pos - fo * p.Tout;
             const int f00 = fo * p.stride - p.pad;
             g_off = (f00 * p.Tin + to) * p.Cin;
             const int t00 = to * p.f0_stride - p.f0_pad;
@@ -664,11 +680,11 @@
     const int n_steps_all = n_live * cpt;
     int s_begin = 0, n_steps = n_steps_all;
     if (p.n_split > 1) {
-        s_begin = (int)((unsigned)(n_steps_all * zsp) / (unsigned)p.n_split);
-        n_steps = (int)((unsigned)(n_steps_all * (zsp + 1)) / (unsigned)p.n_split);
+        s_begin = (int)NAFP_UDIV((unsigned)(n_steps_all * zsp), (unsigned)p.n_split, p.dv_n_split);
+        n_steps = (int)NAFP_UDIV((unsigned)(n_steps_all * (zsp + 1)), (unsigned)p.n_split, p.dv_n_split);
     }
 #define NAFP_STEP_AT(step_, tsel_, c0_)                                                        \
-    const int tsel_ = s_begin == 0 ? ((step_) >= cpt ? 1 : 0) : (step_) / cpt;                 \
+    const int tsel_ = s_begin == 0 ? ((step_) >= cpt ? 1 : 0) : (int)NAFP_UDIV((step_), cpt, p.dv_cpt);                 \
     const int c0_ = ((step_) - tsel_ * cpt) * BK;
 
     const u32x4 rsA = make_rsrc(p.x + (int64_t)b0 * p.sample_in,
@@ -700,7 +716,7 @@
     float4 gg0 = make_float4(0.f, 0.f, 0.f, 0.f), gg1 = gg0;
 #define NAFP_GEN_LOAD(s_)                                                                     \
     {                                                                                          \
-        const int tsel_l = (s_) / cpt;                                                         \
+        const int tsel_l = (int)NAFP_UDIV((s_), cpt, p.dv_cpt);                                                        \
         const int tap_l = (int)((tap_pack >> (2 * tsel_l)) & 3u);                              \
         const int c0_l = ((s_) - tsel_l * cpt) * BK;                                           \
         const int go_l = ((g_valid >> tap_l) & 1u) ? g_off + tap_l * p.tap_stride + c0_l + g_ch : 0; \
@@ -711,7 +727,7 @@
     __fmul_rn((ok_l ? elu1(fmaf(xc_l, wt_l[2 * p.Cin + (j_)], fmaf(xb_l, wt_l[p.Cin + (j_)], fmaf(xa_l, wt_l[(j_)], wt_l[3 * p.Cin + (j_)])))) : 0.f), (G_))
 #define NAFP_GEN_STORE(s_, slot_)                                                             \
     {                                                                                          \
-        const int tsel_l = (s_) / cpt;                                                         \
+        const int tsel_l = (int)NAFP_UDIV((s_), cpt, p.dv_cpt);                                                        \
         const int tap_l = (int)((tap_pack >> (2 * tsel_l)) & 3u);                              \
         const int c0_l = ((s_) - tsel_l * cpt) * BK;                                           \
         const bool ok_l = (g_valid >> tap_l) & 1u;                                             \
@@ -726,13 +742,17 @@
             NAFP_GEN_ONE(4, gg1.x), NAFP_GEN_ONE(5, gg1.y), NAFP_GEN_ONE(6, gg1.z), NAFP_GEN_ONE(7, gg1.w)); \
     }
 
+#if NAFP_GEOM_LEGACY || defined(NAFP_ABLATION) || defined(NAFP_ABL_CONST)
+    constexpr bool ACC_FROM_FIRST = false;
+#else
+    constexpr bool ACC_FROM_FIRST = PREC == 0 && !FUSE0 && BK == 16 && !(BM == 128 && BNT == 128 && (EPI == 0 || EPI == 1));
+#endif
     f32x16 acc[2][NIW];
-#pragma unroll
-    for (int mi = 0; mi < 2; ++mi)
-#pragma unroll
-        for (int ni = 0; ni < NIW; ++ni)
-#pragma unroll
-            for (int r = 0; r < 16; ++r) acc[mi][ni][r] = 0.f;
+#define NAFP_ACC_ZERO(z_)                                                                      \
+    _Pragma("unroll") for (int mi = 0; mi < 2; ++mi)                                           \
+        _Pragma("unroll") for (int ni = 0; ni < NIW; ++ni)                                     \
+            _Pragma("unroll") for (int r = 0; r < 16; ++r) acc[mi][ni][r] = (z_);
+    if (!ACC_FROM_FIRST) { NAFP_ACC_ZERO(0.f) }
 
     NAFP_TL(2)
     if (p.opt & 1) __builtin_amdgcn_s_setprio(0);
@@ -807,6 +827,19 @@
             acc[mi][ni] = __builtin_amdgcn_mfma_f32_32x32x2f32(a_[mi].z, b_[ni].z, acc[mi][ni], 0, 0, 0); \
             acc[mi][ni] = __builtin_amdgcn_mfma_f32_32x32x2f32(a_[mi].w, b_[ni].w, acc[mi][ni], 0, 0, 0); \
         }
+#if NAFP_GEOM_LEGACY || defined(NAFP_ABLATION) || defined(NAFP_ABL_CONST)
+#define NAFP_MM_FRAG_FIRST(a_, b_) NAFP_MM_FRAG(a_, b_)
+#else
+#define NAFP_MM_FRAG_FIRST(a_, b_)                                                             \
+    _Pragma("unroll") for (int mi = 0; mi < 2; ++mi)                                           \
+        _Pragma("unroll") for (int ni = 0; ni < NIW; ++ni) {                                   \
+            const f32x16 zero_l = {0.f, 0.f, 0.f, 0.f, 0.f, 0.f, 0.f, 0.f, 0.f, 0.f, 0.f, 0.f, 0.f, 0.f, 0.f, 0.f}; \
+            acc[mi][ni] = __builtin_amdgcn_mfma_f32_32x32x2f32(a_[mi].x, b_[ni].x, zero_l, 0, 0, 0); \
+            acc[mi][ni] = __builtin_amdgcn_mfma_f32_32x32x2f32(a_[mi].y, b_[ni].y, acc[mi][ni], 0, 0, 0); \
+            acc[mi][ni] = __builtin_amdgcn_mfma_f32_32x32x2f32(a_[mi].z, b_[ni].z, acc[mi][ni], 0, 0, 0); \
+            acc[mi][ni] = __builtin_amdgcn_mfma_f32_32x32x2f32(a_[mi].w, b_[ni].w, acc[mi][ni], 0, 0, 0); \
+        }
+#endif
 #define NAFP_WAIT_STEP(s_)                                                                     \
     if (NSTAGE == 2 || (s_) + NSTAGE - 2 >= n_steps) asm volatile("s_waitcnt vmcnt(0)" ::: "memory"); \
     else asm volatile("s_waitcnt vmcnt(%0)" :: "i"((NSTAGE - 2) * NDMA) : "memory");
@@ -945,7 +978,7 @@
             __builtin_amdgcn_sched_barrier(0);
             if (s_begin + NSTAGE - 1 < n_steps && !NAFP_ABL(p, 1)) { NAFP_DMA_PIECE(0, NSTAGE - 1) NAFP_DMA_PIECE(1, NSTAGE - 1) }
             __builtin_amdgcn_sched_barrier(0);
-            NAFP_MM_FRAG(a0, b0)
+            NAFP_MM_FRAG_FIRST(a0, b0)
             __builtin_amdgcn_sched_barrier(0);
             slot = 1;
         }
@@ -1097,7 +1130,15 @@
 #undef NAFP_X6_GEN
 #undef NAFP_X6_MFMAS
 #undef NAFP_X6_READ_FRAGS
-    } else
+    } else {
+    if (ACC_FROM_FIRST) {
+        float4 za[2], zb[NIW];
+#pragma unroll
+        for (int mi = 0; mi < 2; ++mi) { float z_l = 0.f; asm volatile("" : "+v"(z_l)); za[mi] = make_float4(z_l, z_l, z_l, z_l); }
+#pragma unroll
+        for (int ni = 0; ni < NIW; ++ni) { float z_l = 0.f; asm volatile("" : "+v"(z_l)); zb[ni] = make_float4(z_l, z_l, z_l, z_l); }
+        NAFP_MM_FRAG_FIRST(za, zb)
+    }
     for (int s = s_begin; s < n_steps; ++s) {
         if (FUSE0) asm volatile("s_waitcnt vmcnt(0) lgkmcnt(0)" ::: "memory");
         else if (NSTAGE == 2 || s + NSTAGE - 2 >= n_steps) asm volatile("s_waitcnt vmcnt(0)" ::: "memory");
@@ -1144,6 +1185,8 @@
         if (FUSE0 && has_next) NAFP_GEN_STORE(s + NSTAGE - 1, nslot)
         if (++slot == NSTAGE) slot = 0;
     }
+    }
+#undef NAFP_ACC_ZERO
     NAFP_TL(4)
     if (p.opt & 2) __builtin_amdgcn_s_setprio(3);
     asm volatile("s_waitcnt lgkmcnt(0)" ::: "memory");
@@ -1369,7 +1412,7 @@
         }
         __syncthreads();
         if (tid < 2 * p.ST) {
-            const int which = tid / p.ST, sl = tid - which * p.ST;
+            const int which = NAFP_GEOM_LEGACY || !GEOM_MAGIC ? tid / p.ST : tid >> p.log2ST, sl = tid - which * p.ST;
             const int b = sg * p.ST + sl;
             if (b < p.B) {
                 double t = 0.0;
@@ -1532,7 +1575,20 @@
     return NAFP_OK;
 }
 
+static void set_divisors(ConvKernelParams& p) {
+    p.dv_xcd_group = div_magic(p.xcd_group);
+    p.dv_n_rt = div_magic((int64_t)p.n_sg * p.n_pb);
+    p.dv_n_sg = div_magic(p.n_sg);
+    p.dv_n_split = div_magic(p.n_split);
+    p.dv_cpt = div_magic(p.Cin / 16);
+    p.dv_Tout = div_magic(p.Tout);
+    p.dv_pn0 = div_magic(p.perm_on == 2 ? p.Tout - 1 : p.perm_n0);
+    p.dv_pn1 = div_magic(p.Tout - p.perm_n0);
+    p.dv_f0_group = div_magic(p.f0_group);
+}
+
 static int launch_variant(const ConvKernelRow& row, int lds, ConvKernelParams p, dim3 grid, hipStream_t st, hipEvent_t ev_start, hipEvent_t ev_stop) {
+    set_divisors(p);
     NAFP_HIP_CHECK(hipFuncSetAttribute((const void*)row.fn, hipFuncAttributeMaxDynamicSharedMemorySize, lds));
     if (ev_start || ev_stop) {
         void* args[] = {(void*)&p};
@@ -1550,7 +1606,7 @@
         const float* __restrict__ slab, int S, const float* __restrict__ G, const float* __restrict__ Hb,
         const float* __restrict__ gamma_out, const stat_t* __restrict__ stats_in,
         stat_t* __restrict__ stats_out, float* __restrict__ y, float* __restrict__ v_out, int B, int P, int Cout,
-        double inv_n_in) {
+        double inv_n_in, DivMagic dv_c4, DivMagic dv_P) {
     __shared__ float sR[FIN_MAXS], sC[FIN_MAXS];
     __shared__ float sPart[4][FIN_F4 / 256][2][2];
     __shared__ int sPartB[4][FIN_F4 / 256][2];
@@ -1559,7 +1615,12 @@
     const int64_t total = (int64_t)B * P * c4;
     const int64_t i0 = (int64_t)blockIdx.x * FIN_F4;
     const int64_t i_last = std::min<int64_t>(total, i0 + FIN_F4) - 1;
+#if NAFP_GEOM_LEGACY
     const int b_first = (int)((i0 / c4) / P), b_last = (int)((i_last / c4) / P);
+#else
+    const int b_first = (int)div_by(div_by((unsigned)__builtin_amdgcn_readfirstlane((int)i0), dv_c4), dv_P);
+    const int b_last = (int)div_by(div_by((unsigned)__builtin_amdgcn_readfirstlane((int)i_last), dv_c4), dv_P);
+#endif
     if (tid <= b_last - b_first) {
         const int b = b_first + tid;
         stat_ln_scalars(stats_in + 2 * (int64_t)b, inv_n_in, &sR[tid], &sC[tid]);
@@ -1572,9 +1633,15 @@
         const int64_t idx = i0 + e * 256 + tid;
         const bool live = idx < total;
         const int64_t ii = live ? idx : i0;
+#if NAFP_GEOM_LEGACY
         const int64_t row = ii / c4;
         const int n = (int)(ii - row * c4) * 4;
         const int b = (int)(row / P), pos = (int)(row - (int64_t)b * P);
+#else
+        const int row = (int)div_by((unsigned)ii, dv_c4);
+        const int n = ((int)ii - row * c4) * 4;
+        const int b = (int)div_by((unsigned)row, dv_P), pos = row - b * P;
+#endif
         const float4* src = (const float4*)slab + ii;
         float4 acc = src[0];
         for (int sp = 1; sp < S; ++sp) {
@@ -1620,7 +1687,7 @@
 }
 
 __global__ __launch_bounds__(256) void plain_finish_kernel(const float* __restrict__ slab, int S, const float* __restrict__ bias,
-                                                          float* __restrict__ y, int64_t n4, int Cout) {
+                                                          float* __restrict__ y, int64_t n4, int Cout, DivMagic dv_c4) {
     for (int64_t i = blockIdx.x * 256ll + threadIdx.x; i < n4; i += (int64_t)gridDim.x * 256) {
         float4 acc = ((const float4*)slab)[i];
         for (int sp = 1; sp < S; ++sp) {
@@ -1628,7 +1695,12 @@
             acc.x += t.x; acc.y += t.y; acc.z += t.z; acc.w += t.w;
         }
         if (bias) {
+#if NAFP_GEOM_LEGACY
             const float4 bv = *(const float4*)(bias + (4 * i) % Cout);
+#else
+            const unsigned iu = (unsigned)i, c4 = (unsigned)Cout >> 2;
+            const float4 bv = *(const float4*)(bias + 4u * (iu - div_by(iu, dv_c4) * c4));
+#endif
             acc.x += bv.x; acc.y += bv.y; acc.z += bv.z; acc.w += bv.w;
         }
         ((float4*)y)[i] = acc;
@@ -1645,9 +1717,10 @@
 template <int FIN_F4>
 static void launch_splitk_finish(const ConvGemmArgs& a, const ConvPlan& pl, const ConvKernelParams& p, hipStream_t st) {
     if (a.ev_stop) hipExtLaunchKernelGGL(splitk_finish_kernel<FIN_F4>, dim3(pl.finish_grid), dim3(256), 0, st, nullptr, a.ev_stop, 0, (const float*)a.slab,
-                                         pl.S, a.G, a.Hb, a.gamma_out, a.stats_in, a.stats_out, a.y, a.v_out, p.B, p.P, p.Cout, p.inv_n_in);
+                                         pl.S, a.G, a.Hb, a.gamma_out, a.stats_in, a.stats_out, a.y, a.v_out, p.B, p.P, p.Cout, p.inv_n_in,
+                                         div_magic(p.Cout / 4), div_magic(p.P));
     else splitk_finish_kernel<FIN_F4><<<pl.finish_grid, 256, 0, st>>>(a.slab, pl.S, a.G, a.Hb, a.gamma_out, a.stats_in, a.stats_out, a.y, a.v_out,
-                                                                     p.B, p.P, p.Cout, p.inv_n_in);
+                                                                     p.B, p.P, p.Cout, p.inv_n_in, div_magic(p.Cout / 4), div_magic(p.P));
 }
 
 int launch_conv_gemm(const ConvGemmArgs& a, int64_t B, const ConvGeom& g, hipStream_t st) {
@@ -1698,6 +1771,7 @@
     }
 
     const bool finish_follows = pl.finish == CONV_FINISH_KERNEL;
+    if (finish_follows && B * (int64_t)p.P * (p.Cout / 4) >= ((int64_t)1 << 31)) return NAFP_ERR_UNSUPPORTED;
     hipEvent_t ev_stop = finish_follows ? nullptr : a.ev_stop;
     if (pl.range_step > 0) {
         const int64_t out_per_sample = (int64_t)p.P * p.Cout;
@@ -1718,8 +1792,8 @@
     if (rc != NAFP_OK || !finish_follows) return rc;
     if (a.plain) {
         const int64_t n4 = B * p.P * p.Cout / 4;
-        if (a.ev_stop) hipExtLaunchKernelGGL(plain_finish_kernel, dim3(pl.finish_grid), dim3(256), 0, st, nullptr, a.ev_stop, 0, (const float*)a.slab, pl.S, a.bias, a.y, n4, p.Cout);
-        else plain_finish_kernel<<<pl.finish_grid, 256, 0, st>>>(a.slab, pl.S, a.bias, a.y, n4, p.Cout);
+        if (a.ev_stop) hipExtLaunchKernelGGL(plain_finish_kernel, dim3(pl.finish_grid), dim3(256), 0, st, nullptr, a.ev_stop, 0, (const float*)a.slab, pl.S, a.bias, a.y, n4, p.Cout, div_magic(p.Cout / 4));
+        else plain_finish_kernel<<<pl.finish_grid, 256, 0, st>>>(a.slab, pl.S, a.bias, a.y, n4, p.Cout, div_magic(p.Cout / 4));
     } else if (pl.finish_f4 == 1024) launch_splitk_finish<1024>(a, pl, p, st);
     else if (pl.finish_f4 == 512) launch_splitk_finish<512>(a, pl, p, st);
     else launch_splitk_finish<256>(a, pl, p, st);
@@ -1745,6 +1819,7 @@
     constexpr int TILE = BM * BK, STAGE = 2 * TILE;
     constexpr unsigned OOB = 0x80000000u;
     const ConvKernelParams& p = q.c;
+    constexpr bool GEOM_MAGIC = true;
     extern __shared__ __attribute__((aligned(16))) float smem[];
     float* sSc = smem + NSTAGE * STAGE;
     float* sRow = sSc + BM * 8;
@@ -1812,7 +1887,7 @@
                 for (int r = 0; r < 16; ++r) acc[mi][ni][r] = 0.f;
 #define NAFP_DL_DMA(s_, slot_)                                                                 \
         {                                                                                      \
-            const int tsel_l = (s_) / cpt;                                                     \
+            const int tsel_l = (int)NAFP_UDIV((s_), cpt, p.dv_cpt);                                                    \
             const int tap_l = (int)((tap_pack >> (2 * tsel_l)) & 3u);                          \
             const int c0_l = ((s_) - tsel_l * cpt) * BK;                                       \
             const unsigned la_l = lds0 + (unsigned)((slot_) * STAGE * 4);                      \
@@ -1970,10 +2045,12 @@
     p.inv_n_in = 1.0; p.mode = 1; p.n_split = 1; p.abl = 0; p.tl = nullptr; p.opt = 0; p.tickets = nullptr; p.y_final = nullptr; p.keep_own = 0;
     p.sj = ScalarsJob{nullptr, nullptr, nullptr, nullptr, 0, 0.0};
     p.perm_on = 0; p.perm_n0 = 0; p.perm_c0 = 0;
+    p.n_pb = p.P; p.log2_ncol = 0; p.xcd_group = 1; p.xcd_full = 0; p.f0_group = 0;
     p.wp_bytes = (unsigned)((int64_t)g.Cout * 3 * g.Cin * 4);
     p.f0_feat = nullptr; p.f0_w = nullptr; p.f0_bias = nullptr; p.f0_gamma = nullptr; p.f0_T = 0; p.f0_stride = 1; p.f0_pad = 0;
     q.t = a.t; q.gamma = a.gamma; q.G = a.G; q.Hb = a.Hb; q.sc = a.sc; q.dts = a.dts_out;
     q.dgamma = a.dgamma; q.dbeta = a.dbeta; q.dbias = a.dbias; q.S1 = a.S1; q.S2 = a.S2; q.lnsum_below = a.lnsum_below;
+    set_divisors(p);
     q.n_groups = p.n_sg;
     const int64_t base = (int64_t)p.P * (g.Cin / BN);
     int chunks = (int)std::min<int64_t>(q.n_groups, std::max<int64_t>(1, (1536 + base - 1) / base));
diff --git a/neural-audio-fp_amd/csrc/conv_geom.h b/neural-audio-fp_amd/csrc/conv_geom.h
--- /dev/null
+++ b/neural-audio-fp_amd/csrc/conv_geom.h
@@ -0,0 +1,35 @@
+#pragma once
+#include <stdint.h>
+
+#if defined(__HIPCC__) || defined(__CUDACC__)
+#define NAFP_GEOM_HD __host__ __device__ __forceinline__
+#else
+#define NAFP_GEOM_HD inline
+#endif
+
+namespace nafp {
+
+struct DivMagic { unsigned m, sh; };
+
+inline DivMagic div_magic(int64_t d) {
+    DivMagic k{0x80000000u, 0u};
+    if (d <= 1 || d >= ((int64_t)1 << 31)) return k;
+    unsigned l = 0;
+    while (((int64_t)1 << l) < d) ++l;
+    const uint64_t two = (uint64_t)1 << (31 + l);
+    k.m = (unsigned)((two + (uint64_t)d - 1) / (uint64_t)d);
+    k.sh = l;
+    return k;
+}
+
+NAFP_GEOM_HD unsigned mulhi_u32(unsigned a, unsigned b) {
+#if defined(__HIP_DEVICE_COMPILE__)
+    return __umulhi(a, b);
+#else
+    return (unsigned)(((uint64_t)a * (uint64_t)b) >> 32);
+#endif
+}
+
+NAFP_GEOM_HD unsigned div_by(unsigned n, DivMagic k) { return mulhi_u32(n << 1, k.m) >> k.sh; }
+
+}
```
